# Oliverbansk/Holistic-Robot-Pose-Estimation

Hardware: AMD Instinct MI355X
Metric: images/sec/GPU fwd+bwd HRNet-W32 256x256 bs=64; 1/2/4/8-GPU scaling (higher is better)
Workload: dtype bf16; 1 GPU; full network (HRNet-W32 reg backbone + HRNet-W32 DepthNet + heads + FK loss) fwd+loss+bwd+clip+Adam, BASELINE.json configs[2]; global_batch=64, per_gpu_batch=64, image=3x256x256, hrnet_w32_passes_per_image=2, parallelism=dp1, backend=single-process, rccl_ranks=1, hip_graph=True, plan_mode=hybrid, inputs=resident in HBM, optimizer=hrpe_amd.optim.FusedClipAdam (clip 5 + Adam, lr 1e-4)

## Files before the change

holistic-robot-pose-estimation_amd/_native.py:

```python
import ctypes as C
import os
import subprocess

_HERE = os.path.dirname(os.path.abspath(__file__))
LIB_PATH = os.environ.get("HRP_LIB") or os.path.join(_HERE, "libhrp_hip.so")
CSRC = os.path.join(_HERE, "csrc")

HRP_F32, HRP_BF16, HRP_F32X3 = 0, 1, 2
MAX_TAPS = 16
EW_MAX_IN = 4
EW_IDENTITY, EW_AFFINE, EW_BN_TRAIN = 0, 1, 2
FK_MAX_JOINTS, FK_MAX_KP = 32, 24
PIL_KMAX = 12


class HrpError(RuntimeError):
    pass


class ConvDesc(C.Structure):
    _fields_ = [("x", C.c_void_p), ("w", C.c_void_p), ("y", C.c_void_p), ("res", C.c_void_p),
                ("bias", C.c_void_p), ("scale", C.c_void_p), ("shift", C.c_void_p), ("stats", C.c_void_p),
                ("dtype", C.c_int32),
                ("N", C.c_int32), ("H", C.c_int32), ("W", C.c_int32), ("Cin", C.c_int32), ("x_pitch", C.c_int32),
                ("Ho", C.c_int32), ("Wo", C.c_int32), ("Cout", C.c_int32),
                ("y_H", C.c_int32), ("y_W", C.c_int32), ("y_pitch", C.c_int32), ("res_pitch", C.c_int32),
                ("out_stride", C.c_int32), ("out_off_y", C.c_int32), ("out_off_x", C.c_int32),
                ("in_stride", C.c_int32), ("ntaps", C.c_int32),
                ("dy", C.c_int32 * MAX_TAPS), ("dx", C.c_int32 * MAX_TAPS), ("wtap", C.c_int32 * MAX_TAPS),
                ("w_ntaps", C.c_int32), ("w_cout_pad", C.c_int32), ("relu", C.c_int32),
                ("bnb_x", C.c_void_p), ("bnb_mask", C.c_void_p), ("bnb_consts", C.c_void_p),
                ("bnb_x_pitch", C.c_int32), ("bnb_mask_pitch", C.c_int32),
                ("bnb_stats", C.c_void_p), ("bnb_gamma", C.c_void_p), ("bnb_beta", C.c_void_p),
                ("bnb_count", C.c_float), ("bnb_eps", C.c_float),
                ("pro_mode", C.c_int32), ("pro_reserved", C.c_int32),
                ("pro_x2", C.c_void_p), ("pro_stats", C.c_void_p), ("pro_bsums", C.c_void_p),
                ("pro_gamma", C.c_void_p), ("pro_beta", C.c_void_p),
                ("pro_count", C.c_float), ("pro_eps", C.c_float), ("pro_side", C.c_void_p),
                ("pro_mask", C.c_void_p), ("pro_side2", C.c_void_p), ("pro_side2_acc", C.c_int32), ("pro_reserved2", C.c_int32),
                ("res_mask", C.c_void_p),
                ("tail_mode", C.c_int32), ("tail_side_acc", C.c_int32), ("tail_stats", C.c_void_p), ("tail_bsums", C.c_void_p),
                ("tail_gamma", C.c_void_p), ("tail_beta", C.c_void_p), ("tail_count", C.c_float), ("tail_eps", C.c_float),
                ("tail_mask", C.c_void_p), ("tail_g", C.c_void_p), ("tail_side", C.c_void_p),
                ("tail_x2", C.c_void_p), ("tail_w2", C.c_void_p), ("tail_stats2", C.c_void_p), ("tail_gamma2", C.c_void_p),
                ("tail_beta2", C.c_void_p)]


class WgradDesc(C.Structure):
    _fields_ = [("x", C.c_void_p), ("dy", C.c_void_p), ("dw", C.c_void_p),
                ("dtype", C.c_int32),
                ("N", C.c_int32), ("H", C.c_int32), ("W", C.c_int32), ("Cin", C.c_int32), ("x_pitch", C.c_int32),
                ("Ho", C.c_int32), ("Wo", C.c_int32), ("Cout", C.c_int32), ("dy_pitch", C.c_int32),
                ("in_stride", C.c_int32), ("ntaps", C.c_int32),
                ("dy_t", C.c_int32 * MAX_TAPS), ("dx_t", C.c_int32 * MAX_TAPS),
                ("dw_cin", C.c_int32), ("dw_tap_stride", C.c_int32), ("dw_tap_off", C.c_int32), ("accumulate", C.c_int32),
                ("workspace", C.c_void_p), ("workspace_bytes", C.c_int64),
                ("phase", C.c_int32), ("reserved", C.c_int32)]


class WgradFoldDesc(C.Structure):
    _fields_ = [("workspace", C.c_void_p), ("dw", C.c_void_p),
                ("G", C.c_int32), ("pairs", C.c_int32), ("n_cib", C.c_int32), ("nte", C.c_int32), ("nb", C.c_int32),
                ("Cout", C.c_int32), ("dw_cin", C.c_int32), ("ntaps", C.c_int32), ("dw_tap_stride", C.c_int32),
                ("dw_tap_off", C.c_int32), ("accumulate", C.c_int32), ("reserved", C.c_int32)]


WGRAD_FOUR_WAVE, WGRAD_EIGHT_WAVE_BF16, WGRAD_EIGHT_WAVE_F32X3 = range(3)


class WgradConfig(C.Structure):
    _fields_ = [("program", C.c_int32), ("arrange", C.c_int32), ("nks", C.c_int32), ("BM", C.c_int32),
                ("TI", C.c_int32), ("TH", C.c_int32), ("TW", C.c_int32), ("ring", C.c_int32), ("xmode", C.c_int32),
                ("G", C.c_int32), ("ntiles", C.c_int32), ("pairs", C.c_int32), ("use_ws", C.c_int32),
                ("reserved", C.c_int32 * 3)]


class Sim2RealLossDesc(C.Structure):
    _fields_ = [("rendered", C.c_void_p), ("seg", C.c_void_p), ("kp3d", C.c_void_p), ("kp3d_int", C.c_void_p),
                ("B", C.c_int32), ("HW", C.c_int32), ("K", C.c_int32), ("mask_loss", C.c_int32),
                ("w_mask", C.c_float), ("w_iou", C.c_float), ("w_scale", C.c_float), ("w_align", C.c_float),
                ("terms", C.c_void_p), ("d_rendered", C.c_void_p), ("d_kp3d", C.c_void_p), ("d_kp3d_int", C.c_void_p),
                ("workspace", C.c_void_p)]


class SilhouetteDesc(C.Structure):
    _fields_ = [("uv", C.c_void_p), ("xyz", C.c_void_p), ("faces", C.c_void_p),
                ("B", C.c_int32), ("V", C.c_int32), ("F", C.c_int32), ("H", C.c_int32), ("W", C.c_int32),
                ("sigma", C.c_float), ("blur_radius", C.c_float), ("alpha", C.c_void_p), ("logp", C.c_void_p), ("count", C.c_void_p)]


BLOCK_MAX = 2


class BlockDesc(C.Structure):
    _fields_ = [("conv1", ConvDesc), ("conv2", ConvDesc)]


class BlockInfo(C.Structure):
    _fields_ = [("n", C.c_int32), ("grid", C.c_int32), ("lds_bytes", C.c_int32), ("reserved", C.c_int32),
                ("first_wg", C.c_int32 * BLOCK_MAX), ("bands", C.c_int32 * BLOCK_MAX)]


class PackEntry(C.Structure):
    _fields_ = [("src", C.c_void_p), ("dst", C.c_void_p), ("dst_t", C.c_void_p),
                ("Cout", C.c_int32), ("Cin", C.c_int32), ("ntaps", C.c_int32), ("pad_t", C.c_int32)]


class EwInput(C.Structure):
    _fields_ = [("ptr", C.c_void_p), ("pitch", C.c_int32), ("up", C.c_int32), ("mode", C.c_int32),
                ("a", C.c_void_p), ("b", C.c_void_p), ("stats", C.c_void_p),
                ("count", C.c_float), ("eps", C.c_float)]


class EwDesc(C.Structure):
    _fields_ = [("inp", EwInput * EW_MAX_IN), ("nin", C.c_int32), ("out", C.c_void_p),
                ("out_pitch", C.c_int32), ("dtype", C.c_int32),
                ("N", C.c_int32), ("H", C.c_int32), ("W", C.c_int32), ("C", C.c_int32), ("relu", C.c_int32),
                ("mask", C.c_void_p), ("mask_pitch", C.c_int32), ("consts_out", C.c_void_p)]


class EwBwdDesc(C.Structure):
    _fields_ = [("dout", C.c_void_p), ("out", C.c_void_p), ("dout_pitch", C.c_int32), ("out_pitch", C.c_int32),
                ("inp", EwInput), ("din", C.c_void_p), ("din_pitch", C.c_int32), ("sums", C.c_void_p),
                ("dtype", C.c_int32), ("N", C.c_int32), ("H", C.c_int32), ("W", C.c_int32), ("C", C.c_int32),
                ("relu", C.c_int32), ("accumulate", C.c_int32),
                ("mask", C.c_void_p), ("mask_pitch", C.c_int32),
                ("din2", C.c_void_p), ("din2_pitch", C.c_int32), ("accumulate2", C.c_int32), ("pooled", C.c_void_p)]


class BnEntry(C.Structure):
    _fields_ = [("stats", C.c_void_p), ("a", C.c_void_p), ("b", C.c_void_p), ("c", C.c_void_p), ("d", C.c_void_p),
                ("out_scale", C.c_void_p), ("out_shift", C.c_void_p), ("counter", C.c_void_p),
                ("C", C.c_int32), ("count", C.c_float), ("momentum", C.c_float), ("eps", C.c_float),
                ("accumulate", C.c_int32)]


BATCH_MAX = 32
BATCH_CONV, BATCH_WGRAD, BATCH_EW_FWD, BATCH_EW_BWD_REDUCE, BATCH_EW_BWD_APPLY, BATCH_WGRAD_FOLD = range(6)


class BatchInfo(C.Structure):
    _fields_ = [("family", C.c_int32), ("n", C.c_int32), ("dtype", C.c_int32), ("variant", C.c_int32),
                ("grid", C.c_int32), ("lds_bytes", C.c_int32), ("grid2", C.c_int32),
                ("grid3", C.c_int32), ("lds_bytes3", C.c_int32),
                ("blk0", C.c_int32 * (BATCH_MAX + 1)), ("blk2", C.c_int32 * (BATCH_MAX + 1)),
                ("ws_bytes", C.c_int64 * BATCH_MAX)]


class PoseLossDesc(C.Structure):
    _fields_ = [(n, C.c_void_p) for n in ("pose", "rot", "trans", "root_uv", "depth", "xyz_int", "xyz_fk",
                                          "gt_pose", "gt_root_rot", "gt_root_trans", "gt_root_uv", "gt_kp3d", "gt_kp2d", "mask", "K",
                                          "d_pose", "d_rot", "d_trans", "d_root_uv", "d_depth", "d_xyz_int", "d_xyz_fk", "out")] + \
               [("weights", C.c_float * 10), ("B", C.c_int32), ("P", C.c_int32), ("J", C.c_int32), ("root", C.c_int32),
                ("image_size", C.c_float), ("rot_dim", C.c_int32)]


class EvalDesc(C.Structure):
    INPUTS = ("pred_kp3d_fk", "pred_kp3d_int", "gt_kp3d", "gt_kp2d", "K", "pred_joint", "gt_joint", "pred_rot", "gt_rot")
    PER_IMAGE = ("error3d", "error2d", "mean_jointerror", "error_depth", "batch_error_relative", "error3d_relative",
                 "error3d_int", "error2d_int", "error_depth_int", "batch_error_relative_int", "error3d_relative_int")
    PER_BATCH = ("dis3d", "dis2d", "dis3d_int", "dis2d_int", "l1_jointerror", "rotation_diff")
    _fields_ = [(n, C.c_void_p) for n in INPUTS + PER_IMAGE + PER_BATCH] + \
               [(n, C.c_int32) for n in ("B", "nkp", "dof", "rot_dim", "root", "drop_last_joint", "offset", "capacity",
                                         "batch_index", "batch_capacity")]


DEPTH_LOSS_MAX_KP = 16
DEPTH_LOSS_KINDS = {"l1": 0, "mse": 1}
XY_LOSS_KINDS = {None: 0, "l1": 1, "mse": 2}


class DepthLossDesc(C.Structure):
    POINTERS = ("pred", "gt_root_trans", "gt_kp3d", "mask", "loss", "d_pred", "errors", "losses")
    _fields_ = [(n, C.c_void_p) for n in POINTERS] + \
               [(n, C.c_int32) for n in ("B", "W", "J", "nk")] + [("kp_index", C.c_int32 * DEPTH_LOSS_MAX_KP)] + \
               [(n, C.c_int32) for n in ("depth_loss", "xy_loss", "root_col", "want_grad", "offset", "capacity", "batch_index",
                                         "batch_capacity")]


SIM2REAL_ROW = ("loss", "loss_joint", "loss_rot", "loss_trans", "loss_uv", "loss_depth", "loss_error2d", "loss_error3d", "loss_mask",
                "loss_scale", "loss_iou", "loss_error3d_align")


class Sim2RealMonitorDesc(C.Structure):
    INPUTS = ("pose", "rot", "trans", "root_uv", "depth", "xyz_fk", "gt_pose", "gt_root_rot", "gt_root_trans", "gt_root_uv",
              "gt_kp3d", "gt_kp2d", "mask", "K")
    _fields_ = [(n, C.c_void_p) for n in INPUTS + ("mask_terms", "row", "meters", "rows")] + \
               [("B", C.c_int32), ("P", C.c_int32), ("J", C.c_int32), ("image_size", C.c_float), ("row_index", C.c_int32),
                ("capacity", C.c_int32)]


OPT_CHUNK = 4096


class OptTensor(C.Structure):
    _fields_ = [("param", C.c_void_p), ("grad", C.c_void_p), ("exp_avg", C.c_void_p), ("exp_avg_sq", C.c_void_p),
                ("numel", C.c_int64)]


class OptChunk(C.Structure):
    _fields_ = [("tensor", C.c_int32), ("offset", C.c_int32)]


class OptGroup(C.Structure):
    _fields_ = [("lr", C.c_float), ("beta1", C.c_float), ("beta2", C.c_float), ("eps", C.c_float),
                ("weight_decay", C.c_float), ("reserved", C.c_float * 3)]


class RegStepDesc(C.Structure):
    _fields_ = [("M", C.c_int32), ("P", C.c_int32), ("K", C.c_int32), ("N", C.c_int32),
                ("u_prev", C.c_void_p), ("u_bias", C.c_void_p), ("z", C.c_void_p), ("zw", C.c_void_p),
                ("z_len", C.c_int32), ("z_pitch", C.c_int32), ("zw_sk", C.c_int32), ("zw_sp", C.c_int32),
                ("u_out", C.c_void_p), ("a", C.c_void_p), ("a_mask", C.c_void_p), ("v", C.c_void_p),
                ("a_pitch", C.c_int32), ("v_sk", C.c_int32), ("v_sp", C.c_int32), ("a2_pitch", C.c_int32),
                ("a_out", C.c_void_p), ("w", C.c_void_p), ("bias", C.c_void_p), ("out_mask", C.c_void_p),
                ("a2", C.c_void_p), ("w2", C.c_void_p), ("w_sn", C.c_int64), ("w_sk", C.c_int64),
                ("out_pitch", C.c_int32), ("out_accumulate", C.c_int32), ("out_sum_accumulate", C.c_int32), ("w2_sk", C.c_int32),
                ("out", C.c_void_p), ("out_sum", C.c_void_p)]


class LinWgradDesc(C.Structure):
    _fields_ = [("x", C.c_void_p), ("dy", C.c_void_p), ("dw", C.c_void_p), ("dbias", C.c_void_p),
                ("x_pitch", C.c_int32), ("dy_pitch", C.c_int32), ("dw_ld", C.c_int32), ("M", C.c_int32),
                ("K", C.c_int32), ("N", C.c_int32), ("accumulate", C.c_int32), ("reserved", C.c_int32)]


REG_MAX_P, REG_MAX_PROBLEMS, LIN_WGRAD_MAX = 16, 4, 8
COPY_MAX = 16


class CopyDesc(C.Structure):
    _fields_ = [("src", C.c_void_p), ("dst", C.c_void_p), ("src_pitch", C.c_int), ("dst_pitch", C.c_int), ("rows", C.c_int),
                ("cols", C.c_int), ("accumulate", C.c_int), ("reserved", C.c_int)]


def copy_cols_batch(items, stream):
    for i0 in range(0, len(items), COPY_MAX):
        grp = items[i0:i0 + COPY_MAX]
        arr = (CopyDesc * len(grp))()
        for d, (src, sp, dst, dp, rows, cols, acc) in zip(arr, grp):
            d.src, d.src_pitch, d.dst, d.dst_pitch, d.rows, d.cols, d.accumulate = src, sp, dst, dp, rows, cols, acc
        call("hrp_copy_cols_batch", arr, len(grp), stream)


class FkChain(C.Structure):
    _fields_ = [("njoints", C.c_int32), ("parent", C.c_int32 * FK_MAX_JOINTS), ("type", C.c_int32 * FK_MAX_JOINTS),
                ("cfg", C.c_int32 * FK_MAX_JOINTS), ("mimic_mul", C.c_float * FK_MAX_JOINTS),
                ("mimic_off", C.c_float * FK_MAX_JOINTS), ("origin", (C.c_float * 12) * FK_MAX_JOINTS),
                ("axis", (C.c_float * 3) * FK_MAX_JOINTS), ("nkp", C.c_int32), ("kp_frame", C.c_int32 * FK_MAX_KP),
                ("kp_offset", (C.c_float * 3) * FK_MAX_KP), ("dof", C.c_int32)]


DREAM_BANDS = 32
DREAM_JITTER, DREAM_OCCLUSION, DREAM_SHARPNESS, DREAM_CONTRAST, DREAM_BRIGHTNESS, DREAM_COLOR = 1, 2, 4, 8, 16, 32


class DreamSample(C.Structure):
    _fields_ = [("jitter", C.c_double * 3), ("enh", C.c_double * 4), ("flags", C.c_int32),
                ("occ_x", C.c_int32), ("occ_y", C.c_int32), ("occ_w", C.c_int32), ("occ_h", C.c_int32),
                ("pad_x", C.c_int32), ("pad_y", C.c_int32), ("work_w", C.c_int32), ("work_h", C.c_int32),
                ("crop_x0", C.c_int32), ("crop_y0", C.c_int32), ("crop_x1", C.c_int32), ("crop_y1", C.c_int32),
                ("off_x", C.c_int32), ("off_y", C.c_int32), ("side", C.c_int32), ("reserved", C.c_int32),
                ("noise_off", C.c_int64), ("scratch_off", C.c_int64)]


JPEG_ERR_DATA, JPEG_ERR_MARKER, JPEG_ERR_CODE, JPEG_ERR_INDEX, JPEG_ERR_DESC, JPEG_WARN_TRAILING, JPEG_ERR_CHECKSUM = 1, 2, 4, 8, 16, 32, 64


class JpegHuff(C.Structure):
    _fields_ = [("counts", C.c_uint8 * 16), ("values", C.c_uint8 * 256)]


class JpegImage(C.Structure):
    _fields_ = [("scan_off", C.c_int64), ("scan_len", C.c_int64), ("coef_off", C.c_int64), ("plane_off", C.c_int64),
                ("frame_off", C.c_int64), ("width", C.c_int32), ("height", C.c_int32), ("hsamp", C.c_int32), ("vsamp", C.c_int32),
                ("restart_interval", C.c_int32), ("scan_sum", C.c_uint32), ("sum_len", C.c_int64),
                ("comp_tq", C.c_uint8 * 4), ("comp_td", C.c_uint8 * 4), ("comp_ta", C.c_uint8 * 4), ("reserved2", C.c_uint8 * 4),
                ("quant", (C.c_uint16 * 64) * 4), ("dc", JpegHuff * 2), ("ac", JpegHuff * 2)]


class JpegSegment(C.Structure):
    _fields_ = [("off", C.c_int64), ("len", C.c_int64), ("image", C.c_int32), ("mcu0", C.c_int32)]


TRACK_NO_ESTIMATE, TRACK_BAD_BOX, TRACK_LOST_OUT = 1, 2, 4
TRACK_BBOX_EXTENDED, TRACK_BBOX_ORIGIN, TRACK_BBOX_STRICT = 0, 1, 2
PNP_NO_CONSENSUS, PNP_CONVERGED, PNP_FEW_POINTS = 1, 2, 4
PNP_POOLED_MAX_N, PNP_POOLED_REFITS = 16384, 8
TRACK_MAX_KP, TRACK_MAX_SIZE = 32, 4096
SEED_SKIPPED, SEED_TAKEN, SEED_REFUSED = 1, 2, 4
VERIFY_SKIPPED, VERIFY_KEPT, VERIFY_UNDECIDED, VERIFY_DROPPED = 1, 2, 4, 8
VERIFY_FAIL_SUPPORT, VERIFY_FAIL_COVERAGE, VERIFY_FAIL_IOU = 16, 32, 64
TRACK_MAX_BONES, TRACK_MAX_SAMPLES = 32, 64
KIN_CONVERGED, KIN_AT_LIMIT, KIN_FEW_ROWS, KIN_BAD_START = 1, 2, 4, 8
KIN_MAX_IT = 200
KF_INIT, KF_COASTED, KF_LOST, KF_BAD_START, KF_REWRAPPED, KF_CONVERGED, KF_AT_LIMIT = 1, 2, 4, 8, 16, 32, 64
KIN_FILTER_MAX_N = 20
KS_SMOOTHED, KS_TAIL, KS_INVALID, KS_BAD_LINK, KS_CLAMPED = 1, 2, 4, 8, 16
KP_STRIP_ROWS = 1


class TrackGeom(C.Structure):
    _fields_ = [("status", C.c_int32), ("crop_x0", C.c_int32), ("crop_y0", C.c_int32), ("crop_x1", C.c_int32), ("crop_y1", C.c_int32),
                ("side", C.c_int32), ("off_x", C.c_int32), ("off_y", C.c_int32), ("bbox_strict_bounded", (C.c_float * 4) * 2),
                ("bbox_gt2d_extended", (C.c_float * 4) * 2), ("bbox_strict_bounded_original", C.c_float * 4)]


class TrackVerifyDesc(C.Structure):
    _fields_ = [(n, C.c_void_p) for n in ("state_kp2d", "state_have", "mask", "alpha", "verify_status", "counts", "sums")] + \
               [(n, C.c_int32) for n in ("B", "nkp", "hm", "wm", "nb", "samples", "min_fg", "min_samples")] + \
               [("bones", (C.c_int32 * 2) * TRACK_MAX_BONES), ("scale", C.c_double * 2), ("extend_ratio", C.c_double * 2),
                ("min_support", C.c_double), ("min_coverage", C.c_double), ("min_iou", C.c_double), ("min_prob", C.c_float),
                ("reserved", C.c_int32)]


class KinDesc(C.Structure):
    _fields_ = [(n, C.c_void_p) for n in ("chain", "pts2d", "w2d", "pts3d", "w3d", "K")] + \
               [("K_stride", C.c_int32), ("nkp", C.c_int32)] + [(n, C.c_void_p) for n in ("q0", "rot0", "trans0")] + \
               [("rot_dim", C.c_int32), ("pose_stride", C.c_int32)] + [(n, C.c_void_p) for n in ("q_lo", "q_hi", "prior_q")] + \
               [("free_q", C.c_uint32), ("free_pose", C.c_int32), ("root", C.c_int32), ("B", C.c_int32), ("dof", C.c_int32),
                ("reserved", C.c_int32)] + \
               [(n, C.c_void_p) for n in ("q", "rot", "trans", "xyz", "uv", "rms", "status", "cov")]


class KinFilterDesc(C.Structure):
    _fields_ = [(n, C.c_void_p) for n in ("chain", "pts2d", "w2d", "K")] + [("K_stride", C.c_int32), ("nkp", C.c_int32)] + \
               [(n, C.c_void_p) for n in ("q_in", "rot_in", "trans_in")] + [("rot_dim", C.c_int32), ("pose_stride", C.c_int32)] + \
               [(n, C.c_void_p) for n in ("q_lo", "q_hi", "w_q", "q_meas", "keep", "q_acc", "p0_var")] + \
               [("free_q", C.c_uint32), ("free_pose", C.c_int32), ("root", C.c_int32), ("B", C.c_int32), ("dof", C.c_int32),
                ("max_coast", C.c_int32), ("dt", C.c_double), ("gate_chi2", C.c_double)] + \
               [(n, C.c_void_p) for n in ("mean", "cov", "valid", "coast", "q", "rot", "trans", "xyz", "uv", "vel", "cov_p", "xyz_next", "d2",
                                          "status")]


class KinHistoryDesc(C.Structure):
    _fields_ = [(n, C.c_void_p) for n in ("mean", "cov", "valid", "status", "q_in", "h_mean", "h_cov", "h_valid", "h_flags", "h_dt", "h_q_in")] + \
               [(n, C.c_int32) for n in ("B", "n", "dof", "cap", "slot", "reserved")] + [("dt", C.c_double)]


class KinSmoothDesc(C.Structure):
    _fields_ = [(n, C.c_void_p) for n in ("chain", "mean", "cov", "valid", "flags", "dt", "q_in", "rot_fixed", "trans_fixed", "q_lo", "q_hi",
                                          "q_acc", "gain", "link")] + \
               [("free_q", C.c_uint32)] + [(n, C.c_int32) for n in ("free_pose", "root", "B", "dof", "nkp", "rot_dim", "cap", "first", "L",
                                                                    "want_cov", "reserved")] + \
               [(n, C.c_void_p) for n in ("q", "rot", "trans", "vel", "cov_p", "xyz", "status", "mean_s", "cov_s")]


_P, _I, _F, _L, _Z = C.c_void_p, C.c_int, C.c_float, C.c_int64, C.c_size_t
PROTOTYPES = {
    "hrp_version": [], "hrp_device_ok": [],
    "hrp_nchw_to_nhwc": [_P, _P, _I, _I, _I, _I, _I, _I, _P],
    "hrp_nhwc_to_nchw": [_P, _P, _I, _I, _I, _I, _I, _I, _P],
    "hrp_nchw_grad_from_nhwc": [_P, _P, _I, _I, _I, _I, _I, _I, _P],
    "hrp_pack_weights": [_P, _I, _I, _I, _P],
    "hrp_pack_blocks": [_I, _I, _I, _I, _I, _I],
    "hrp_pack_weights_compact": [_P, _P, _I, _I, _I, _P],
    "hrp_nchw_to_nhwc_s2d": [_P, _P, _I, _I, _I, _I, _I, _I, _P],
    "hrp_u8_nchw_to_nhwc": [_P, _P, _I, _I, _I, _I, _I, _I, _F, _I, _P],
    "hrp_gather_f32": [_P, _P, _P, _I, _I, _P],
    "hrp_pil_resize_table": [_I, _I, _P],
    "hrp_pil_resize_normalize": [_P, _I, _I, _I, _I, _P, _P, _I, _I, _P, _I, _I, _I, _P, _P, _P],
    "hrp_broadcast_hw": [_P, _I, _P, _I, _I, _I, _I, _I, _P],
    "hrp_bilinear_nhwc_to_nchw": [_P, _I, _I, _I, _I, _I, _I, _P, _I, _I, _I, _P],
    "hrp_fill_zero": [_P, _L, _P],
    "hrp_maxpool3x3s2_fwd": [_P, _I, _I, _I, _I, _I, _I, _P, _I, _P, _P],
    "hrp_maxpool3x3s2_bwd": [_P, _I, _P, _P, _I, _I, _I, _I, _I, _I, _I, _P],
    "hrp_conv2d_fwd": [C.POINTER(ConvDesc), _P],
    "hrp_conv_rowstrip_channels": [C.POINTER(ConvDesc)],
    "hrp_conv_pointwise": [C.POINTER(ConvDesc)],
    "hrp_conv_parity_fusable": [C.POINTER(ConvDesc)],
    "hrp_conv_parity_fuse_enable": [_I],
    "hrp_conv_tile_config": [C.POINTER(ConvDesc)],
    "hrp_conv2d_bwd_weight": [C.POINTER(WgradDesc), _P],
    "hrp_colsum": [_P, _I, _L, _I, _I, _P, _I, _P, _L, _P],
    "hrp_colsum_workspace_bytes": [_L, _I],
    "hrp_ew_fwd": [C.POINTER(EwDesc), _P],
    "hrp_ew_bwd_reduce": [C.POINTER(EwBwdDesc), _P],
    "hrp_ew_pool2": [_P, _I, _I, _P, _I, _I, _I, _I, _I, _P, _P],
    "hrp_ew_bwd_apply": [C.POINTER(EwBwdDesc), _P],
    "hrp_bn_running_update": [_P, _I, _P], "hrp_bn_fold": [_P, _I, _P], "hrp_bn_param_grad": [_P, _I, _P],
    "hrp_avgpool_fwd": [_P, _I, _I, _I, _I, _I, _P, _I, _P],
    "hrp_avgpool_bwd": [_P, _I, _P, _I, _I, _I, _I, _I, _I, _P],
    "hrp_softargmax3d_fwd": [_P, _I, _I, _I, _I, _I, _I, _I, _I, _I, _P, _P, _P],
    "hrp_softargmax3d_bwd": [_P, _I, _I, _I, _I, _I, _I, _I, _I, _I, _P, _P, _P, _P, _I, _P],
    "hrp_pose_geometry_fwd": [_P, _P, _P, _P, _I, _I, _I, _F, _F, _P, _P, _P, _P, _P],
    "hrp_pose_geometry_bwd": [_P, _P, _P, _P, _I, _I, _I, _F, _F, _P, _P, _P, _P, _P, _P, _P],
    "hrp_fk_project_fwd": [_P, _P, _P, _P, _P, _I, _I, _P, _P, _P, _P],
    "hrp_fk_project_bwd": [_P, _P, _P, _P, _P, _I, _I, _P, _P, _P, _P, _P, _P],
    "hrp_fk_project_rot_fwd": [_P, _P, _P, _I, _P, _P, _I, _I, _P, _P, _P, _P],
    "hrp_fk_project_rot_bwd": [_P, _P, _P, _I, _P, _P, _I, _I, _P, _P, _P, _P, _P, _P],
    "hrp_copy_cols": [_P, _I, _P, _I, _I, _I, _I, _P],
    "hrp_copy_cols_batch": [_P, _I, _P],
    "hrp_scale_rows": [_P, _I, _I, _I, _P, _F, _P],
    "hrp_mul_f32": [_P, _I, _P, _I, _P, _I, _I, _I, _I, _P],
    "hrp_opt_grad_sumsq": [_P, _P, _I, _P, _P, _P],
    "hrp_opt_adam_step": [_P, _P, _I, _P, _F, _P, _F, _F, _F, _F, _P],
    "hrp_opt_adam_step_groups": [_P, _P, _I, _P, _F, _P, _P, _I, _P, _P],
    "hrp_opt_set_group": [_P, _I, _I, _F, _F, _F, _F, _F, _P],
    "hrp_grad_accumulate": [_P, _P, _L, _I, _F, _P],
    "hrp_batch_prepare": [_I, _P, _I, _P, C.POINTER(BatchInfo)],
    "hrp_batch_launch": [_P, C.POINTER(BatchInfo), _P],
    "hrp_batch_conv_parity_configs": [_P, C.POINTER(BatchInfo), _P],
    "hrp_softargmax_flat_fwd": [_P, _I, _I, _I, _I, _I, _P, _P, _P],
    "hrp_softargmax_flat_bwd": [_P, _I, _I, _I, _I, _I, _P, _P, _P, _P, _I, _P],
    "hrp_rot6d_compose_fwd": [_P, _P, _P, _I, _P],
    "hrp_rot6d_compose_bwd": [_P, _P, _P, _P, _P, _I, _I, _I, _P],
    "hrp_wgrad_fold_desc_of": [C.POINTER(WgradDesc), C.POINTER(WgradFoldDesc)],
    "hrp_batch_wgrad_fold_descs": [_P, C.POINTER(BatchInfo), C.POINTER(WgradFoldDesc)],
    "hrp_wgrad_config_of": [C.POINTER(WgradDesc), C.POINTER(WgradConfig)],
    "hrp_batch_wgrad_configs": [_P, C.POINTER(BatchInfo), C.POINTER(WgradConfig)],
    "hrp_block_channels": [C.POINTER(BlockDesc)],
    "hrp_block_prepare": [_P, _I, _P, C.POINTER(BlockInfo)],
    "hrp_block_launch": [_P, C.POINTER(BlockInfo), _P],
    "hrp_pose_loss": [C.POINTER(PoseLossDesc), _P],
    "hrp_l1_loss": [_P, _P, _F, _I, _P, _P, _P],
    "hrp_sim2real_loss": [C.POINTER(Sim2RealLossDesc), _P],
    "hrp_mesh_pose": [_P, _P, _P, _P, _I, _I, _P, _P, _I, _P, _P, _P, _P],
    "hrp_mesh_pose_bwd": [_P, _P, _P, _P, _I, _I, _P, _P, _I, _P, _P, _P, _P],
    "hrp_silhouette_fwd": [C.POINTER(SilhouetteDesc), _P],
    "hrp_silhouette_bwd": [C.POINTER(SilhouetteDesc), _P, _P, _P],
    "hrp_linear_fwd": [_P, _I, _P, _P, _P, _I, _P, _I, _I, _I, _I, _P, _L, _P],
    "hrp_linear_bwd_data": [_P, _I, _P, _P, _I, _I, _I, _I, _I, _P, _L, _P],
    "hrp_linear_workspace_bytes": [_I, _I, _I],
    "hrp_linear_bwd_weight": [_P, _I, _P, _I, _P, _P, _I, _I, _I, _I, _P],
    "hrp_rng_advance": [_P, _P],
    "hrp_dropout_f32": [_P, _I, _P, _I, _P, _I, _I, _F, _P, C.c_uint32, _P],
    "hrp_dropout_masks": [_P, _L, _F, _P, C.c_uint32, _P],
    "hrp_regressor_step": [_P, _I, _P],
    "hrp_linear_wgrad_batch": [_P, _I, _P],
    "hrp_project_fwd": [_P, _P, _I, _I, _P, _P],
    "hrp_project_bwd": [_P, _P, _P, _I, _I, _P, _P],
    "hrp_pnp_solve": [_P, _P, _I, _P, _I, _P, _I, _I, _P, _P, _P, _P],
    "hrp_pnp_bwd": [_P, _P, _I, _P, _I, _P, _P, _I, _I, _I, _P, _P, _P, _P, _P, _P, _P],
    "hrp_pnp_solve_robust": [_P, _P, _I, _P, _I, _P, _I, _I, C.c_double, _I, _I, C.c_uint32, _I, _P, _P, _P, _P, _P],
    "hrp_pnp_bwd_masked": [_P, _P, _I, _P, _I, _P, _P, _P, _I, _I, _I, _P, _P, _P, _P, _P, _P, _P],
    "hrp_pnp_pooled_workspace_bytes": [_I, _I, _I, C.POINTER(C.c_size_t)],
    "hrp_pnp_solve_pooled": [_P, _P, _P, _I, _P, _I, _I, C.c_double, _I, _I, C.c_uint32, _I, _P, _Z, _P, _P, _P, _P, _P, _P],
    "hrp_dream_augment": [_P, _I, _I, _I, _P, _P, _L, _I, _I, _P, _L, _P, _P],
    "hrp_dream_crop_resize": [_P, _L, _P, _P, _I, _I, _I, _P, _I, _I, _P, _I, _I, _P],
    "hrp_eval_batch": [C.POINTER(EvalDesc), _P],
    "hrp_depth_loss": [C.POINTER(DepthLossDesc), _P],
    "hrp_sim2real_monitor": [C.POINTER(Sim2RealMonitorDesc), _P],
    "hrp_jpeg_decode": [_P, _I, _P, _I, _P, _Z, _P, _Z, _P, _Z, _P, _Z, _P, _P],
    "hrp_jpeg_decode_stage": [_I, _I, _P, _I, _P, _I, _P, _Z, _P, _Z, _P, _Z, _P, _Z, _P, _P],
    "hrp_jpeg_decode_sync": [_P, _I, _P, _I, _P, _I, _I, _P, _Z, _P, _Z, _P, _Z, _P, _Z, _P, _Z, _P, _P],
    "hrp_jpeg_decode_sync_stage": [_I, _I, _I, _P, _I, _P, _I, _P, _I, _I, _P, _Z, _P, _Z, _P, _Z, _P, _Z, _P, _Z, _P, _P],
    "hrp_jpeg_sync_scratch_bytes": [_Z, _I, _I],
    "hrp_track_prepare": [_P, _P, _P, _P, _I, _I, _I, _I, _P, _I, _I, _P, _I, _I, C.POINTER(C.c_double), _I, _P, _P, _P, _P, _P],
    "hrp_track_update": [_P, _P, _I, _I, _I, _I, _I, _P, _P, _P, _P, _P],
    "hrp_track_seed": [_P, _I, _I, C.POINTER(C.c_double), _P, _I, _I, _F, _P, _F, _I, _I, _I, _I, _P, _P, _P, _P],
    "hrp_track_verify": [C.POINTER(TrackVerifyDesc), _P],
    "hrp_kin_solve": [C.POINTER(KinDesc), _P],
    "hrp_kin_filter_step": [C.POINTER(KinFilterDesc), _P],
    "hrp_kin_history_push": [C.POINTER(KinHistoryDesc), _P],
    "hrp_kin_smooth": [C.POINTER(KinSmoothDesc), _P],
    "hrp_kp_readout_pack": [_P, _I, _I, _P, _I, _P],
    "hrp_kp_readout_ws": [_I, _I],
    "hrp_kp_readout_fwd": [_P, _I, _I, _I, _I, _I, _I, _P, _P, _I, _F, _F, _F, _F, _P, _P, _P, _L, _P],
}

_lib = None


def source_hash():
    import glob
    import hashlib
    files = [os.path.basename(f) for f in glob.glob(os.path.join(CSRC, "*.hip")) + glob.glob(os.path.join(CSRC, "*.h"))]
    names = sorted(files + ["../../include/hrp.h", "Makefile"])
    h = hashlib.sha256()
    for n in names:
        with open(os.path.join(CSRC, n), "rb") as fh:
            h.update(fh.read())
    return h.hexdigest()[:16]


def build(force=False):
    if force:
        subprocess.run(["make", "-C", CSRC, "clean"], check=True, stdout=subprocess.DEVNULL)
    r = subprocess.run(["make", "-C", CSRC, "-j8"], stdout=subprocess.PIPE, stderr=subprocess.STDOUT, text=True)
    if r.returncode != 0:
        raise HrpError("building libhrp_hip.so failed:\n" + r.stdout[-4000:])
    return LIB_PATH


def lib():
    global _lib
    if _lib is None:
        if not os.path.exists(LIB_PATH):
            raise HrpError(f"{LIB_PATH} not found: run `python -c 'import __graft_entry__ as g; g.build()'` "
                           "(there is no CPU fallback)")
        import torch
        L = C.CDLL(LIB_PATH)
        for name, args in PROTOTYPES.items():
            fn = getattr(L, name)
            fn.argtypes = args
            fn.restype = C.c_int
        L.hrp_last_error.restype = C.c_char_p
        L.hrp_last_error.argtypes = []
        L.hrp_source_hash.restype = C.c_char_p
        L.hrp_source_hash.argtypes = []
        L.hrp_wgrad_workspace_bytes.restype = C.c_int64
        L.hrp_linear_workspace_bytes.restype = C.c_int64
        L.hrp_colsum_workspace_bytes.restype = C.c_int64
        L.hrp_wgrad_workspace_bytes.argtypes = [C.POINTER(WgradDesc)]
        L.hrp_batch_table_bytes.restype = C.c_int64
        L.hrp_batch_table_bytes.argtypes = [C.c_int, C.c_int]
        L.hrp_block_table_bytes.restype = C.c_int64
        L.hrp_block_table_bytes.argtypes = []
        L.hrp_jpeg_sync_scratch_bytes.restype = C.c_size_t
        L.hrp_kp_readout_ws.restype = C.c_int64
        _lib = L
    return _lib


def check(rc, what=""):
    if rc != 0:
        raise HrpError(f"{what} failed ({rc}): {lib().hrp_last_error().decode()}")


_profile_hook = None


def set_profile_hook(fn):
    global _profile_hook
    _profile_hook = fn


def profiling():
    return _profile_hook is not None


_skip = frozenset(filter(None, os.environ.get("HRP_SKIP", "").split(",")))


def call(name, *args):
    if _skip and name in _skip:
        return
    if _profile_hook is not None:
        _profile_hook(name, args, lambda: check(getattr(lib(), name)(*args), name))
        return
    check(getattr(lib(), name)(*args), name)


def call_batch(batch, stream):
    name = "hrp_batch_launch"
    if _skip and (name in _skip or FAMILY_FN[batch.fam] in _skip):
        return
    fn = lambda: check(lib().hrp_batch_launch(batch.table.data_ptr(), C.byref(batch.info), stream), name)
    if _profile_hook is not None:
        _profile_hook(name, (batch,), fn)
        return
    fn()


def call_block(batch, stream):
    name = "hrp_block_launch"
    if _skip and name in _skip:
        return
    fn = lambda: check(lib().hrp_block_launch(batch.table, C.byref(batch.info), stream), name)
    if _profile_hook is not None:
        _profile_hook(name, (batch,), fn)
        return
    fn()


FAMILY_FN = {"block": "hrp_block_launch", "conv": "hrp_conv2d_fwd", "wgrad": "hrp_conv2d_bwd_weight", "wgrad_fold": "hrp_wgrad_fold", "ew_fwd": "hrp_ew_fwd", "ew_red": "hrp_ew_bwd_reduce",
             "ew_app": "hrp_ew_bwd_apply"}
```

holistic-robot-pose-estimation_amd/csrc/core.hip:

```cpp
#include "hrp_common.h"
#include <type_traits>
#include <string.h>

namespace hrp {

static thread_local char g_err[512] = "";

void set_error(const char* fmt, ...) {
  va_list ap;
  va_start(ap, fmt);
  vsnprintf(g_err, sizeof(g_err), fmt, ap);
  va_end(ap);
}

int check_launch(const char* what) {
  hipError_t e = hipGetLastError();
  if (e != hipSuccess) {
    set_error("%s: %s", what, hipGetErrorString(e));
    return HRP_ERR_LAUNCH;
  }
  return HRP_OK;
}

template <typename T, typename S>
__global__ __launch_bounds__(256) void nchw_to_nhwc_kernel(const S* __restrict__ src, void* __restrict__ dst,
                                                           int C, int HW, int pitch, float div) {
  size_t p = (size_t)blockIdx.x * 256 + threadIdx.x;
  int n = blockIdx.y;
  if (p >= (size_t)HW) return;
  const S* s = src + (size_t)n * C * HW + p;
  size_t o = ((size_t)n * HW + p) * pitch;
  if (pitch * Elem<T>::SZ == 16) {
    constexpr int V = 16 / Elem<T>::SZ;
    float v[V];
#pragma unroll
    for (int c = 0; c < V; ++c) {
      v[c] = c < C ? (float)s[(size_t)c * HW] : 0.f;
      if (sizeof(S) == 1) v[c] = v[c] * (1.0f / div);
    }
    *(uint4*)((char*)dst + o * Elem<T>::SZ) = Elem<T>::pack(v);
    return;
  }
  for (int c = 0; c < pitch; ++c) {
    float v = c < C ? (float)s[(size_t)c * HW] : 0.f;
    if (sizeof(S) == 1) v = v * (1.0f / div);
    Elem<T>::st(dst, o + c, v);
  }
}

template <typename T, typename S>
__global__ __launch_bounds__(256) void nchw_to_nhwc_s2d_kernel(const S* __restrict__ src, void* __restrict__ dst,
                                                               int C, int H, int W, int pitch, float div) {
  const int Ho = (H + 1) / 2, Wo = (W + 1) / 2;
  size_t p = (size_t)blockIdx.x * 256 + threadIdx.x;
  const int n = blockIdx.y;
  if (p >= (size_t)Ho * Wo) return;
  const int y = p / Wo, x = p - (size_t)y * Wo;
  const S* sn = src + (size_t)n * C * H * W;
  size_t o = ((size_t)n * Ho * Wo + p) * pitch;
  for (int k = 0; k < pitch; ++k) {
    float v = 0.f;
    if (k < 4 * C) {
      const int q = k / C, c = k - q * C, iy = 2 * y + (q >> 1), ix = 2 * x + (q & 1);
      if (iy < H && ix < W) v = (float)sn[((size_t)c * H + iy) * W + ix];
      if (sizeof(S) == 1) v = v * (1.0f / div);
    }
    Elem<T>::st(dst, o + k, v);
  }
}

__global__ __launch_bounds__(256) void gather_f32_kernel(const float* __restrict__ src, const int* __restrict__ idx,
                                                         float* __restrict__ dst, int n, int accumulate) {
  const int i = blockIdx.x * 256 + threadIdx.x;
  if (i >= n) return;
  const int j = idx[i];
  const float v = j >= 0 ? src[j] : 0.f;
  dst[i] = accumulate ? dst[i] + v : v;
}

template <typename T>
__global__ __launch_bounds__(256) void maxpool_fwd_kernel(const void* __restrict__ x, int H, int W, int C, int pitch,
                                                          void* __restrict__ y, int Ho, int Wo, int y_pitch,
                                                          uint8_t* __restrict__ arg, long total) {
  constexpr int V = Elem<T>::VEC;
  const int nv = C / V;
  for (long i = (long)blockIdx.x * 256 + threadIdx.x; i < total; i += (long)gridDim.x * 256) {
    const int cv = i % nv;
    long r = i / nv;
    const int ox = r % Wo; r /= Wo;
    const int oy = r % Ho;
    const long n = r / Ho;
    float best[V];
    int bi[V];
#pragma unroll
    for (int k = 0; k < V; ++k) { best[k] = -INFINITY; bi[k] = 0; }
    for (int ky = 0; ky < 3; ++ky) {
      const int iy = 2 * oy - 1 + ky;
      if (iy < 0 || iy >= H) continue;
      for (int kx = 0; kx < 3; ++kx) {
        const int ix = 2 * ox - 1 + kx;
        if (ix < 0 || ix >= W) continue;
        float f[V];
        Elem<T>::unpack(*(const uint4*)((const char*)x + ((((size_t)n * H + iy) * W + ix) * pitch + cv * V) * Elem<T>::SZ), f);
#pragma unroll
        for (int k = 0; k < V; ++k)
          if (f[k] > best[k]) { best[k] = f[k]; bi[k] = ky * 3 + kx; }
      }
    }
    const size_t o = (((size_t)n * Ho + oy) * Wo + ox);
    *(uint4*)((char*)y + (o * y_pitch + cv * V) * Elem<T>::SZ) = Elem<T>::pack(best);
    if (arg) {
#pragma unroll
      for (int k = 0; k < V; ++k) arg[o * C + cv * V + k] = (uint8_t)bi[k];
    }
  }
}

template <typename T>
__global__ __launch_bounds__(256) void maxpool_bwd_kernel(const void* __restrict__ dy, int Ho, int Wo, int dy_pitch,
                                                          const uint8_t* __restrict__ arg, void* __restrict__ dx, int H, int W,
                                                          int C, int pitch, int accumulate, long total) {
  constexpr int V = Elem<T>::VEC;
  const int nv = C / V;
  for (long i = (long)blockIdx.x * 256 + threadIdx.x; i < total; i += (long)gridDim.x * 256) {
    const int cv = i % nv;
    long r = i / nv;
    const int ix = r % W; r /= W;
    const int iy = r % H;
    const long n = r / H;
    float g[V];
#pragma unroll
    for (int k = 0; k < V; ++k) g[k] = 0.f;
    for (int oy = iy / 2; oy <= (iy + 1) / 2; ++oy) {
      if (oy < 0 || oy >= Ho) continue;
      const int ky = iy - (2 * oy - 1);
      if (ky < 0 || ky > 2) continue;
      for (int ox = ix / 2; ox <= (ix + 1) / 2; ++ox) {
        if (ox < 0 || ox >= Wo) continue;
        const int kx = ix - (2 * ox - 1);
        if (kx < 0 || kx > 2) continue;
        const size_t o = (((size_t)n * Ho + oy) * Wo + ox);
        float f[V];
        Elem<T>::unpack(*(const uint4*)((const char*)dy + (o * dy_pitch + cv * V) * Elem<T>::SZ), f);
        const uint8_t* a = arg + o * C + cv * V;
#pragma unroll
        for (int k = 0; k < V; ++k)
          if (a[k] == ky * 3 + kx) g[k] += f[k];
      }
    }
    char* dst = (char*)dx + ((((size_t)n * H + iy) * W + ix) * pitch + cv * V) * Elem<T>::SZ;
    if (accumulate) {
      float old[V];
      Elem<T>::unpack(*(const uint4*)dst, old);
#pragma unroll
      for (int k = 0; k < V; ++k) g[k] += old[k];
    }
    *(uint4*)dst = Elem<T>::pack(g);
  }
}

template <typename T, bool GRAD>
__global__ __launch_bounds__(256) void nhwc_to_nchw_kernel(const void* __restrict__ src, float* __restrict__ dst,
                                                           int C, int HW, int pitch) {
  __shared__ float tile[64][65];
  const int n = blockIdx.z, p0 = blockIdx.x * 64, c0 = blockIdx.y * 64;
  const int tx = threadIdx.x & 63, ty = threadIdx.x >> 6;
  for (int r = ty; r < 64; r += 4) {
    int p = p0 + r, c = c0 + tx;
    tile[r][tx] = (p < HW && c < C) ? Elem<T>::ld(src, ((size_t)n * HW + p) * pitch + c) : 0.f;
  }
  __syncthreads();
  for (int r = ty; r < 64; r += 4) {
    int c = c0 + r, p = p0 + tx;
    if (p < HW && c < C) dst[((size_t)n * C + c) * HW + p] = tile[tx][r];
  }
}

template <typename T>
__device__ __forceinline__ void pack_entry(const hrp_pack_entry& e, const unsigned blk, const unsigned nblk) {
  constexpr int CK = 32 / Elem<T>::SZ;
  const unsigned Cout = e.Cout, Cin = e.Cin, nt = e.ntaps;
  const unsigned cout_pad = (Cout + 31) / 32 * 32, cin_pad = (Cin + 31) / 32 * 32;
  auto store_row = [&](void* dst, size_t row, const float (&v)[CK]) {
    if constexpr (std::is_same<T, f32x3_t>::value) {
      uint4* q = (uint4*)((char*)dst + row * 32);
      split_bf16x8(v, q[0], q[1]);
      return;
    }
    float a[CK / 2], b[CK / 2];
#pragma unroll
    for (int k = 0; k < CK / 2; ++k) { a[k] = v[k]; b[k] = v[CK / 2 + k]; }
    uint4* q = (uint4*)((char*)dst + row * 32);
    q[0] = Elem<T>::pack(a);
    q[1] = Elem<T>::pack(b);
  };
  if (e.dst) {
    const unsigned nch = (Cin + CK - 1) / CK, rows = nch * nt * cout_pad;
    for (unsigned i = blk * 256 + threadIdx.x; i < rows; i += nblk * 256) {
      const unsigned tap = i % nt, q = i / nt, co = q % cout_pad, ch = q / cout_pad;
      float v[CK];
#pragma unroll
      for (int k = 0; k < CK; ++k) {
        const unsigned ci = ch * CK + k;
        v[k] = (co < Cout && ci < Cin) ? e.src[((size_t)co * Cin + ci) * nt + tap] : 0.f;
      }
      store_row(e.dst, (size_t)(ch * nt + tap) * cout_pad + co, v);
    }
  }
  if (e.dst_t) {
    const unsigned nch = (Cout + CK - 1) / CK, rows = nch * nt * cin_pad;
    for (unsigned i = blk * 256 + threadIdx.x; i < rows; i += nblk * 256) {
      const unsigned tap = i % nt, q = i / nt, ci = q % cin_pad, ch = q / cin_pad;
      float v[CK];
#pragma unroll
      for (int k = 0; k < CK; ++k) {
        const unsigned co = ch * CK + k;
        v[k] = (co < Cout && ci < Cin) ? e.src[((size_t)co * Cin + ci) * nt + tap] : 0.f;
      }
      store_row(e.dst_t, (size_t)(ch * (nt + e.pad_t) + tap) * cin_pad + ci, v);
    }
  }
}

template <typename T>
__global__ __launch_bounds__(256) void pack_weights_kernel(const hrp_pack_entry* __restrict__ table) {
  const hrp_pack_entry e = table[blockIdx.y];
  pack_entry<T>(e, blockIdx.x, gridDim.x);
}

constexpr int PACK_TILE_TAPS = 9;
template <typename T>
__device__ __forceinline__ void pack_store_row(void* dst, const size_t row, const float (&v)[32 / Elem<T>::SZ]) {
  constexpr int CK = 32 / Elem<T>::SZ;
  uint4* q = (uint4*)((char*)dst + row * 32);
  if constexpr (std::is_same<T, f32x3_t>::value) {
    split_bf16x8(v, q[0], q[1]);
  } else {
    float a[CK / 2], b[CK / 2];
#pragma unroll
    for (int k = 0; k < CK / 2; ++k) { a[k] = v[k]; b[k] = v[CK / 2 + k]; }
    q[0] = Elem<T>::pack(a);
    q[1] = Elem<T>::pack(b);
  }
}

template <typename T>
__device__ __forceinline__ void pack_entry_tile(const hrp_pack_entry& e, const unsigned tile_id, float* __restrict__ lds) {
  constexpr int CK = 32 / Elem<T>::SZ, NC = 32 / CK;
  const unsigned Cout = e.Cout, Cin = e.Cin, nt = e.ntaps;
  const unsigned cout_pad = (Cout + 31) / 32 * 32, cin_pad = (Cin + 31) / 32 * 32;
  const unsigned n_cit = cin_pad / 32;
  if (tile_id >= (cout_pad / 32) * n_cit) return;
  const unsigned co0 = (tile_id / n_cit) * 32, ci0 = (tile_id % n_cit) * 32;
  const unsigned span = 32 * nt, pitch = span + 1;
  {
    const unsigned wave = threadIdx.x >> 6, lane = threadIdx.x & 63;
    const unsigned valid = Cin > ci0 ? (Cin - ci0 < 32 ? (Cin - ci0) * nt : span) : 0;
    for (unsigned r0 = wave; r0 < 32; r0 += 16) {
      for (unsigned j = lane; j < span; j += 64) {
        float v[4];
#pragma unroll
        for (int u = 0; u < 4; ++u) {
          const unsigned co = co0 + r0 + 4 * u;
          v[u] = (co < Cout && j < valid) ? e.src[((size_t)co * Cin + ci0) * nt + j] : 0.f;
        }
#pragma unroll
        for (int u = 0; u < 4; ++u) lds[(r0 + 4 * u) * pitch + j] = v[u];
      }
    }
  }
  __syncthreads();
  if (e.dst) {
    const unsigned nch = (Cin + CK - 1) / CK;
    for (unsigned r = threadIdx.x; r < NC * nt * 32; r += 256) {
      const unsigned co = r & 31, q = r >> 5, tap = q % nt, c = q / nt, ch = ci0 / CK + c;
      if (ch >= nch) continue;
      float v[CK];
#pragma unroll
      for (int k = 0; k < CK; ++k) v[k] = lds[co * pitch + (c * CK + k) * nt + tap];
      pack_store_row<T>(e.dst, (size_t)(ch * nt + tap) * cout_pad + co0 + co, v);
    }
  }
  if (e.dst_t) {
    const unsigned nch = (Cout + CK - 1) / CK;
    for (unsigned r = threadIdx.x; r < NC * nt * 32; r += 256) {
      const unsigned ci = r & 31, q = r >> 5, tap = q % nt, c = q / nt, ch = co0 / CK + c;
      if (ch >= nch) continue;
      float v[CK];
#pragma unroll
      for (int k = 0; k < CK; ++k) v[k] = lds[(c * CK + k) * pitch + ci * nt + tap];
      pack_store_row<T>(e.dst_t, (size_t)(ch * (nt + e.pad_t) + tap) * cin_pad + ci0 + ci, v);
    }
  }
}

constexpr int PACK_ROWS_PER_BLOCK = 256 * 4;
template <typename T>
__global__ __launch_bounds__(256) void pack_weights_compact_kernel(const hrp_pack_entry* __restrict__ table, const int32_t* __restrict__ first,
                                                                   const int count) {
  int lo = 0, hi = count;
  while (hi - lo > 1) {
    const int mid = (lo + hi) >> 1;
    if (first[mid] <= (int)blockIdx.x) lo = mid; else hi = mid;
  }
  const hrp_pack_entry e = table[lo];
  if (e.ntaps <= PACK_TILE_TAPS) {
    __shared__ float lds[32 * (32 * PACK_TILE_TAPS + 1)];
    pack_entry_tile<T>(e, blockIdx.x - first[lo], lds);
    return;
  }
  pack_entry<T>(e, blockIdx.x - first[lo], first[lo + 1] - first[lo]);
}

template <typename T>
__global__ __launch_bounds__(256) void colsum_kernel(const void* __restrict__ x, long rows, int C, int pitch,
                                                     float* __restrict__ out, float* __restrict__ ws) {
  __shared__ float part[4][64];
  const int tx = threadIdx.x & 63, ty = threadIdx.x >> 6;
  const int c = blockIdx.y * 64 + tx;
  float s = 0.f;
  if (c < C)
    for (long r = (long)blockIdx.x * 4 + ty; r < rows; r += (long)gridDim.x * 4) s += Elem<T>::ld(x, (size_t)r * pitch + c);
  part[ty][tx] = s;
  __syncthreads();
  if (ty == 0 && c < C) {
    const float v = part[0][tx] + part[1][tx] + part[2][tx] + part[3][tx];
    if (ws) ws[(size_t)blockIdx.x * C + c] = v;
    else atomicAdd(&out[c], v);
  }
}

__global__ __launch_bounds__(256) void colsum_fold_kernel(const float* __restrict__ ws, int groups, int C, float* __restrict__ out,
                                                          int accumulate) {
  const int c = blockIdx.x * 256 + threadIdx.x;
  if (c >= C) return;
  float v = 0.f;
  for (int g0 = 0; g0 < groups; g0 += 8) {
    float t[8];
#pragma unroll
    for (int u = 0; u < 8; ++u) t[u] = g0 + u < groups ? ws[(size_t)(g0 + u) * C + c] : 0.f;
#pragma unroll
    for (int u = 0; u < 8; ++u) v += t[u];
  }
  out[c] = accumulate ? out[c] + v : v;
}

__global__ void bn_running_update_kernel(const hrp_bn_entry* __restrict__ table) {
  const hrp_bn_entry e = table[blockIdx.x];
  for (int c = threadIdx.x; c < e.C; c += blockDim.x) {
    float mean = slot_sum(e.stats, c, 2 * e.C) / e.count;
    float var = fmaxf(slot_sum(e.stats, e.C + c, 2 * e.C) / e.count - mean * mean, 0.f);
    float unbiased = e.count > 1.f ? var * (e.count / (e.count - 1.f)) : var;
    e.a[c] = (1.f - e.momentum) * e.a[c] + e.momentum * mean;
    e.b[c] = (1.f - e.momentum) * e.b[c] + e.momentum * unbiased;
  }
  if (threadIdx.x == 0 && e.counter) *e.counter += 1;
}

__global__ void bn_fold_kernel(const hrp_bn_entry* __restrict__ table) {
  const hrp_bn_entry e = table[blockIdx.x];
  for (int c = threadIdx.x; c < e.C; c += blockDim.x) {
    float sc = e.a[c] * rsqrtf(e.d[c] + e.eps);
    e.out_scale[c] = sc;
    e.out_shift[c] = e.b[c] - e.c[c] * sc;
  }
}

__global__ void bn_param_grad_kernel(const hrp_bn_entry* __restrict__ table) {
  const hrp_bn_entry e = table[blockIdx.x];
  for (int c = threadIdx.x; c < e.C; c += blockDim.x) {
    float dbeta = slot_sum(e.stats, c, 2 * e.C), dgamma = slot_sum(e.stats, e.C + c, 2 * e.C);
    if (e.accumulate) { e.a[c] += dgamma; e.b[c] += dbeta; }
    else { e.a[c] = dgamma; e.b[c] = dbeta; }
  }
}

template <typename T>
__global__ __launch_bounds__(256) void avgpool_fwd_kernel(const void* __restrict__ x, int HW, int C, int pitch,
                                                          float* __restrict__ out, int out_pitch) {
  const int n = blockIdx.y;
  const int c = blockIdx.x * 256 + threadIdx.x;
  if (c >= C) return;
  float s = 0.f;
  for (int p = 0; p < HW; ++p) s += Elem<T>::ld(x, ((size_t)n * HW + p) * pitch + c);
  out[(size_t)n * out_pitch + c] = s / (float)HW;
}

template <typename T>
__global__ __launch_bounds__(256) void avgpool_bwd_kernel(const float* __restrict__ dout, int dout_pitch, void* __restrict__ dx,
                                                          int HW, int C, int pitch, int accumulate) {
  const int n = blockIdx.y;
  const int c = blockIdx.x * 256 + threadIdx.x;
  if (c >= C) return;
  const float g = dout[(size_t)n * dout_pitch + c] / (float)HW;
  for (int p = 0; p < HW; ++p) {
    size_t o = ((size_t)n * HW + p) * pitch + c;
    Elem<T>::st(dx, o, accumulate ? Elem<T>::ld(dx, o) + g : g);
  }
}

__global__ void copy_cols_kernel(const float* __restrict__ src, int sp, float* __restrict__ dst, int dp, int rows, int cols, int acc) {
  size_t i = (size_t)blockIdx.x * 256 + threadIdx.x;
  if (i >= (size_t)rows * cols) return;
  int r = i / cols, c = i % cols;
  float v = src[(size_t)r * sp + c];
  float* d = dst + (size_t)r * dp + c;
  *d = acc ? *d + v : v;
}

struct CopyBatchArgs { hrp_copy_desc d[HRP_COPY_MAX]; };
__global__ void copy_cols_batch_kernel(const CopyBatchArgs a) {
  const hrp_copy_desc& d = a.d[blockIdx.y];
  const size_t total = (size_t)d.rows * d.cols;
  for (size_t i = (size_t)blockIdx.x * 256 + threadIdx.x; i < total; i += (size_t)gridDim.x * 256) {
    const int r = (int)(i / d.cols), c = (int)(i - (size_t)r * d.cols);
    const float v = d.src ? d.src[(size_t)r * d.src_pitch + c] : 0.f;
    float* q = d.dst + (size_t)r * d.dst_pitch + c;
    *q = d.accumulate ? *q + v : v;
  }
}

__global__ void scale_rows_kernel(float* __restrict__ x, int pitch, int rows, int cols, const float* __restrict__ rs, float s) {
  size_t i = (size_t)blockIdx.x * 256 + threadIdx.x;
  if (i >= (size_t)rows * cols) return;
  int r = i / cols, c = i % cols;
  x[(size_t)r * pitch + c] *= (rs ? rs[r] : 1.f) * s;
}

__global__ void mul_kernel(const float* __restrict__ x, int xp, const float* __restrict__ m, int mp, float* __restrict__ y, int yp,
                           int rows, int cols, int acc) {
  size_t i = (size_t)blockIdx.x * 256 + threadIdx.x;
  if (i >= (size_t)rows * cols) return;
  int r = i / cols, c = i % cols;
  float v = x[(size_t)r * xp + c] * m[(size_t)r * mp + c];
  float* d = y + (size_t)r * yp + c;
  *d = acc ? *d + v : v;
}

__device__ __forceinline__ void philox_round(uint32_t (&c)[4], uint32_t k0, uint32_t k1) {
  const uint32_t hi0 = __umulhi(0xD2511F53u, c[0]), lo0 = 0xD2511F53u * c[0];
  const uint32_t hi1 = __umulhi(0xCD9E8D57u, c[2]), lo1 = 0xCD9E8D57u * c[2];
  const uint32_t n0 = hi1 ^ c[1] ^ k0, n1 = lo1, n2 = hi0 ^ c[3] ^ k1, n3 = lo0;
  c[0] = n0; c[1] = n1; c[2] = n2; c[3] = n3;
}

__global__ void rng_advance_kernel(uint64_t* state) { state[1] += 1; }

__global__ __launch_bounds__(256) void dropout_kernel(const float* __restrict__ x, int xp, float* __restrict__ y, int yp,
                                                      float* __restrict__ mask, int rows, int cols, float keep,
                                                      const uint64_t* __restrict__ state, uint32_t salt) {
  const size_t q = (size_t)blockIdx.x * 256 + threadIdx.x;
  const size_t n = (size_t)rows * cols;
  if (q * 4 >= n) return;
  const uint64_t seed = state[0], step = state[1];
  uint32_t c[4] = {(uint32_t)q, (uint32_t)(q >> 32) ^ salt, (uint32_t)step, (uint32_t)(step >> 32)};
  uint32_t k0 = (uint32_t)seed, k1 = (uint32_t)(seed >> 32);
#pragma unroll
  for (int r = 0; r < 10; ++r) {
    philox_round(c, k0, k1);
    k0 += 0x9E3779B9u; k1 += 0xBB67AE85u;
  }
  const float scale = 1.0f / keep;
#pragma unroll
  for (int j = 0; j < 4; ++j) {
    const size_t i = q * 4 + j;
    if (i >= n) break;
    const float u = (float)(c[j] >> 8) * (1.0f / 16777216.0f);
    const float m = u < keep ? scale : 0.f;
    const int r = (int)(i / cols), cc = (int)(i - (size_t)r * cols);
    mask[i] = m;
    y[(size_t)r * yp + cc] = x[(size_t)r * xp + cc] * m;
  }
}

}

using namespace hrp;

#ifndef HRP_SRC_HASH
#define HRP_SRC_HASH "unknown"
#endif
extern "C" const char* hrp_source_hash(void) { return HRP_SRC_HASH; }

extern "C" int hrp_rng_advance(uint64_t* state_dev, void* stream) {
  HRP_REQUIRE(state_dev, "rng_advance: null state");
  hipLaunchKernelGGL(rng_advance_kernel, dim3(1), dim3(1), 0, (hipStream_t)stream, state_dev);
  return check_launch("rng_advance");
}

extern "C" int hrp_dropout_f32(const float* x, int x_pitch, float* y, int y_pitch, float* mask, int rows, int cols, float keep,
                               const uint64_t* state_dev, uint32_t salt, void* stream) {
  HRP_REQUIRE(x && y && mask && state_dev && rows > 0 && cols > 0, "dropout: bad args");
  HRP_REQUIRE(keep > 0.f && keep <= 1.f, "dropout: keep probability %f", (double)keep);
  const size_t quads = ((size_t)rows * cols + 3) / 4;
  hipLaunchKernelGGL(dropout_kernel, dim3((unsigned)((quads + 255) / 256)), dim3(256), 0, (hipStream_t)stream, x, x_pitch, y, y_pitch,
                     mask, rows, cols, keep, state_dev, salt);
  return check_launch("dropout");
}

extern "C" int hrp_mul_f32(const float* x, int x_pitch, const float* m, int m_pitch, float* y, int y_pitch, int rows, int cols,
                           int accumulate, void* stream) {
  HRP_REQUIRE(x && m && y && rows > 0 && cols > 0, "mul_f32: bad args");
  hipLaunchKernelGGL(mul_kernel, dim3(cdiv(rows * cols, 256)), dim3(256), 0, (hipStream_t)stream, x, x_pitch, m, m_pitch, y, y_pitch,
                     rows, cols, accumulate);
  return check_launch("mul_f32");
}

extern "C" const char* hrp_last_error(void) { return hrp::g_err; }
extern "C" int hrp_version(void) { return 100; }

extern "C" int hrp_device_ok(void) {
  int dev = 0;
  if (hipGetDevice(&dev) != hipSuccess) return 0;
  hipDeviceProp_t p;
  if (hipGetDeviceProperties(&p, dev) != hipSuccess) return 0;
  return strncmp(p.gcnArchName, "gfx950", 6) == 0 ? 1 : 0;
}

extern "C" int hrp_nchw_to_nhwc(const float* src, void* dst, int dtype, int N, int C, int H, int W, int dst_pitch, void* stream) {
  HRP_REQUIRE(src && dst && N > 0 && C > 0 && dst_pitch >= C, "nchw_to_nhwc: bad args");
  dim3 grid(cdiv(H * W, 256), N);
  if (dtype == HRP_F32) hipLaunchKernelGGL((nchw_to_nhwc_kernel<float, float>), grid, dim3(256), 0, (hipStream_t)stream, src, dst, C, H * W, dst_pitch, 1.f);
  else hipLaunchKernelGGL((nchw_to_nhwc_kernel<bf16_t, float>), grid, dim3(256), 0, (hipStream_t)stream, src, dst, C, H * W, dst_pitch, 1.f);
  return check_launch("nchw_to_nhwc");
}

extern "C" int hrp_u8_nchw_to_nhwc(const uint8_t* src, void* dst, int dtype, int N, int C, int H, int W, int dst_pitch,
                                   float divisor, int s2d, void* stream) {
  HRP_REQUIRE(src && dst && N > 0 && C > 0 && divisor > 0.f, "u8_nchw_to_nhwc: bad args");
  HRP_REQUIRE(dst_pitch >= (s2d ? 4 * C : C), "u8_nchw_to_nhwc: dst_pitch too small");
  hipStream_t st = (hipStream_t)stream;
  if (s2d) {
    dim3 grid(cdiv(((H + 1) / 2) * ((W + 1) / 2), 256), N);
    if (dtype == HRP_F32) hipLaunchKernelGGL((nchw_to_nhwc_s2d_kernel<float, uint8_t>), grid, dim3(256), 0, st, src, dst, C, H, W, dst_pitch, divisor);
    else hipLaunchKernelGGL((nchw_to_nhwc_s2d_kernel<bf16_t, uint8_t>), grid, dim3(256), 0, st, src, dst, C, H, W, dst_pitch, divisor);
  } else {
    dim3 grid(cdiv(H * W, 256), N);
    if (dtype == HRP_F32) hipLaunchKernelGGL((nchw_to_nhwc_kernel<float, uint8_t>), grid, dim3(256), 0, st, src, dst, C, H * W, dst_pitch, divisor);
    else hipLaunchKernelGGL((nchw_to_nhwc_kernel<bf16_t, uint8_t>), grid, dim3(256), 0, st, src, dst, C, H * W, dst_pitch, divisor);
  }
  return check_launch("u8_nchw_to_nhwc");
}

extern "C" int hrp_nchw_to_nhwc_s2d(const float* src, void* dst, int dtype, int N, int C, int H, int W, int dst_pitch, void* stream) {
  HRP_REQUIRE(src && dst && N > 0 && C > 0 && dst_pitch >= 4 * C, "nchw_to_nhwc_s2d: bad args");
  dim3 grid(cdiv(((H + 1) / 2) * ((W + 1) / 2), 256), N);
  if (dtype == HRP_F32) hipLaunchKernelGGL((nchw_to_nhwc_s2d_kernel<float, float>), grid, dim3(256), 0, (hipStream_t)stream, src, dst, C, H, W, dst_pitch, 1.f);
  else hipLaunchKernelGGL((nchw_to_nhwc_s2d_kernel<bf16_t, float>), grid, dim3(256), 0, (hipStream_t)stream, src, dst, C, H, W, dst_pitch, 1.f);
  return check_launch("nchw_to_nhwc_s2d");
}

extern "C" int hrp_fill_zero(void* p, int64_t bytes, void* stream) {
  HRP_REQUIRE(p && bytes >= 0, "fill_zero: bad args");
  zero_async(p, (size_t)bytes, (hipStream_t)stream);
  return check_launch("fill_zero");
}

extern "C" int hrp_gather_f32(const float* src, const int32_t* idx, float* dst, int n, int accumulate, void* stream) {
  HRP_REQUIRE(src && idx && dst && n > 0, "gather_f32: bad args");
  hipLaunchKernelGGL(gather_f32_kernel, dim3(cdiv(n, 256)), dim3(256), 0, (hipStream_t)stream, src, idx, dst, n, accumulate);
  return check_launch("gather_f32");
}

extern "C" int hrp_maxpool3x3s2_fwd(const void* x, int dtype, int N, int H, int W, int C, int pitch, void* y, int y_pitch,
                                    uint8_t* argmax, void* stream) {
  const int vec = dtype == HRP_F32 ? 4 : 8, sz = dtype == HRP_F32 ? 4 : 2;
  HRP_REQUIRE(x && y && N > 0 && H > 0 && W > 0 && C > 0, "maxpool_fwd: bad args");
  HRP_REQUIRE(C % vec == 0 && pitch % vec == 0 && y_pitch % vec == 0 && (uintptr_t)x % 16 == 0 && (uintptr_t)y % 16 == 0,
              "maxpool_fwd: channels / pitches must be multiples of %d and the tensors 16-byte aligned", vec);
  (void)sz;
  const int Ho = (H + 2 - 3) / 2 + 1, Wo = (W + 2 - 3) / 2 + 1;
  const long total = (long)N * Ho * Wo * (C / vec);
  long blocks = (total + 255) / 256;
  if (blocks > 4096) blocks = 4096;
  if (dtype == HRP_F32) hipLaunchKernelGGL(maxpool_fwd_kernel<float>, dim3((int)blocks), dim3(256), 0, (hipStream_t)stream, x, H, W, C, pitch, y, Ho, Wo, y_pitch, argmax, total);
  else hipLaunchKernelGGL(maxpool_fwd_kernel<bf16_t>, dim3((int)blocks), dim3(256), 0, (hipStream_t)stream, x, H, W, C, pitch, y, Ho, Wo, y_pitch, argmax, total);
  return check_launch("maxpool_fwd");
}

extern "C" int hrp_maxpool3x3s2_bwd(const void* dy, int dy_pitch, const uint8_t* argmax, void* dx, int dtype, int N, int H, int W,
                                    int C, int pitch, int accumulate, void* stream) {
  const int vec = dtype == HRP_F32 ? 4 : 8;
  HRP_REQUIRE(dy && argmax && dx && N > 0 && H > 0 && W > 0 && C > 0, "maxpool_bwd: bad args");
  HRP_REQUIRE(C % vec == 0 && pitch % vec == 0 && dy_pitch % vec == 0 && (uintptr_t)dx % 16 == 0 && (uintptr_t)dy % 16 == 0,
              "maxpool_bwd: channels / pitches must be multiples of %d and the tensors 16-byte aligned", vec);
  const int Ho = (H + 2 - 3) / 2 + 1, Wo = (W + 2 - 3) / 2 + 1;
  const long total = (long)N * H * W * (C / vec);
  long blocks = (total + 255) / 256;
  if (blocks > 4096) blocks = 4096;
  if (dtype == HRP_F32) hipLaunchKernelGGL(maxpool_bwd_kernel<float>, dim3((int)blocks), dim3(256), 0, (hipStream_t)stream, dy, Ho, Wo, dy_pitch, argmax, dx, H, W, C, pitch, accumulate, total);
  else hipLaunchKernelGGL(maxpool_bwd_kernel<bf16_t>, dim3((int)blocks), dim3(256), 0, (hipStream_t)stream, dy, Ho, Wo, dy_pitch, argmax, dx, H, W, C, pitch, accumulate, total);
  return check_launch("maxpool_bwd");
}

extern "C" int hrp_nhwc_to_nchw(const void* src, float* dst, int dtype, int N, int C, int H, int W, int src_pitch, void* stream) {
  HRP_REQUIRE(src && dst && N > 0 && C > 0 && src_pitch >= C, "nhwc_to_nchw: bad args");
  dim3 grid(cdiv(H * W, 64), cdiv(C, 64), N);
  if (dtype == HRP_F32) hipLaunchKernelGGL((nhwc_to_nchw_kernel<float, false>), grid, dim3(256), 0, (hipStream_t)stream, src, dst, C, H * W, src_pitch);
  else hipLaunchKernelGGL((nhwc_to_nchw_kernel<bf16_t, false>), grid, dim3(256), 0, (hipStream_t)stream, src, dst, C, H * W, src_pitch);
  return check_launch("nhwc_to_nchw");
}

extern "C" int hrp_nchw_grad_from_nhwc(const void* src, float* dst, int dtype, int N, int C, int H, int W, int src_pitch, void* stream) {
  return hrp_nhwc_to_nchw(src, dst, dtype, N, C, H, W, src_pitch, stream);
}

extern "C" int hrp_pack_weights(const hrp_pack_entry* table_dev, int count, int dtype, int max_elems, void* stream) {
  HRP_REQUIRE(table_dev && count > 0, "pack_weights: empty table");
  int bx = cdiv(max_elems, 256 * 16 * 4);
  if (bx < 1) bx = 1;
  if (bx > 256) bx = 256;
  dim3 grid(bx, count);
  if (dtype == HRP_F32) hipLaunchKernelGGL(pack_weights_kernel<float>, grid, dim3(256), 0, (hipStream_t)stream, table_dev);
  else if (dtype == HRP_F32X3) hipLaunchKernelGGL(pack_weights_kernel<f32x3_t>, grid, dim3(256), 0, (hipStream_t)stream, table_dev);
  else hipLaunchKernelGGL(pack_weights_kernel<bf16_t>, grid, dim3(256), 0, (hipStream_t)stream, table_dev);
  return check_launch("pack_weights");
}

extern "C" int hrp_pack_blocks(int Cout, int Cin, int ntaps, int dtype, int has_dst, int has_dst_t) {
  if (Cout <= 0 || Cin <= 0 || ntaps <= 0) return 0;
  const int CK = dtype == HRP_BF16 ? 16 : 8;
  const long cout_pad = (Cout + 31) / 32 * 32, cin_pad = (Cin + 31) / 32 * 32;
  if (ntaps <= PACK_TILE_TAPS) return (int)((cout_pad / 32) * (cin_pad / 32));
  const long rf = has_dst ? (long)cdiv(Cin, CK) * ntaps * cout_pad : 0, rt = has_dst_t ? (long)cdiv(Cout, CK) * ntaps * cin_pad : 0;
  const long rows = rf > rt ? rf : rt;
  const long b = (rows + PACK_ROWS_PER_BLOCK - 1) / PACK_ROWS_PER_BLOCK;
  return (int)(b < 1 ? 1 : b);
}

extern "C" int hrp_pack_weights_compact(const hrp_pack_entry* table_dev, const int32_t* first_block_dev, int count, int total_blocks,
                                        int dtype, void* stream) {
  HRP_REQUIRE(table_dev && first_block_dev && count > 0 && total_blocks >= count, "pack_weights_compact: empty table / fewer workgroups than entries");
  const dim3 grid(total_blocks);
  if (dtype == HRP_F32) hipLaunchKernelGGL(pack_weights_compact_kernel<float>, grid, dim3(256), 0, (hipStream_t)stream, table_dev, first_block_dev, count);
  else if (dtype == HRP_F32X3) hipLaunchKernelGGL(pack_weights_compact_kernel<f32x3_t>, grid, dim3(256), 0, (hipStream_t)stream, table_dev, first_block_dev, count);
  else hipLaunchKernelGGL(pack_weights_compact_kernel<bf16_t>, grid, dim3(256), 0, (hipStream_t)stream, table_dev, first_block_dev, count);
  return check_launch("pack_weights_compact");
}

static inline int colsum_groups(int64_t rows) {
  int gx = (int)((rows + 63) / 64);
  if (gx > 512) gx = 512;
  return gx < 1 ? 1 : gx;
}

extern "C" int64_t hrp_colsum_workspace_bytes(int64_t rows, int C) { return rows > 0 && C > 0 ? (int64_t)colsum_groups(rows) * C * 4 : 0; }

extern "C" int hrp_colsum(const void* x, int dtype, int64_t rows, int C, int pitch, float* out, int accumulate, void* workspace,
                          int64_t workspace_bytes, void* stream) {
  HRP_REQUIRE(x && out && rows > 0 && C > 0, "colsum: bad args");
  const int gx = colsum_groups(rows);
  float* ws = (float*)workspace;
  HRP_REQUIRE(!ws || workspace_bytes >= (int64_t)gx * C * 4, "colsum: workspace too small");
  if (!ws && !accumulate) zero_async(out, sizeof(float) * C, (hipStream_t)stream);
  dim3 grid(gx, cdiv(C, 64));
  if (dtype == HRP_F32) hipLaunchKernelGGL(colsum_kernel<float>, grid, dim3(256), 0, (hipStream_t)stream, x, (long)rows, C, pitch, out, ws);
  else hipLaunchKernelGGL(colsum_kernel<bf16_t>, grid, dim3(256), 0, (hipStream_t)stream, x, (long)rows, C, pitch, out, ws);
  if (ws) hipLaunchKernelGGL(colsum_fold_kernel, dim3(cdiv(C, 256)), dim3(256), 0, (hipStream_t)stream, ws, gx, C, out, accumulate);
  return check_launch("colsum");
}

extern "C" int hrp_bn_running_update(const hrp_bn_entry* table_dev, int count, void* stream) {
  HRP_REQUIRE(table_dev && count > 0, "bn_running_update: empty table");
  hipLaunchKernelGGL(bn_running_update_kernel, dim3(count), dim3(256), 0, (hipStream_t)stream, table_dev);
  return check_launch("bn_running_update");
}
extern "C" int hrp_bn_fold(const hrp_bn_entry* table_dev, int count, void* stream) {
  HRP_REQUIRE(table_dev && count > 0, "bn_fold: empty table");
  hipLaunchKernelGGL(bn_fold_kernel, dim3(count), dim3(256), 0, (hipStream_t)stream, table_dev);
  return check_launch("bn_fold");
}
extern "C" int hrp_bn_param_grad(const hrp_bn_entry* table_dev, int count, void* stream) {
  HRP_REQUIRE(table_dev && count > 0, "bn_param_grad: empty table");
  hipLaunchKernelGGL(bn_param_grad_kernel, dim3(count), dim3(256), 0, (hipStream_t)stream, table_dev);
  return check_launch("bn_param_grad");
}

__global__ __launch_bounds__(256) void opt_grad_sumsq_kernel(const hrp_opt_tensor* __restrict__ tensors,
                                                             const hrp_opt_chunk* __restrict__ chunks,
                                                             float* __restrict__ slots, float* __restrict__ chunk_sums) {
  const hrp_opt_chunk ck = chunks[blockIdx.x];
  const hrp_opt_tensor t = tensors[ck.tensor];
  const int64_t base = (int64_t)ck.offset * HRP_OPT_CHUNK;
  const int64_t left = t.numel - base;
  const int n = left < HRP_OPT_CHUNK ? (int)left : HRP_OPT_CHUNK;
  const float* g = t.grad + base;
  float s = 0.f;
  if ((n & 3) == 0 && ((uintptr_t)g & 15) == 0) {
    for (int i = threadIdx.x * 4; i < n; i += 1024) {
      const float4 v = *(const float4*)(g + i);
      s += v.x * v.x + v.y * v.y + v.z * v.z + v.w * v.w;
    }
  } else {
    for (int i = threadIdx.x; i < n; i += 256) s += g[i] * g[i];
  }
  s = wave_sum(s);
  __shared__ float part[4];
  if ((threadIdx.x & 63) == 0) part[threadIdx.x >> 6] = s;
  __syncthreads();
  if (threadIdx.x == 0) {
    const float tot = part[0] + part[1] + part[2] + part[3];
    if (chunk_sums) chunk_sums[blockIdx.x] = tot;
    else atomicAdd(&slots[blockIdx.x & (HRP_STAT_SLOTS - 1)], tot);
  }
}

__global__ __launch_bounds__(256) void opt_fold_sumsq_kernel(const float* __restrict__ chunk_sums, int n, float* __restrict__ slots) {
  __shared__ float part[256];
  float s = 0.f;
  for (int i = threadIdx.x; i < n; i += 256) s += chunk_sums[i];
  part[threadIdx.x] = s;
  __syncthreads();
  for (int o = 128; o > 0; o >>= 1) {
    if ((int)threadIdx.x < o) part[threadIdx.x] += part[threadIdx.x + o];
    __syncthreads();
  }
  if (threadIdx.x < HRP_STAT_SLOTS) slots[threadIdx.x] = threadIdx.x == 0 ? part[0] : 0.f;
}

template <bool DECAY>
__device__ __forceinline__ void opt_adam_chunk(const hrp_opt_tensor t, const hrp_opt_chunk ck, const float* __restrict__ slots,
                                               float max_norm, const float* __restrict__ step_dev, float lr, float b1, float b2,
                                               float eps, float wd) {
  const int64_t base = (int64_t)ck.offset * HRP_OPT_CHUNK;
  const int64_t left = t.numel - base;
  const int n = left < HRP_OPT_CHUNK ? (int)left : HRP_OPT_CHUNK;
  float clip = 1.f;
  if (max_norm > 0.f) {
    float ss = 0.f;
#pragma unroll
    for (int k = 0; k < HRP_STAT_SLOTS; ++k) ss += slots[k];
    clip = fminf(1.f, max_norm / (sqrtf(ss) + 1e-6f));
  }
  const float step = *step_dev;
  const float bc1 = 1.f - powf(b1, step), bc2 = 1.f - powf(b2, step);
  const float step_size = lr / bc1, inv_sqrt_bc2 = 1.f / sqrtf(bc2);
  float* p = t.param + base;
  float* g = t.grad + base;
  float* m = t.exp_avg + base;
  float* v = t.exp_avg_sq + base;
  auto run = [&](auto with_decay) {
    auto upd = [&](float& pp, float& gg, float& mm, float& vv) {
      gg *= clip;
      if constexpr (decltype(with_decay)::value) {
        const float ge = gg + wd * pp;
        mm = b1 * mm + (1.f - b1) * ge;
        vv = b2 * vv + (1.f - b2) * ge * ge;
      } else {
        mm = b1 * mm + (1.f - b1) * gg;
        vv = b2 * vv + (1.f - b2) * gg * gg;
      }
      pp -= step_size * mm / (sqrtf(vv) * inv_sqrt_bc2 + eps);
    };
    if ((n & 3) == 0 && (((uintptr_t)p | (uintptr_t)g | (uintptr_t)m | (uintptr_t)v) & 15) == 0) {
      for (int i = threadIdx.x * 4; i < n; i += 1024) {
        float4 pp = *(float4*)(p + i), gg = *(float4*)(g + i), mm = *(float4*)(m + i), vv = *(float4*)(v + i);
        upd(pp.x, gg.x, mm.x, vv.x); upd(pp.y, gg.y, mm.y, vv.y); upd(pp.z, gg.z, mm.z, vv.z); upd(pp.w, gg.w, mm.w, vv.w);
        *(float4*)(p + i) = pp; *(float4*)(g + i) = gg; *(float4*)(m + i) = mm; *(float4*)(v + i) = vv;
      }
    } else {
      for (int i = threadIdx.x; i < n; i += 256) upd(p[i], g[i], m[i], v[i]);
    }
  };
  if (DECAY && wd != 0.f) run(std::true_type{});
  else run(std::false_type{});
}

__global__ __launch_bounds__(256) void opt_adam_kernel(const hrp_opt_tensor* __restrict__ tensors,
                                                       const hrp_opt_chunk* __restrict__ chunks,
                                                       const float* __restrict__ slots, float max_norm,
                                                       const float* __restrict__ step_dev, float lr, float b1, float b2,
                                                       float eps) {
  const hrp_opt_chunk ck = chunks[blockIdx.x];
  const hrp_opt_tensor t = tensors[ck.tensor];
  opt_adam_chunk<false>(t, ck, slots, max_norm, step_dev, lr, b1, b2, eps, 0.f);
}

__global__ __launch_bounds__(256) void opt_adam_groups_kernel(const hrp_opt_tensor* __restrict__ tensors,
                                                              const hrp_opt_chunk* __restrict__ chunks,
                                                              const float* __restrict__ slots, float max_norm,
                                                              const float* __restrict__ step_dev,
                                                              const hrp_opt_group* __restrict__ groups, int ngroups,
                                                              const int32_t* __restrict__ tensor_group) {
  const hrp_opt_chunk ck = chunks[blockIdx.x];
  const int gi = tensor_group[ck.tensor];
  const hrp_opt_group h = groups[gi < 0 ? 0 : gi >= ngroups ? ngroups - 1 : gi];
  opt_adam_chunk<true>(tensors[ck.tensor], ck, slots, max_norm, step_dev, h.lr, h.beta1, h.beta2, h.eps, h.weight_decay);
}

__global__ void opt_set_group_kernel(hrp_opt_group* __restrict__ groups, int index, float lr, float b1, float b2, float eps,
                                     float wd) {
  hrp_opt_group h = {};
  h.lr = lr, h.beta1 = b1, h.beta2 = b2, h.eps = eps, h.weight_decay = wd;
  groups[index] = h;
}

extern "C" int hrp_opt_grad_sumsq(const hrp_opt_tensor* tensors_dev, const hrp_opt_chunk* chunks_dev, int nchunks,
                                  float* sumsq_slots, float* chunk_sums, void* stream) {
  HRP_REQUIRE(tensors_dev && chunks_dev && sumsq_slots && nchunks > 0, "opt_grad_sumsq: bad args");
  hipLaunchKernelGGL(opt_grad_sumsq_kernel, dim3(nchunks), dim3(256), 0, (hipStream_t)stream, tensors_dev, chunks_dev, sumsq_slots,
                     chunk_sums);
  if (chunk_sums)
    hipLaunchKernelGGL(opt_fold_sumsq_kernel, dim3(1), dim3(256), 0, (hipStream_t)stream, chunk_sums, nchunks, sumsq_slots);
  return check_launch("opt_grad_sumsq");
}
extern "C" int hrp_opt_adam_step(const hrp_opt_tensor* tensors_dev, const hrp_opt_chunk* chunks_dev, int nchunks,
                                 const float* sumsq_slots, float max_norm, const float* step_dev,
                                 float lr, float beta1, float beta2, float eps, void* stream) {
  HRP_REQUIRE(tensors_dev && chunks_dev && step_dev && nchunks > 0, "opt_adam_step: bad args");
  HRP_REQUIRE(max_norm <= 0.f || sumsq_slots, "opt_adam_step: clipping needs the sum-of-squares slots");
  hipLaunchKernelGGL(opt_adam_kernel, dim3(nchunks), dim3(256), 0, (hipStream_t)stream, tensors_dev, chunks_dev, sumsq_slots,
                     max_norm, step_dev, lr, beta1, beta2, eps);
  return check_launch("opt_adam_step");
}

extern "C" int hrp_opt_adam_step_groups(const hrp_opt_tensor* tensors_dev, const hrp_opt_chunk* chunks_dev, int nchunks,
                                        const float* sumsq_slots, float max_norm, const float* step_dev,
                                        const hrp_opt_group* groups_dev, int ngroups, const int32_t* tensor_group_dev,
                                        void* stream) {
  HRP_REQUIRE(tensors_dev && chunks_dev && step_dev && nchunks > 0, "opt_adam_step_groups: bad args");
  HRP_REQUIRE(groups_dev && tensor_group_dev, "opt_adam_step_groups: null group table");
  HRP_REQUIRE(ngroups >= 1, "opt_adam_step_groups: ngroups %d < 1", ngroups);
  HRP_REQUIRE(max_norm <= 0.f || sumsq_slots, "opt_adam_step_groups: clipping needs the sum-of-squares slots");
  hipLaunchKernelGGL(opt_adam_groups_kernel, dim3(nchunks), dim3(256), 0, (hipStream_t)stream, tensors_dev, chunks_dev,
                     sumsq_slots, max_norm, step_dev, groups_dev, ngroups, tensor_group_dev);
  return check_launch("opt_adam_step_groups");
}
extern "C" int hrp_opt_set_group(hrp_opt_group* groups_dev, int ngroups, int index, float lr, float beta1, float beta2, float eps,
                                 float weight_decay, void* stream) {
  HRP_REQUIRE(groups_dev, "opt_set_group: null group table");
  HRP_REQUIRE(ngroups >= 1, "opt_set_group: ngroups %d < 1", ngroups);
  HRP_REQUIRE(index >= 0 && index < ngroups, "opt_set_group: index %d outside [0, %d)", index, ngroups);
  hipLaunchKernelGGL(opt_set_group_kernel, dim3(1), dim3(1), 0, (hipStream_t)stream, groups_dev, index, lr, beta1, beta2, eps,
                     weight_decay);
  return check_launch("opt_set_group");
}

constexpr int GACC_THREADS = 256, GACC_MAX_BLOCKS = 256 * 8;

typedef float gacc_f4 __attribute__((ext_vector_type(4)));

template <int MODE, bool SCALED, typename V>
__device__ __forceinline__ V gacc_sum(V a, V s, float scale) {
#pragma clang fp contract(off)
  V v = s;
  if (SCALED) v = s * scale;
  if (MODE) v = a + v;
  return v;
}
template <int MODE, typename V>
__device__ __forceinline__ V gacc_load(const V* p) {
  if (MODE) return *p;
  return V(0.f);
}

template <int MODE, bool SCALED>
__global__ __launch_bounds__(GACC_THREADS) void grad_accumulate_kernel(const float* __restrict__ src, float* __restrict__ acc,
                                                                       int64_t n, float scale) {
  const int64_t nvec = n >> 2;
  const int64_t stride = (int64_t)gridDim.x * GACC_THREADS;
  const gacc_f4* __restrict__ s4 = (const gacc_f4*)src;
  gacc_f4* __restrict__ a4 = (gacc_f4*)acc;
  int64_t i = (int64_t)blockIdx.x * GACC_THREADS + threadIdx.x;
  for (; i + stride < nvec; i += 2 * stride) {
    const gacc_f4 s0 = s4[i], s1 = s4[i + stride];
    const gacc_f4 a0 = gacc_load<MODE>(a4 + i), a1 = gacc_load<MODE>(a4 + i + stride);
    a4[i] = gacc_sum<MODE, SCALED>(a0, s0, scale);
    a4[i + stride] = gacc_sum<MODE, SCALED>(a1, s1, scale);
  }
  if (i < nvec) a4[i] = gacc_sum<MODE, SCALED>(gacc_load<MODE>(a4 + i), s4[i], scale);
  const int64_t t = (nvec << 2) + threadIdx.x;
  if (blockIdx.x == 0 && t < n) acc[t] = gacc_sum<MODE, SCALED>(gacc_load<MODE>(acc + t), src[t], scale);
}

extern "C" int hrp_grad_accumulate(const float* src, float* acc, int64_t n, int first, float scale, void* stream) {
  HRP_REQUIRE(src && acc && n > 0, "grad_accumulate: bad args");
  HRP_REQUIRE((uintptr_t)src % 16 == 0 && (uintptr_t)acc % 16 == 0, "grad_accumulate: src and acc must be 16-byte aligned");
  HRP_REQUIRE(src != acc, "grad_accumulate: src and acc are the same buffer");
  const int64_t nvec = n >> 2;
  const int64_t want = (nvec + 2 * GACC_THREADS - 1) / (2 * GACC_THREADS);
  const dim3 grid((unsigned)(want < 1 ? 1 : (want > GACC_MAX_BLOCKS ? GACC_MAX_BLOCKS : want))), block(GACC_THREADS);
  const hipStream_t st = (hipStream_t)stream;
  const bool scaled = scale != 1.f;
  if (first) {
    if (scaled) hipLaunchKernelGGL((grad_accumulate_kernel<0, true>), grid, block, 0, st, src, acc, n, scale);
    else hipLaunchKernelGGL((grad_accumulate_kernel<0, false>), grid, block, 0, st, src, acc, n, scale);
  } else {
    if (scaled) hipLaunchKernelGGL((grad_accumulate_kernel<1, true>), grid, block, 0, st, src, acc, n, scale);
    else hipLaunchKernelGGL((grad_accumulate_kernel<1, false>), grid, block, 0, st, src, acc, n, scale);
  }
  return check_launch("grad_accumulate");
}

extern "C" int hrp_avgpool_fwd(const void* x, int dtype, int N, int HW, int C, int pitch, float* out, int out_pitch, void* stream) {
  HRP_REQUIRE(x && out && N > 0 && HW > 0 && C > 0, "avgpool_fwd: bad args");
  dim3 grid(cdiv(C, 256), N);
  if (dtype == HRP_F32) hipLaunchKernelGGL(avgpool_fwd_kernel<float>, grid, dim3(256), 0, (hipStream_t)stream, x, HW, C, pitch, out, out_pitch);
  else hipLaunchKernelGGL(avgpool_fwd_kernel<bf16_t>, grid, dim3(256), 0, (hipStream_t)stream, x, HW, C, pitch, out, out_pitch);
  return check_launch("avgpool_fwd");
}
extern "C" int hrp_avgpool_bwd(const float* dout, int dout_pitch, void* dx, int dtype, int N, int HW, int C, int pitch, int accumulate, void* stream) {
  HRP_REQUIRE(dout && dx && N > 0 && HW > 0 && C > 0, "avgpool_bwd: bad args");
  dim3 grid(cdiv(C, 256), N);
  if (dtype == HRP_F32) hipLaunchKernelGGL(avgpool_bwd_kernel<float>, grid, dim3(256), 0, (hipStream_t)stream, dout, dout_pitch, dx, HW, C, pitch, accumulate);
  else hipLaunchKernelGGL(avgpool_bwd_kernel<bf16_t>, grid, dim3(256), 0, (hipStream_t)stream, dout, dout_pitch, dx, HW, C, pitch, accumulate);
  return check_launch("avgpool_bwd");
}

extern "C" int hrp_copy_cols(const float* src, int src_pitch, float* dst, int dst_pitch, int rows, int cols, int accumulate, void* stream) {
  HRP_REQUIRE(src && dst && rows > 0 && cols > 0, "copy_cols: bad args");
  hipLaunchKernelGGL(copy_cols_kernel, dim3(cdiv(rows * cols, 256)), dim3(256), 0, (hipStream_t)stream, src, src_pitch, dst, dst_pitch, rows, cols, accumulate);
  return check_launch("copy_cols");
}
extern "C" int hrp_copy_cols_batch(const hrp_copy_desc* descs, int n, void* stream) {
  HRP_REQUIRE(descs && n > 0 && n <= HRP_COPY_MAX, "copy_cols_batch: 1 .. %d problems (n=%d)", HRP_COPY_MAX, n);
  CopyBatchArgs a;
  size_t most = 0;
  for (int i = 0; i < n; ++i) {
    const hrp_copy_desc& d = descs[i];
    HRP_REQUIRE(d.dst && d.rows > 0 && d.cols > 0 && d.dst_pitch >= d.cols && (!d.src || d.src_pitch >= d.cols),
                "copy_cols_batch: problem %d: bad pointers / shape (rows=%d cols=%d pitches %d -> %d)", i, d.rows, d.cols, d.src_pitch, d.dst_pitch);
    HRP_REQUIRE(d.src || !d.accumulate, "copy_cols_batch: problem %d accumulates nothing (src == NULL)", i);
    a.d[i] = d;
    const size_t t = (size_t)d.rows * d.cols;
    most = t > most ? t : most;
  }
  const int gx = (int)(most >= 64 * 256 ? 64 : cdiv((int)most, 256));
  hipLaunchKernelGGL(copy_cols_batch_kernel, dim3(gx, n), dim3(256), 0, (hipStream_t)stream, a);
  return check_launch("copy_cols_batch");
}
extern "C" int hrp_scale_rows(float* x, int pitch, int rows, int cols, const float* row_scale, float s, void* stream) {
  HRP_REQUIRE(x && rows > 0 && cols > 0, "scale_rows: bad args");
  hipLaunchKernelGGL(scale_rows_kernel, dim3(cdiv(rows * cols, 256)), dim3(256), 0, (hipStream_t)stream, x, pitch, rows, cols, row_scale, s);
  return check_launch("scale_rows");
}
```

holistic-robot-pose-estimation_amd/optim.py:

```python
import ctypes as C

import torch

from . import _native as nv


class FusedClipAdam(torch.optim.Optimizer):
    def __init__(self, params, lr=1e-3, betas=(0.9, 0.999), eps=1e-8, max_norm=None, weight_decay=0.0, device_hyper=False):
        params = list(params)
        grouped = any(isinstance(p, dict) for p in params)
        if grouped:
            if not all(isinstance(p, dict) for p in params):
                raise ValueError("FusedClipAdam: either parameters or parameter-group dicts, not both")
            params = [dict(g, params=[p for p in g["params"] if p.requires_grad]) for g in params]
            params = [g for g in params if g["params"]]
        else:
            params = [p for p in params if p.requires_grad]
        if not params:
            raise ValueError("FusedClipAdam: no parameters")
        self._device_hyper = bool(grouped or device_hyper or weight_decay)
        super().__init__(params, dict(lr=float(lr), betas=(float(betas[0]), float(betas[1])), eps=float(eps),
                                      weight_decay=float(weight_decay) if self._device_hyper else 0, amsgrad=False,
                                      maximize=False, foreach=None, capturable=True, differentiable=False, fused=None))
        for g in self.param_groups:
            if g["amsgrad"] or g["maximize"]:
                raise ValueError("FusedClipAdam: amsgrad / maximize are not supported")
        self.params = [p for g in self.param_groups for p in g["params"]] if self._device_hyper else self.param_groups[0]["params"]
        dev = self.params[0].device
        if dev.type != "cuda":
            raise nv.HrpError("FusedClipAdam runs on an MI355X (gfx950) only; there is no CPU path")
        for p in self.params:
            if p.dtype != torch.float32 or not p.is_contiguous() or p.device != dev:
                raise ValueError("FusedClipAdam: parameters must be contiguous fp32 tensors on one device")
        self.device = dev
        self.max_norm = float(max_norm) if max_norm else 0.0
        total = sum((p.numel() + 3) // 4 * 4 for p in self.params)
        self._m = torch.zeros(total, dtype=torch.float32, device=dev)
        self._v = torch.zeros(total, dtype=torch.float32, device=dev)
        self.state_views, off = [], 0
        for p in self.params:
            n = p.numel()
            self.state_views.append((self._m[off:off + n].view_as(p), self._v[off:off + n].view_as(p)))
            off += (n + 3) // 4 * 4
        self.step_count = torch.zeros(1, dtype=torch.float32, device=dev)
        self._publish_state()
        self._slots = torch.zeros(8, dtype=torch.float32, device=dev)
        self._chunk_sums = None
        self._grad_ptrs = None
        self._tensors = self._chunks = None
        self._nchunks = 0
        if self._device_hyper:
            ng = len(self.param_groups)
            self._groups = torch.zeros(ng * C.sizeof(nv.OptGroup) // 4, dtype=torch.float32, device=dev)
            self._tensor_group = torch.tensor([i for i, g in enumerate(self.param_groups) for _ in g["params"]],
                                              dtype=torch.int32, device=dev)
            self._hyper_mirror = [None] * ng
            self.publish_hyper()

    def _hyper(self, g):
        return (float(g["lr"]), float(g["betas"][0]), float(g["betas"][1]), float(g["eps"]), float(g["weight_decay"]))

    def hyper_is_stale(self):
        return self._device_hyper and any(self._hyper(g) != m for g, m in zip(self.param_groups, self._hyper_mirror))

    def publish_hyper(self):
        if not self._device_hyper:
            return
        s = None
        for i, g in enumerate(self.param_groups):
            h = self._hyper(g)
            if h == self._hyper_mirror[i]:
                continue
            if s is None:
                if torch.cuda.is_current_stream_capturing():
                    raise RuntimeError("FusedClipAdam.publish_hyper() during a HIP graph capture: publish before the capture "
                                       "and after every replay")
                s = torch.cuda.current_stream(self.device).cuda_stream
            nv.call("hrp_opt_set_group", self._groups.data_ptr(), len(self.param_groups), i, *h, s)
            self._hyper_mirror[i] = h

    def _publish_state(self):
        for p, (m, v) in zip(self.params, self.state_views):
            self.state[p] = {"step": self.step_count.view(()), "exp_avg": m, "exp_avg_sq": v}

    def state_dict(self):
        sd = super().state_dict()
        sd["state"] = {k: dict(v, step=v["step"].clone()) for k, v in sd["state"].items()}
        return sd

    def load_state_dict(self, state_dict):
        if not self._device_hyper and len(state_dict["param_groups"]) != 1:
            raise ValueError("FusedClipAdam: one parameter group only")
        for g in state_dict["param_groups"]:
            if self._device_hyper:
                if g.get("amsgrad", False) or g.get("maximize", False):
                    raise ValueError("FusedClipAdam: amsgrad / maximize are not supported")
            elif g.get("weight_decay", 0) or g.get("amsgrad", False) or g.get("maximize", False):
                raise ValueError("FusedClipAdam: weight_decay / amsgrad / maximize are not supported")
        super().load_state_dict(state_dict)
        steps = set()
        with torch.no_grad():
            for p, (m, v) in zip(self.params, self.state_views):
                st = self.state.get(p)
                if not st:
                    m.zero_()
                    v.zero_()
                    continue
                m.copy_(st["exp_avg"])
                v.copy_(st["exp_avg_sq"])
                steps.add(float(st["step"]))
            if len(steps) > 1:
                raise ValueError(f"FusedClipAdam: parameters at different step counts {sorted(steps)}")
            self.step_count.fill_(steps.pop() if steps else 0.0)
        for g in self.param_groups:
            g["capturable"] = True
        self._publish_state()

    def _build_tables(self):
        ptrs = tuple(p.grad.data_ptr() for p in self.params)
        if ptrs == self._grad_ptrs:
            return
        tab = (nv.OptTensor * len(self.params))()
        chunks = []
        for i, (p, (m, v)) in enumerate(zip(self.params, self.state_views)):
            g = p.grad
            if g.dtype != torch.float32 or not g.is_contiguous():
                raise ValueError("FusedClipAdam: gradients must be contiguous fp32")
            tab[i].param, tab[i].grad, tab[i].exp_avg, tab[i].exp_avg_sq = p.data_ptr(), g.data_ptr(), m.data_ptr(), v.data_ptr()
            tab[i].numel = p.numel()
            chunks += [(i, k) for k in range((p.numel() + nv.OPT_CHUNK - 1) // nv.OPT_CHUNK)]
        ck = (nv.OptChunk * len(chunks))()
        for j, (i, k) in enumerate(chunks):
            ck[j].tensor, ck[j].offset = i, k
        self._tensors = torch.frombuffer(bytearray(bytes(tab)), dtype=torch.uint8).to(self.device)
        self._chunks = torch.frombuffer(bytearray(bytes(ck)), dtype=torch.uint8).to(self.device)
        self._nchunks = len(chunks)
        self._chunk_sums = torch.zeros(self._nchunks, dtype=torch.float32, device=self.device)
        self._grad_ptrs = ptrs

    def prepare(self):
        if any(p.grad is None for p in self.params):
            raise ValueError("FusedClipAdam: every parameter needs a gradient (run one backward first)")
        self._build_tables()

    @torch.no_grad()
    def step(self, closure=None):
        if closure is not None:
            raise ValueError("FusedClipAdam: closures are not supported")
        if self._device_hyper:
            if not torch.cuda.is_current_stream_capturing():
                self.publish_hyper()
            elif self.hyper_is_stale():
                raise RuntimeError("FusedClipAdam: param_groups changed since the device table was written and a HIP graph is being "
                                   "captured; call publish_hyper() before the capture (and after every replay)")
        self.prepare()
        g = self.param_groups[0]
        s = torch.cuda.current_stream(self.device).cuda_stream
        self.step_count += 1
        if self.max_norm > 0:
            nv.call("hrp_opt_grad_sumsq", self._tensors.data_ptr(), self._chunks.data_ptr(), self._nchunks,
                    self._slots.data_ptr(), self._chunk_sums.data_ptr(), s)
        if self._device_hyper:
            nv.call("hrp_opt_adam_step_groups", self._tensors.data_ptr(), self._chunks.data_ptr(), self._nchunks,
                    self._slots.data_ptr(), self.max_norm, self.step_count.data_ptr(),
                    self._groups.data_ptr(), len(self.param_groups), self._tensor_group.data_ptr(), s)
        else:
            nv.call("hrp_opt_adam_step", self._tensors.data_ptr(), self._chunks.data_ptr(), self._nchunks,
                    self._slots.data_ptr(), self.max_norm, self.step_count.data_ptr(),
                    float(g["lr"]), float(g["betas"][0]), float(g["betas"][1]), float(g["eps"]), s)
        from .plan import bump_param_epoch
        bump_param_epoch()

    def total_norm(self):
        return self._slots.sum().sqrt()

    def zero_grad(self, set_to_none=False):
        for p in self.params:
            if p.grad is not None:
                if set_to_none:
                    p.grad = None
                else:
                    p.grad.zero_()
```

holistic-robot-pose-estimation_amd/plan.py:

```python
import collections
import contextlib
import ctypes as C
import math
import os

import torch

from . import _native as nv
from . import conv_geometry as G
from .conv_geometry import rup as _rup

BN_EPS = 1e-5
STAT_SLOTS = 8


def _dt(dtype):
    return nv.HRP_F32 if dtype == torch.float32 else nv.HRP_BF16


def _cdt(plan, dtype):
    if dtype == torch.float32:
        return nv.HRP_F32X3 if plan.x3 else nv.HRP_F32
    return nv.HRP_BF16


class TensorH:

    def __init__(self, plan, N, H, W, Cc, dtype, buf=None, offset=0, pitch=None, base=None):
        self.plan, self.N, self.H, self.W, self.C, self.dtype = plan, N, H, W, Cc, dtype
        self.pitch = pitch if pitch is not None else _rup(Cc, 8)
        self.offset = offset
        self.base = base
        if buf is None:
            buf = torch.zeros(N * H * W * self.pitch, dtype=dtype, device=plan.device)
            plan.keep.append(buf)
        self.buf = buf
        self._grad = None
        self.grad_written = False
        self.requires_grad = False
        self.stats = None
        self.producer = None
        self.lane_path = plan.lane_path
        self._grad_paths = []
        self.n_readers = self.n_bn_readers = 0

    @property
    def esz(self):
        return self.buf.element_size()

    def ptr(self):
        return self.buf.data_ptr() + self.offset * self.esz

    def grad_buf(self):
        root = self.base if self.base is not None else self
        if root._grad is None:
            root._grad = torch.zeros_like(root.buf)
            self.plan.keep.append(root._grad)
        return root._grad

    def gptr(self):
        return self.grad_buf().data_ptr() + self.offset * self.esz

    def operand(self, grad=False):
        return G.Operand(self.gptr() if grad else self.ptr(), self.N, self.H, self.W, self.C, self.pitch)

    def take_grad_slot(self):
        acc = self.grad_written
        self.grad_written = True
        self.grad_buf()
        root = self.base if self.base is not None else self
        root.grad_written = True
        self.plan.grad_owner[self.gptr()] = root
        here = self.plan.lane_path
        if any(lanes_concurrent(here, q) for q in root._grad_paths):
            raise RuntimeError("plan: a gradient is accumulated from two concurrent lanes")
        root._grad_paths.append(here)
        return 1 if acc else 0

    def check_readable(self):
        if lanes_concurrent(self.plan.lane_path, self.lane_path):
            raise RuntimeError("plan: a tensor is consumed in a lane concurrent with its producer")
        self.materialize()
        self.n_readers += 1

    def materialize(self):
        op = getattr(self, "pending_input", None)
        if op is not None:
            self.pending_input = None
            self.plan.pending_inputs.remove(self)
            self.lane_path = self.plan.lane_path
            self.plan.fwd.append(op)
        pend = getattr(self, "pending_block_end", None)
        if pend is not None:
            self.pending_block_end = None
            self.plan.fwd.append(pend["launch"])
            if self in self.plan.pending_block_ends:
                self.plan.pending_block_ends.remove(self)

    def view4(self):
        return self.buf.view(self.N, self.H, self.W, self.pitch)[..., :self.C]


class Term:

    def __init__(self, t, bn=None, up=1):
        self.t, self.bn, self.up = t, bn, up


class ParamW:

    def __init__(self, param, cout, cin, ntaps):
        self.param, self.cout, self.cin, self.ntaps = param, cout, cin, ntaps
        self.fwd_off = self.bwd_off = None
        self.pad_t = 0
        self.t_ntaps = set()
        self.grad_written = False
        self.first_use = None
        self.src = None


SERIAL_LANES = bool(os.environ.get("HRP_SERIAL_LANES"))

MAX_LANE_DEPTH = 1

PLAN_MODE = os.environ.get("HRP_PLAN_MODE", "hybrid")
BATCHING = True
WGRAD_DEFER = True
WGRAD_FOLD_EVERY = 32
WGRAD_SINK = int(os.environ.get("HRP_WGRAD_SINK", "16"))
PARITY_PAD = True
PARITY_FUSE = os.environ.get("HRP_PARITY_FUSE", "1") not in ("0", "")
ROWCONV_FUSE = True
BLOCK_END_FUSE = True
BLOCK_END_FWD_FUSE = os.environ.get("HRP_BLOCK_END_FWD", "1") not in ("0", "")
BLOCK_FUSE = os.environ.get("HRP_BLOCK_FUSE", "1") not in ("0", "")
BNECK_TAIL_FUSE = os.environ.get("HRP_TAIL_FUSE", "1") not in ("0", "")
POOL_FUSE_GRADS = os.environ.get("HRP_POOL_FUSE", "0") not in ("0", "")
LAZY_INPUTS = os.environ.get("HRP_LAZY_INPUTS", "1") not in ("0", "")
PLAN_STATS = bool(os.environ.get("HRP_PLAN_STATS"))
DBG_SYNC = os.environ.get("HRP_DBG_SYNC")

MAX_TILE_DILATION = 4

PARAM_EPOCH = 0
_PLAN_SERIAL = 0


def bump_param_epoch():
    global PARAM_EPOCH
    PARAM_EPOCH += 1


Entry = collections.namedtuple("Entry", "lane path op")


class _OpList(list):

    def __init__(self, plan):
        super().__init__()
        self.plan = plan

    def append(self, op):
        list.append(self, Entry(self.plan.cur_lane, self.plan.lane_path, op))


FAMILIES = {"conv": (nv.BATCH_CONV, "hrp_conv2d_fwd", nv.ConvDesc),
            "wgrad": (nv.BATCH_WGRAD, "hrp_conv2d_bwd_weight", nv.WgradDesc),
            "ew_fwd": (nv.BATCH_EW_FWD, "hrp_ew_fwd", nv.EwDesc),
            "ew_red": (nv.BATCH_EW_BWD_REDUCE, "hrp_ew_bwd_reduce", nv.EwBwdDesc),
            "ew_app": (nv.BATCH_EW_BWD_APPLY, "hrp_ew_bwd_apply", nv.EwBwdDesc),
            "wgrad_fold": (nv.BATCH_WGRAD_FOLD, None, nv.WgradFoldDesc)}
PARITY_KEY = ("conv", nv.HRP_BF16, "parity")


class LaunchOp:
    __slots__ = ()
    fam = None

    def launches(self):
        return [self]

    def merge_key(self):
        return None

    def set_ws(self, regions):
        for it, (ws, nbytes) in zip(self.launches(), regions):
            it.desc.workspace, it.desc.workspace_bytes = ws, nbytes


def is_fam(op, *fams):
    return isinstance(op, LaunchOp) and op.fam in fams


def marker_kind(e):
    return e.op.kind if e.lane is None else None


class Launch(LaunchOp):
    __slots__ = ("fam", "desc")

    def __init__(self, fam, desc):
        self.fam, self.desc = fam, desc

    def __call__(self, s):
        nv.call(FAMILIES[self.fam][1], C.byref(self.desc), s)

    def ws_need(self, alone=True):
        return [int(nv.lib().hrp_wgrad_workspace_bytes(C.byref(self.desc)))]

    def fold_desc(self):
        f = nv.WgradFoldDesc()
        nv.check(nv.lib().hrp_wgrad_fold_desc_of(C.byref(self.desc), C.byref(f)), "hrp_wgrad_fold_desc_of")
        return f

    def fold_descs(self):
        return [self.fold_desc()]

    def merge_key(self):
        d = self.desc
        esz = 2 if d.dtype == nv.HRP_BF16 else 4
        if self.fam == "conv":
            if d.ntaps not in (1, 2, 4, 9) or (d.Cin * esz) % 32 or (d.dtype != nv.HRP_BF16 and d.H == 1 and d.W == 1 and d.Cin >= 512):
                return None
            if d.ntaps == 1 and nv.lib().hrp_conv_pointwise(C.byref(d)):
                return None
            if PARITY_FUSE and d.out_stride == 2 and nv.lib().hrp_conv_parity_fusable(C.byref(d)):
                return PARITY_KEY
            return ("conv", d.dtype, d.ntaps)
        if self.fam == "wgrad":
            return ("wgrad", d.dtype, d.ntaps, d.reserved)
        if d.C % (16 // esz):
            return None
        return (self.fam, d.dtype)

    def written(self):
        d = self.desc
        if self.fam == "conv":
            main = d.y + ((d.out_off_y * d.y_W + d.out_off_x) * d.y_pitch if d.out_stride > 1 else 0)
            return tuple(a for a in (main, d.pro_side, d.pro_side2) if a)
        if self.fam in ("wgrad", "wgrad_fold"):
            return (d.dw + 4 * d.dw_tap_off,)
        if self.fam == "ew_fwd":
            return (d.out,)
        if self.fam == "ew_red":
            return (d.sums,)
        return tuple(x for x in (d.din, d.din2) if x)


class BatchLaunch(LaunchOp):

    def __init__(self, plan, items):
        self.plan, self.items = plan, list(items)
        self.fam = items[0].fam
        self.info, self.table, self.singles, self.folds = None, None, False, None

    def launches(self):
        return self.items

    def merge_key(self):
        return self.items[0].merge_key()

    def ws_need(self, alone=True):
        n = len(self.items)
        arr = (nv.WgradDesc * n)(*[it.desc for it in self.items])
        info = nv.BatchInfo()
        nv.check(nv.lib().hrp_batch_prepare(nv.BATCH_WGRAD, arr, n, None, C.byref(info)), "hrp_batch_prepare")
        return [max(int(info.ws_bytes[i]), it.ws_need()[0] if alone else 0) for i, it in enumerate(self.items)]

    def prepare(self):
        famid, _, dtype = FAMILIES[self.fam]
        n = len(self.items)
        arr = (dtype * n)(*[it.desc for it in self.items])
        info = nv.BatchInfo()
        nbytes = int(nv.lib().hrp_batch_table_bytes(famid, n))
        host = (C.c_char * nbytes)()
        fuse = nv.lib().hrp_conv_parity_fuse_enable(1 if PARITY_FUSE else 0)
        try:
            nv.check(nv.lib().hrp_batch_prepare(famid, arr, n, host, C.byref(info)), "hrp_batch_prepare")
        except nv.HrpError:
            if self.fam == "wgrad_fold":
                raise
            if PLAN_STATS:
                import sys
                print(f"plan: batch of {n} {self.fam} launches runs one by one ({nv.lib().hrp_last_error().decode()})", file=sys.stderr)
            self.singles = True
            return
        finally:
            nv.lib().hrp_conv_parity_fuse_enable(fuse)
        self.info = info
        if self.fam == "wgrad" and self.items[0].desc.phase == 1:
            folds = (nv.WgradFoldDesc * n)()
            nv.check(nv.lib().hrp_batch_wgrad_fold_descs(host, C.byref(info), folds), "hrp_batch_wgrad_fold_descs")
            self.folds = list(folds)
        self.table = self.plan.upload(host)

    def fold_descs(self):
        if not self.singles:
            return self.folds
        return [it.fold_desc() for it in self.items]

    def __call__(self, s):
        if self.singles:
            for it in self.items:
                it(s)
        else:
            nv.call_batch(self, s)


class BlockLaunch(LaunchOp):
    fam = "block"

    def __init__(self, desc):
        self.desc = desc
        self._single = None

    def merge_key(self):
        return ("block",)

    def written(self):
        return (self.desc.conv2.y,)

    def __call__(self, s):
        if self._single is None:
            self._single = BlockBatch(None, [self])
        self._single(s)


class BlockBatch(LaunchOp):
    fam = "block"

    def __init__(self, plan, items):
        self.plan, self.items = plan, sorted(items, key=lambda it: it.desc.conv1.Cin)
        self.info, self.table = None, None

    def launches(self):
        return self.items

    def prepare(self):
        n = len(self.items)
        arr = (nv.BlockDesc * n)(*[it.desc for it in self.items])
        self.info = nv.BlockInfo()
        self.table = (C.c_char * int(nv.lib().hrp_block_table_bytes()))()
        nv.check(nv.lib().hrp_block_prepare(arr, n, self.table, C.byref(self.info)), "hrp_block_prepare")

    def __call__(self, s):
        if self.table is None:
            self.prepare()
        nv.call_block(self, s)


def _pair_block(plan, ops):
    items = [l for op in ops for l in op.launches()]
    c32 = [it for it in items if it.desc.conv1.Cin == 32]
    c64 = [it for it in items if it.desc.conv1.Cin != 32]
    out = []
    while c32 and c64:
        out.append(BlockBatch(plan, [c32.pop(0), c64.pop(0)]))
    out += [BlockBatch(plan, [it]) for it in c32 + c64]
    return out


def _merge_ops(plan, ops):
    items = [l for op in ops for l in op.launches()]
    step = 4 if ops[0].merge_key() == PARITY_KEY and len(items) % 4 == 0 else 1
    out, cur, seen = [], [], set()
    for i in range(0, len(items), step):
        unit = items[i:i + step]
        w = [a for it in unit for a in it.written()]
        if len(cur) + step > nv.BATCH_MAX or any(a in seen for a in w):
            out.append(cur)
            cur, seen = [], set()
        cur += unit
        seen.update(w)
    out.append(cur)
    return [g[0] if len(g) == 1 else BatchLaunch(plan, g) for g in out]


class _Seq:
    def __init__(self):
        self.items, self.blocks = [], {}


class _Par:
    def __init__(self):
        self.lanes = {}


class _LaneSync:

    def __init__(self, kind, parent, children):
        self.kind, self.parent, self.children = kind, parent, children

    def run(self, streams):
        for c in self.children:
            if self.kind == "fork":
                streams[c].wait_stream(streams[self.parent])
            else:
                streams[self.parent].wait_stream(streams[c])


class _PackJoin:
    kind = "pack_join"

    def __init__(self, plan):
        self.plan = plan

    def run(self, streams):
        if self.plan._pack_stream is not None:
            streams[0].wait_stream(self.plan._pack_stream)

    def __call__(self, s):
        if self.plan._pack_stream is not None and not SERIAL_LANES:
            torch.cuda.current_stream(self.plan.device).wait_stream(self.plan._pack_stream)


def lanes_concurrent(a, b):
    for (ba, la), (bb, lb) in zip(a, b):
        if ba != bb:
            return False
        if la != lb:
            return True
    return False


class GradAccumulation:

    def __init__(self, steps, average):
        self.steps = steps
        self.scale = 1.0 / steps if average else 1.0
        self.index = 0
        self.buf, self.views, self._key = None, {}, None

    def begin(self):
        self.index = 0

    def complete(self):
        return self.index >= self.steps

    def bind(self, plan):
        key = (str(plan.device), plan.grad_arena.numel(), tuple((id(p), off) for p, (off, _) in zip(plan._grad_params, plan._grad_layout)))
        if key == self._key:
            return
        if self.index:
            raise RuntimeError("gradient accumulation: the set of trainable parameters changed in the middle of a cycle "
                               "(this plan lays its gradient arena out differently); call begin_accumulation() first")
        self.buf = torch.zeros_like(plan.grad_arena)
        self.views = {}
        for p, (off, n) in zip(plan._grad_params, plan._grad_layout):
            v = self.buf[off:off + n].view(p.shape)
            v._hrp_plan_grad = True
            self.views[id(p)] = v
        self._key = key

    def accumulate(self, plan, stream):
        self.bind(plan)
        if self.index >= self.steps:
            raise RuntimeError(f"gradient accumulation: {self.steps} micro-batches are already in the buffer "
                               f"(set_grad_accumulation(steps={self.steps})); call begin_accumulation() to start the next cycle")
        nv.call("hrp_grad_accumulate", plan.grad_arena.data_ptr(), self.buf.data_ptr(), plan.grad_arena.numel(),
                1 if self.index == 0 else 0, self.scale, stream)
        self.index += 1


class Plan:
    def __init__(self, device, dtype, training, need_grad):
        self.device, self.dtype, self.training, self.need_grad = device, dtype, training, need_grad
        self.x3 = False
        self.keep = []
        self.cur_lane, self.lane_path, self.n_lanes = 0, (), 1
        self._lane_ids, self._n_blocks, self._side_streams = {}, 0, []
        self.fwd, self.bwd = _OpList(self), _OpList(self)
        self.weights = {}
        self.weight_list = []
        self.bn_train = []
        self.bn_fold = {}
        self.bn_fold_hat = {}
        self.bn_bwd = []
        self.stats_floats = 0
        self.bsums_floats = 0
        self.param_grads = {}
        self.inputs, self.outputs = {}, {}
        self.dyn = {}
        self.built = False
        self._versions = None
        self._late = []
        self.out_handles = []
        self.grad_arena = None
        self._grad_views = {}
        self._grad_layout = []
        self._grad_params = []
        self.accum = None
        self.bwd_split, self.split_active = None, False
        self.bwd_cuts = None
        self.pre_pack = []
        self.tracked_params = []
        self.counters = {}
        self.wgrad_ws_bytes = {}
        self.wgrad_ws = {}
        self.merged, self.fwd_run, self.bwd_run = False, [], []
        self._block_lanes = {}
        self._rng, self.n_dropout = None, 0
        self.linear_grad_written = set()
        self.grad_owner = {}
        self.reg_chains = []
        self.pending_inputs = []
        self.pending_block_ends = []
        self.row_last_writer = {}

    def new(self, N, H, W, Cc, dtype=None, pitch=None):
        return TensorH(self, N, H, W, Cc, dtype or self.dtype, pitch=pitch)

    def weight(self, param, cout, cin, ntaps):
        w = self.weights.get(id(param))
        if w is None:
            w = ParamW(param, cout, cin, ntaps)
            self.weights[id(param)] = w
            self.weight_list.append(w)
        if w.first_use is None:
            w.first_use = len(self.fwd)
        return w

    def preallocate_param_grads(self, params):
        params = [p for p in params if p.requires_grad]
        params = [p for p in params if p.dim() > 1] + [p for p in params if p.dim() <= 1]
        total = sum(_rup(p.numel(), 4) for p in params)
        self.grad_arena = torch.zeros(max(total, 4), dtype=torch.float32, device=self.device)
        off = 0
        self._grad_layout = []
        self._grad_params = params
        for p in params:
            self._grad_views[id(p)] = self.grad_arena[off:off + p.numel()].view(p.shape)
            self._grad_views[id(p)]._hrp_plan_grad = True
            self._grad_layout.append((off, p.numel()))
            off += _rup(p.numel(), 4)

    def grad_of_param(self, p):
        e = self.param_grads.get(id(p))
        if e is None:
            g = self._grad_views.get(id(p))
            if g is None:
                g = torch.zeros_like(p, dtype=torch.float32)
            e = (p, g)
            self.param_grads[id(p)] = e
            self.keep.append(e[1])
        return e[1]

    def rng_state(self):
        if self._rng is None:
            global _PLAN_SERIAL
            _PLAN_SERIAL += 1
            rank = torch.distributed.get_rank() if (torch.distributed.is_available() and torch.distributed.is_initialized()) else 0
            seed = (int(torch.initial_seed()) ^ (rank << 48) ^ (_PLAN_SERIAL << 32)) & 0x7FFFFFFFFFFFFFFF
            self._rng = torch.tensor([seed, 0], dtype=torch.int64, device=self.device)
            self.keep.append(self._rng)
        return self._rng

    def alloc_stats(self, Cc):
        off = self.stats_floats
        self.stats_floats += 2 * Cc * STAT_SLOTS
        return off

    def alloc_bsums(self, Cc):
        off = self.bsums_floats
        self.bsums_floats += 2 * Cc * STAT_SLOTS
        return off

    def finalize(self):
        dev = self.device
        self.stats = torch.zeros(max(self.stats_floats, 2), dtype=torch.float64, device=dev)
        self.bsums = torch.zeros(max(self.bsums_floats, 2), dtype=torch.float64, device=dev)
        cut = self._late_pack_cut()
        self._layout_packed_weights(cut)
        self._pack_stream = None
        self._arena_clean = False
        if self._pack_tables_late:
            self._pack_stream = torch.cuda.Stream(device=dev)
            list.insert(self.fwd, cut, Entry(None, (), _PackJoin(self)))
        self.merged = PLAN_MODE in ("merged", "hybrid")
        if not self.merged:
            self.wgrad_ws = {lane: torch.zeros(max(nb // 4, 4), dtype=torch.float32, device=dev)
                             for lane, nb in self.wgrad_ws_bytes.items()}
        for fn in self._late:
            fn()
        self._late = []
        if self.need_grad:
            passes.fuse_bn_reduce(self)
        if self.merged:
            self.fwd_run, self.bwd_run = passes.flatten(self, self.fwd), passes.flatten(self, self.bwd)
            if WGRAD_SINK > 1 and WGRAD_DEFER and BATCHING:
                self.bwd_run = passes.sink_wgrads(self, self.bwd_run)
            if passes.assign_wgrad_scratch(self):
                self.bwd_run = passes.insert_folds(self, self.bwd_run)
            used = {e.lane for e in self.fwd_run + self.bwd_run if e.lane is not None}
            self._side_streams = [torch.cuda.Stream(device=dev) if (i + 1) in used else None for i in range(self.n_lanes - 1)]
        else:
            self._side_streams = [torch.cuda.Stream(device=dev) for _ in range(self.n_lanes - 1)]
        self._bn_tables()
        self.built = True
        if PLAN_STATS:
            self._print_stats()

    def _layout_packed_weights(self, cut):
        self._pack_tables, self._pack_tables_late = [], []
        for w in self.weight_list:
            assert all(t == w.ntaps + w.pad_t for t in w.t_ntaps), f"plan: data gradients of one weight disagree on its tap slots ({w.t_ntaps}, pad_t {w.pad_t})"
        for dtype in (torch.float32, torch.bfloat16):
            ws = [w for w in self.weight_list if w.dtype == dtype]
            if not ws:
                continue
            esz = G.ELEM[_dt(dtype)][0]
            ck = 32 // esz
            total = 0
            for w in ws:
                nf = math.ceil(w.cin_used / ck) * w.ntaps * _rup(w.cout, 32) * ck
                w.fwd_off = total
                total += _rup(nf, 64)
                w.max_elems = nf
                if w.need_t:
                    nb = math.ceil(w.cout / ck) * (w.ntaps + w.pad_t) * _rup(w.cin_used, 32) * ck
                    w.bwd_off = total
                    total += _rup(nb, 64)
                    w.max_elems = max(nf, nb)
            arena = torch.zeros(total, dtype=dtype, device=self.device)
            self.keep.append(arena)
            for w in ws:
                w.arena = arena
            early = [w for w in ws if cut is None or w.first_use is None or w.first_use < cut]
            late = [w for w in ws if not (cut is None or w.first_use is None or w.first_use < cut)]
            for group, dest in ((early, self._pack_tables), (late, self._pack_tables_late)):
                if not group:
                    continue
                tab = (nv.PackEntry * len(group))()
                for i, w in enumerate(group):
                    tab[i].src = (w.src if w.src is not None else w.param).data_ptr()
                    tab[i].dst = arena.data_ptr() + w.fwd_off * esz
                    tab[i].dst_t = (arena.data_ptr() + w.bwd_off * esz) if w.need_t else None
                    tab[i].Cout, tab[i].Cin, tab[i].ntaps, tab[i].pad_t = w.cout, w.cin, w.ntaps, w.pad_t
                tdev = self.upload(tab)
                cdt = _cdt(self, dtype)
                first = [0]
                for w in group:
                    first.append(first[-1] + nv.lib().hrp_pack_blocks(w.cout, w.cin, w.ntaps, cdt, 1, 1 if w.need_t else 0))
                fdev = torch.tensor(first, dtype=torch.int32, device=self.device)
                self.keep.append(fdev)
                dest.append((tdev, fdev, len(group), first[-1], cdt))

    def _print_stats(self):
        import sys
        msg = f"plan: {len(self.fwd)} forward / {len(self.bwd)} backward ops, {self.n_lanes} lanes, {self.counters}"
        if self.merged:
            ops = [e.op for e in self.fwd_run + self.bwd_run if e.lane is not None]
            nb = sum(isinstance(op, BatchLaunch) and not op.singles for op in ops)
            msg += (f"; {PLAN_MODE}: {sum(e.lane is not None for e in self.fwd_run)} / {sum(e.lane is not None for e in self.bwd_run)}"
                    f" launches, {nb} of them batched, streams {sorted({e.lane for e in self.fwd_run if e.lane is not None})}")
        print(msg, file=sys.stderr)

    def upload(self, cobj, dtype=torch.uint8):
        t = torch.frombuffer(bytearray(bytes(cobj)), dtype=dtype).to(self.device)
        self.keep.append(t)
        return t

    def analyze_backward_split(self, min_frac=0.55, fracs=None):
        return passes.analyze_backward_split(self, min_frac, fracs)

    def _late_pack_cut(self):
        if not self.need_grad or len(self.weight_list) < 64:
            return None
        joins = [i for i, e in enumerate(self.fwd) if marker_kind(e) == "join"]
        forks = [i for i, e in enumerate(self.fwd) if marker_kind(e) == "fork"]
        if len(forks) < 2 or not joins or forks[1] < joins[0]:
            return None
        return joins[0] + 1

    def patch_wgrad_ws(self, g, lane):
        if lane in self.wgrad_ws:
            g.workspace, g.workspace_bytes = self.wgrad_ws[lane].data_ptr(), self.wgrad_ws[lane].numel() * 4

    def late(self, fn):
        self._late.append(fn)

    def late_weight(self, w, *descs, transposed=False, field="w"):
        def patch():
            for d in descs:
                setattr(d, field, w.arena.data_ptr() + (w.bwd_off if transposed else w.fwd_off) * G.ELEM[_dt(w.dtype)][0])
        self.late(patch)

    def _table(self, entries):
        tab = (nv.BnEntry * len(entries))()
        for i, e in enumerate(entries):
            for k, v in e.items():
                setattr(tab[i], k, v)
        return self.upload(tab), len(entries)

    def _bn_tables(self):
        self._run_tab = self._fold_tab = self._pgrad_tab = None
        if self.bn_train:
            ents = []
            for bn, off, count in self.bn_train:
                ents.append(dict(stats=self.stats.data_ptr() + 8 * off, a=bn.running_mean.data_ptr(),
                                 b=bn.running_var.data_ptr(), counter=bn.num_batches_tracked.data_ptr(),
                                 C=bn.num_features, count=float(count), momentum=bn.momentum, eps=bn.eps))
            self._run_tab = self._table(ents)
        if self.bn_fold:
            ents = []
            for bn, sc, sh in self.bn_fold.values():
                ents.append(dict(a=bn.weight.data_ptr(), b=bn.bias.data_ptr(), c=bn.running_mean.data_ptr(),
                                 d=bn.running_var.data_ptr(), out_scale=sc.data_ptr(), out_shift=sh.data_ptr(),
                                 C=bn.num_features, eps=bn.eps))
            if self.bn_fold_hat:
                cmax = max(bn.num_features for bn, _, _ in self.bn_fold_hat.values())
                ones, zeros = torch.ones(cmax, device=self.device), torch.zeros(cmax, device=self.device)
                self.keep += [ones, zeros]
                for bn, inv, nmi in self.bn_fold_hat.values():
                    ents.append(dict(a=ones.data_ptr(), b=zeros.data_ptr(), c=bn.running_mean.data_ptr(),
                                     d=bn.running_var.data_ptr(), out_scale=inv.data_ptr(), out_shift=nmi.data_ptr(),
                                     C=bn.num_features, eps=bn.eps))
            self._fold_tab = self._table(ents)
        if self.bn_bwd:
            ents = []
            for bn, off in self.bn_bwd:
                ents.append(dict(stats=self.bsums.data_ptr() + 8 * off, a=self.grad_of_param(bn.weight).data_ptr(),
                                 b=self.grad_of_param(bn.bias).data_ptr(), C=bn.num_features, accumulate=0))
            self._pgrad_tab = self._table(ents)

    def _stream(self):
        return torch.cuda.current_stream(self.device).cuda_stream

    def params_dirty(self):
        v = tuple(w.param._version for w in self.weight_list) + tuple(t._version for t in self.tracked_params) + \
            tuple(t._version for bn, _, _ in self.bn_fold.values() for t in (bn.weight, bn.bias, bn.running_mean, bn.running_var)) + \
            (PARAM_EPOCH,)
        if v != self._versions:
            self._versions = v
            return True
        return False

    def run_prep(self, force=False):
        if not (force or self.params_dirty()):
            return
        s = self._stream()
        for op in self.pre_pack:
            op(s)
        late_s = s
        if self._pack_stream is not None and not SERIAL_LANES:
            self._pack_stream.wait_stream(torch.cuda.current_stream(self.device))
            late_s = self._pack_stream.cuda_stream
        for tdev, fdev, n, nblk, dt in self._pack_tables_late:
            nv.call("hrp_pack_weights_compact", tdev.data_ptr(), fdev.data_ptr(), n, nblk, dt, late_s)
        if late_s != s and self.need_grad and self.grad_arena is not None:
            with torch.cuda.stream(self._pack_stream):
                self.grad_arena.zero_()
            self._arena_clean = True
        for tdev, fdev, n, nblk, dt in self._pack_tables:
            nv.call("hrp_pack_weights_compact", tdev.data_ptr(), fdev.data_ptr(), n, nblk, dt, s)
        if self._fold_tab:
            nv.call("hrp_bn_fold", self._fold_tab[0].data_ptr(), self._fold_tab[1], s)

    def lane_id(self, parent, index):
        key = (parent, index)
        if key not in self._lane_ids:
            self._lane_ids[key] = self.n_lanes
            self.n_lanes += 1
        return self._lane_ids[key]

    def _run_list(self, ops):
        if SERIAL_LANES:
            h = self._stream()
            for lane, _, op in ops:
                if lane is not None:
                    op(h)
            return
        streams = [torch.cuda.current_stream(self.device)] + self._side_streams
        handles = [st.cuda_stream if st is not None else None for st in streams]
        dbg = DBG_SYNC
        for lane, _, op in ops:
            if lane is None:
                op.run(streams)
                if dbg:
                    torch.cuda.synchronize(self.device)
            else:
                if dbg == "pre1" and lane == 1:
                    torch.cuda.synchronize(self.device)
                op(handles[lane])
                if dbg == "all" or (dbg == "lane1" and lane == 1) or (dbg == "lane0" and lane == 0):
                    torch.cuda.synchronize(self.device)
                elif dbg == "s1" and lane == 1:
                    streams[1].synchronize()

    def fwd_ops(self):
        return self.fwd_run if self.merged else self.fwd

    def bwd_ops(self):
        return self.bwd_run if self.merged else self.bwd

    def run_forward(self):
        global PARAM_EPOCH
        s = self._stream()
        if self._rng is not None:
            nv.call("hrp_rng_advance", self._rng.data_ptr(), s)
        if self.training and self._run_tab:
            PARAM_EPOCH += 1
        if self.stats_floats:
            self.stats.zero_()
        self._run_list(self.fwd_ops())
        if self._run_tab:
            nv.call("hrp_bn_running_update", self._run_tab[0].data_ptr(), self._run_tab[1], s)

    def run_backward(self, part=None):
        s = self._stream()
        cuts = self.bwd_cuts if self.bwd_cuts else ([self.bwd_split] if self.bwd_split is not None else [])
        if part == "first":
            part = ("seg", 0)
        if part == "rest":
            assert len(cuts) == 1, "run_backward('rest') is the two-segment form"
            part = ("seg", 1)
        j = None if part is None else part[1]
        if j in (None, 0):
            if self.grad_arena is not None and not self._arena_clean:
                self.grad_arena.zero_()
            self._arena_clean = False
            if self.bsums_floats:
                self.bsums.zero_()
        ops = self.bwd_ops()
        if j is None:
            self._run_list(ops)
        else:
            lo = 0 if j == 0 else cuts[j - 1]
            hi = cuts[j] if j < len(cuts) else None
            self._run_list(list.__getitem__(ops, slice(lo, hi)))
        if (j is None or j == len(cuts)) and self._pgrad_tab:
            nv.call("hrp_bn_param_grad", self._pgrad_tab[0].data_ptr(), self._pgrad_tab[1], s)


    def publish_param_grads(self):
        if self.accum is not None:
            views = self.accum.views
            for p, g in self.param_grads.values():
                t = views.get(id(p))
                if t is None:
                    raise RuntimeError("gradient accumulation: a parameter of this plan has no slot in the gradient arena")
                if p.grad is None or p.grad is t or getattr(p.grad, "_hrp_plan_grad", False):
                    p.grad = t
                else:
                    raise RuntimeError("gradient accumulation: a parameter carries a foreign .grad tensor (not a plan's); "
                                       "set it to None first - adding the running sum onto it would count micro-batches twice")
            return
        for p, g in self.param_grads.values():
            if p.grad is None or p.grad is g or getattr(p.grad, "_hrp_plan_grad", False):
                p.grad = g
            else:
                p.grad.add_(g)


class _BwdStack(list):

    def __init__(self, plan):
        super().__init__()
        self.plan = plan

    def append(self, fn):
        list.append(self, (self.plan.cur_lane, self.plan.lane_path, fn))


class _Parallel:
    def __init__(self, pb, block, lanes):
        self.pb, self.block, self.lanes = pb, block, lanes

    @contextlib.contextmanager
    def lane(self, i):
        p = self.pb.plan
        saved = (p.cur_lane, p.lane_path)
        p.cur_lane, p.lane_path = self.lanes[i], saved[1] + ((self.block, i),)
        try:
            yield
        finally:
            p.cur_lane, p.lane_path = saved


from .plan_blocks import BlockOps
from .plan_heads import HeadOps
from . import plan_passes as passes


class PlanBuilder(BlockOps, HeadOps):
    def __init__(self, plan):
        self.plan = plan
        self.bwd_stack = _BwdStack(plan)
        self.fuse_inference = (not plan.training) and (not plan.need_grad)

    def image_input(self, name, N, Cc, H, W, u8=False, dtype=None, lazy=False):
        p = self.plan
        t = p.new(N, H, W, Cc, dtype)
        dt = _dt(t.dtype)

        def op(s):
            x = p.dyn[name]
            if u8:
                assert x.dtype == torch.uint8
                nv.call("hrp_u8_nchw_to_nhwc", x.data_ptr(), t.ptr(), dt, N, Cc, H, W, t.pitch, 255.0, 0, s)
            else:
                nv.call("hrp_nchw_to_nhwc", x.data_ptr(), t.ptr(), dt, N, Cc, H, W, t.pitch, s)
        if lazy and LAZY_INPUTS:
            t.pending_input = op
            p.pending_inputs.append(t)
        else:
            p.fwd.append(op)
        t.external = name
        return t

    def image_input_s2d(self, name, N, Cc, H, W, u8=False):
        p = self.plan
        t = p.new(N, (H + 1) // 2, (W + 1) // 2, 4 * Cc, pitch=_rup(4 * Cc, 16))
        dt = _dt(t.dtype)

        def op(s):
            x = p.dyn[name]
            if u8:
                assert x.dtype == torch.uint8
                nv.call("hrp_u8_nchw_to_nhwc", x.data_ptr(), t.ptr(), dt, N, Cc, H, W, t.pitch, 255.0, 1, s)
            else:
                nv.call("hrp_nchw_to_nhwc_s2d", x.data_ptr(), t.ptr(), dt, N, Cc, H, W, t.pitch, s)
        p.fwd.append(op)
        t.external = name
        return t

    def stem7x7_s2d(self, xs, weight, want_stats=False):
        p = self.plan
        cout, cin = weight.shape[0], weight.shape[1]
        assert tuple(weight.shape[2:]) == (7, 7) and xs.C == 4 * cin
        dev, dtype = p.device, xs.dtype
        idx_w, idx_g = (torch.from_numpy(m).to(dev) for m in G.stem_index_maps(cout, cin))
        w12 = torch.zeros(cout, 4 * cin, 4, 4, dtype=torch.float32, device=dev)
        gw12 = torch.zeros(cout, 4 * cin, 16, dtype=torch.float32, device=dev)
        p.keep += [idx_w, idx_g, w12, gw12]
        p.pre_pack.append(lambda s: nv.call("hrp_gather_f32", weight.data_ptr(), idx_w.data_ptr(), w12.data_ptr(),
                                            w12.numel(), 0, s))
        w = ParamW(weight, cout, 4 * cin, 16)
        w.first_use = len(p.fwd)
        w.src, w.dtype, w.cin_used, w.need_t = w12, dtype, 4 * cin, False
        p.weights[("s2d", id(weight))] = w
        p.weight_list.append(w)
        y = p.new(xs.N, xs.H, xs.W, cout, dtype)
        y.requires_grad = p.need_grad
        d = self._conv_desc(G.stem_s2d(xs.H, xs.W), xs.operand(), y.operand(), dtype)
        if want_stats:
            y.stats = p.alloc_stats(cout)
        self._launch_fwd(d, w, y)
        y.producer = ("conv", d)
        if p.need_grad and weight.requires_grad:
            def bw():
                if not y.grad_written:
                    return
                self._emit_wgrad(G.wgrad_groups(G.TAPS4_STEM, 1), xs.operand(), y.operand(grad=True), w, dtype, scratch=gw12)
                gp = p.grad_of_param(weight)
                acc = 1 if p.grad_arena is not None else 0
                p.bwd.append(lambda s: nv.call("hrp_gather_f32", gw12.data_ptr(), idx_g.data_ptr(), gp.data_ptr(),
                                               gp.numel(), acc, s))
            self.bwd_stack.append(bw)
        return y

    def maxpool3x3s2(self, x):
        p = self.plan
        x.check_readable()
        Ho, Wo = (x.H - 1) // 2 + 1, (x.W - 1) // 2 + 1
        y = p.new(x.N, Ho, Wo, x.C, x.dtype)
        y.requires_grad = p.need_grad and x.requires_grad
        arg = None
        if y.requires_grad:
            arg = torch.zeros(x.N * Ho * Wo * x.C, dtype=torch.uint8, device=p.device)
            p.keep.append(arg)
        p.fwd.append(lambda s: nv.call("hrp_maxpool3x3s2_fwd", x.ptr(), _dt(x.dtype), x.N, x.H, x.W, x.C, x.pitch, y.ptr(),
                                       y.pitch, arg.data_ptr() if arg is not None else None, s))
        if y.requires_grad:
            def bw():
                if not y.grad_written:
                    return
                acc = x.take_grad_slot()
                p.bwd.append(lambda s: nv.call("hrp_maxpool3x3s2_bwd", y.gptr(), y.pitch, arg.data_ptr(), x.gptr(), _dt(x.dtype),
                                               x.N, x.H, x.W, x.C, x.pitch, acc, s))
            self.bwd_stack.append(bw)
        return y

    def deconv4x4s2(self, x, weight, want_stats=False):
        p = self.plan
        x.check_readable()
        cin_t, cout_t = weight.shape[0], weight.shape[1]
        assert tuple(weight.shape[2:]) == (4, 4) and x.C == cin_t
        dtype = x.dtype
        w = p.weight(weight, cin_t, cout_t, 16)
        w.dtype, w.cin_used, w.need_t = dtype, cout_t, True
        y = p.new(x.N, 2 * x.H, 2 * x.W, cout_t, dtype)
        y.requires_grad = p.need_grad
        if want_stats:
            y.stats = p.alloc_stats(cout_t)
        for geo in G.deconv4x4s2_forward(x.H, x.W):
            d = self._conv_desc(geo, x.operand(), y.operand(), dtype)
            self._launch_fwd(d, w, y, transposed=True)
        if p.need_grad:
            self.bwd_stack.append(lambda: self._deconv_bwd(x, w, y, dtype))
        return y

    def _deconv_bwd(self, x, w, y, dtype):
        p = self.plan
        if not y.grad_written:
            return
        if w.param.requires_grad:
            self._emit_wgrad(G.wgrad_groups(G.TAPS4_DECONV, 2), y.operand(grad=True), x.operand(), w, dtype)
        if x.requires_grad:
            acc = x.take_grad_slot()
            d = self._conv_desc(G.deconv4x4s2_data_grad(x.H, x.W), y.operand(grad=True), x.operand(grad=True), dtype,
                                res=(x.gptr(), x.pitch) if acc else None)
            p.late_weight(w, d)
            p.bwd.append(Launch("conv", d))

    def constant(self, N, Cc, value):
        t = self.plan.new(N, 1, 1, Cc, torch.float32, pitch=Cc)
        t.buf.fill_(value)
        return t

    def vector_input(self, name, N, Cc, dense=False):
        p = self.plan
        t = p.new(N, 1, 1, Cc, torch.float32, pitch=Cc if dense else None)

        grp = getattr(self, "_vec_group", None)
        if grp is None or grp["at"] != len(p.fwd) or grp["lane"] != p.lane_path or len(grp["items"]) >= nv.COPY_MAX:
            grp = self._vec_group = dict(items=[], lane=p.lane_path)
            items = grp["items"]
            p.fwd.append(lambda s: nv.copy_cols_batch([(p.dyn[n_].data_ptr(), c_, t_.ptr(), t_.pitch, r_, c_, 0) for n_, r_, c_, t_ in items], s))
            grp["at"] = len(p.fwd)
        grp["items"].append((name, N, Cc, t))
        return t

    def nchw_output(self, t):
        dt = _dt(t.dtype)
        holder = {}
        p = self.plan
        t.materialize()

        def op(s):
            out = torch.empty(t.N, t.C, t.H, t.W, dtype=torch.float32, device=p.device)
            nv.call("hrp_nhwc_to_nchw", t.ptr(), out.data_ptr(), dt, t.N, t.C, t.H, t.W, t.pitch, s)
            holder["out"] = out
        p.fwd.append(op)
        return holder

    def pil_resize_input(self, name, N, H, W, scale=0.5, mean=(0.485, 0.456, 0.406), std=(0.229, 0.224, 0.225)):
        p = self.plan
        Ho, Wo = int(H * scale), int(W * scale)
        if Ho % 2 or Wo % 2:
            raise nv.HrpError(f"pil_resize_input: the resized image {Ho} x {Wo} (image {H} x {W}, scale {scale}) must have even sides: "
                              "it is written straight into the ResNet stem's 2 x 2 space-to-depth layout")
        t = p.new(N, Ho // 2, Wo // 2, 12, pitch=16)
        tabs = []
        for n_in, n_out in ((W, Wo), (H, Ho)):
            host = (C.c_int32 * (n_out * (nv.PIL_KMAX + 2)))()
            nv.check(nv.lib().hrp_pil_resize_table(n_in, n_out, host), "hrp_pil_resize_table")
            tabs.append(p.upload(host, torch.int32))
        m3, s3 = (C.c_float * 3)(*mean), (C.c_float * 3)(*std)
        dt = _dt(t.dtype)
# ... 395 lines not shown
```

holistic-robot-pose-estimation_amd/runtime.py:

```python
import os

import torch
import torch.nn as nn

from . import _native as nv
from .plan import GradAccumulation, Plan, PlanBuilder, _dt


def require_gpu(device):
    if device.type != "cuda":
        raise nv.HrpError("hrpe_amd runs on an MI355X (gfx950) only: tensors must live on a HIP device; "
                          "there is no CPU path")
    nv.lib()


GRAPH_CACHE = not os.environ.get("HRP_NO_MODULE_GRAPH")
PLAN_CACHE_MAX = int(os.environ.get("HRP_PLAN_CACHE", "6"))
GRAPH_WARMUP = 2


class Runner:

    def __init__(self, plan, in_names, outs, img_inputs):
        self.plan, self.in_names, self.outs, self.img_inputs = plan, in_names, outs, img_inputs
        self.calls = self.bwd_calls = 0
        self.g_fwd = self.g_bwd = self.static_in = None
        self.graph_failed = False

    def _forward_launches(self, prep=True):
        p = self.plan
        if prep or p.need_grad:
            p.run_prep(force=p.need_grad)
        p.run_forward()

    def _results(self):
        p = self.plan
        res = [None] * len(self.outs)
        dense = [(i, h, shape) for i, (kind, h, shape) in enumerate(self.outs) if kind != "nchw" and h.dtype == torch.float32]
        if len(dense) > 1:
            flat = torch.empty(sum(h.N * h.C for _, h, _ in dense), dtype=torch.float32, device=p.device)
            items, off = [], 0
            for i, h, shape in dense:
                items.append((h.ptr(), h.pitch, flat.data_ptr() + 4 * off, h.C, h.N, h.C, 0))
                res[i] = flat[off:off + h.N * h.C].view(shape)
                off += h.N * h.C
            nv.copy_cols_batch(items, torch.cuda.current_stream(p.device).cuda_stream)
        for i, (kind, h, shape) in enumerate(self.outs):
            if res[i] is not None:
                continue
            if kind == "nchw":
                res[i] = h["out"].clone() if self.g_fwd is not None else h["out"]
            else:
                res[i] = h.buf.view(-1)[h.offset: h.offset + h.N * h.pitch].view(h.N, h.pitch)[:, : h.C].reshape(shape).clone()
        return tuple(res)

    def _graphs_allowed(self):
        p = self.plan
        return (GRAPH_CACHE and not self.graph_failed and not p.split_active and not torch.cuda.is_current_stream_capturing()
                and not nv.profiling())

    def _capture(self, what):
        p = self.plan
        try:
            g = torch.cuda.CUDAGraph()
            pool = self.g_fwd.pool() if self.g_fwd is not None else None
            with torch.cuda.graph(g, pool=pool, capture_error_mode="thread_local"):
                if what == "fwd":
                    self._forward_launches(prep=False)
                else:
                    p._arena_clean = False
                    p.run_backward(None)
            return g
        except Exception as e:
            import sys
            print(f"hrpe_amd: graph capture of the {what} plan failed ({e!r}); running it eagerly", file=sys.stderr)
            self.graph_failed = True
            return None

    def forward(self, tensors):
        p = self.plan
        self.calls += 1
        if self._graphs_allowed() and self.calls > GRAPH_WARMUP:
            if self.g_fwd is None:
                self.static_in = [torch.empty_like(t) for t in tensors]
                for n, st in zip(self.in_names, self.static_in):
                    p.dyn[n] = st
                self.g_fwd = self._capture("fwd")
            if self.g_fwd is not None and p.need_grad and self.g_bwd is None and self.bwd_calls >= GRAPH_WARMUP:
                self.g_bwd = self._capture("bwd")
        if self.g_fwd is not None and self._graphs_allowed():
            for st, t in zip(self.static_in, tensors):
                st.copy_(t)
            if not p.need_grad:
                p.run_prep(force=False)
            self.g_fwd.replay()
            if p.training and p._run_tab:
                from .plan import bump_param_epoch
                bump_param_epoch()
            return self._results()
        for n, t in zip(self.in_names, tensors):
            p.dyn[n] = t
        self._forward_launches()
        return self._results()

    def backward(self, grads):
        p = self.plan
        s = torch.cuda.current_stream(p.device).cuda_stream
        items, keep = [], []
        for (kind, h, shape), g in zip(self.outs, grads):
            t = h["handle"] if kind == "nchw" else h
            if not (t.requires_grad and t.grad_written):
                continue
            gb = t.grad_buf()
            if kind != "nchw" and t.dtype == torch.float32:
                if g is not None:
                    g = g.reshape(t.N, t.C)
                    if g.dtype != torch.float32 or not g.is_contiguous():
                        g = g.contiguous().float()
                    keep.append(g)
                items.append((None if g is None else g.data_ptr(), t.C, t.gptr(), t.pitch, t.N, t.C, 0))
            elif g is None:
                gb.zero_()
            elif kind == "nchw":
                g = g.contiguous().float()
                nv.call("hrp_nchw_to_nhwc", g.data_ptr(), t.gptr(), _dt(t.dtype), t.N, t.C, t.H, t.W, t.pitch, s)
            else:
                gb.view(t.N, t.pitch)[:, : t.C].copy_(g.reshape(t.N, t.C))
        if items:
            nv.copy_cols_batch(items, s)
        self.bwd_calls += 1
        if self.g_bwd is not None and self._graphs_allowed():
            self.g_bwd.replay()
        else:
            p.run_backward("first" if p.split_active else None)
        if p.accum is not None:
            p.accum.accumulate(p, s)
        p.publish_param_grads()
        gin = []
        for n in self.in_names:
            t = self.img_inputs.get(n)
            if t is not None and t.requires_grad and t.grad_written:
                out = torch.empty(t.N, t.C, t.H, t.W, dtype=torch.float32, device=p.device)
                nv.call("hrp_nhwc_to_nchw", t.gptr(), out.data_ptr(), _dt(t.dtype), t.N, t.C, t.H, t.W, t.pitch, s)
                gin.append(out)
            else:
                gin.append(None)
        return gin


class _PlanFn(torch.autograd.Function):
    @staticmethod
    def forward(ctx, runner, anchor, *tensors):
        ctx.runner = runner
        ctx.n = len(tensors)
        outs = runner.forward(tensors)
        return outs

    @staticmethod
    def backward(ctx, *grads):
        gin = ctx.runner.backward(grads)
        return (None, None) + tuple(gin)


MODE_EPOCH = [0]


class PlannedModule(nn.Module):

    def train(self, mode=True):
        MODE_EPOCH[0] += 1
        return super().train(mode)

    def __init__(self):
        super().__init__()
        object.__setattr__(self, "_plans", {})
        object.__setattr__(self, "_bn_sig", (-1, []))
        object.__setattr__(self, "_compute_dtype", torch.float32)
        object.__setattr__(self, "_x3", False)
        object.__setattr__(self, "_accum", None)
        object.__setattr__(self, "_plan_mode", None)

    def _select_plans(self, mode):
        object.__setattr__(self, "_plan_mode", mode)

    def set_compute_dtype(self, dtype):
        x3 = dtype == "fp32x3"
        if x3:
            dtype = torch.float32
        assert dtype in (torch.float32, torch.bfloat16)
        for m in self.modules():
            if isinstance(m, PlannedModule):
                object.__setattr__(m, "_compute_dtype", dtype)
                object.__setattr__(m, "_x3", x3)
                m._plans.clear()
        return self

    @property
    def compute_dtype(self):
        return self._compute_dtype

    def flat_grads(self):
        if self._accum is not None:
            return [self._accum.buf] if self._accum.buf is not None else []
        return [r.plan.grad_arena for r in self._plans.values() if r.plan.grad_arena is not None]

    def set_grad_accumulation(self, steps, average=False):
        if isinstance(steps, bool) or not isinstance(steps, int) or steps < 1:
            raise ValueError(f"set_grad_accumulation: steps must be an integer >= 1 (got {steps!r})")
        mods = [m for m in self.modules() if isinstance(m, PlannedModule)]
        if steps > 1 and any(r.plan.split_active for m in mods for r in m._plans.values()):
            raise ValueError("set_grad_accumulation(steps > 1) cannot be combined with enable_split_backward(): the overlapped "
                             "all-reduce hands out arena ranges of a single backward; call disable_split_backward() first")
        for m in mods:
            acc = GradAccumulation(steps, bool(average)) if steps > 1 else None
            object.__setattr__(m, "_accum", acc)
            for r in m._plans.values():
                r.plan.accum = acc if r.plan.need_grad else None
        return self

    def begin_accumulation(self):
        for m in self.modules():
            if isinstance(m, PlannedModule) and m._accum is not None:
                m._accum.begin()
        return self

    def accumulation_complete(self):
        return self._accum is None or self._accum.complete()

    def enable_split_backward(self, min_frac=0.55, fracs=None):
        if self._accum is not None:
            raise ValueError("enable_split_backward() cannot be combined with set_grad_accumulation(steps > 1): the ranges it hands "
                             "out are final for ONE backward, not for the accumulated sum; call set_grad_accumulation(1) first")
        runners = [r for r in self._plans.values() if r.plan.grad_arena is not None]
        if len(runners) != 1:
            return None
        plan = runners[0].plan
        if fracs is not None:
            cuts = plan.analyze_backward_split(fracs=fracs)
            if not cuts:
                return None
            plan.bwd_cuts, plan.bwd_split = [c for c, _ in cuts], None
            plan.split_active = True
            return plan, [r for _, r in cuts]
        info = plan.analyze_backward_split(min_frac)
        if info is None:
            return None
        plan.bwd_split, ranges = info
        plan.bwd_cuts = None
        plan.split_active = True
        return plan, ranges

    def check_split_backward(self, ranges):
        runners = [r for r in self._plans.values() if r.plan.grad_arena is not None and r.plan.split_active]
        if len(runners) != 1:
            raise RuntimeError("check_split_backward: no plan with an active split")
        plan = runners[0].plan
        arena = plan.grad_arena
        multi = plan.bwd_cuts is not None
        groups = ranges if multi else [ranges]
        nseg = len(plan.bwd_cuts) + 1 if multi else 2
        snaps = []
        ok = True
        for j in range(1, nseg):
            torch.cuda.synchronize(arena.device)
            grp = groups[j - 1]
            snaps.append((grp, torch.cat([arena[o:o + n] for o, n in grp]).clone() if grp else arena[:0].clone()))
            plan.run_backward(("seg", j))
            torch.cuda.synchronize(arena.device)
            for grp_, before in snaps:
                after = torch.cat([arena[o:o + n] for o, n in grp_]) if grp_ else arena[:0]
                ok = ok and torch.equal(before, after)
        ok = ok and bool(torch.isfinite(arena).all())
        if not ok:
            self.disable_split_backward()
            raise RuntimeError("split backward self-check failed: a later part of the backward touched gradient ranges "
                               "that were final after an earlier one")
        return True

    def disable_split_backward(self):
        for r in self._plans.values():
            r.plan.split_active = False

    def invalidate_plans(self):
        for m in self.modules():
            if isinstance(m, PlannedModule):
                m._plans.clear()
                if m._accum is not None:
                    object.__setattr__(m, "_accum", GradAccumulation(m._accum.steps, m._accum.scale != 1.0))

    def _apply(self, fn, *a, **k):
        r = super()._apply(fn, *a, **k)
        self.invalidate_plans()
        return r

    def load_state_dict(self, *a, **k):
        r = super().load_state_dict(*a, **k)
        for m in self.modules():
            if isinstance(m, PlannedModule):
                for pl in m._plans.values():
                    pl.plan._versions = None
        return r

    def _frozen_bn_signature(self):
        if self._bn_sig[0] != MODE_EPOCH[0]:
            object.__setattr__(self, "_bn_sig", (MODE_EPOCH[0], [m for m in self.modules() if hasattr(m, "running_mean")]))
        sig = 0
        if self.training:
            for i, m in enumerate(self._bn_sig[1]):
                if not m.training:
                    sig |= 1 << i
        return sig

    def _run(self, *tensors):
        dev = tensors[0].device
        require_gpu(dev)
        need_grad = torch.is_grad_enabled() and (any(p.requires_grad for p in self.parameters())
                                                 or any(t.requires_grad for t in tensors))
        bn_eval = self._frozen_bn_signature()
        key = (tuple(tuple(t.shape) for t in tensors), self._compute_dtype, self.training, need_grad,
               tuple(bool(t.requires_grad) for t in tensors) if need_grad else (),
               tuple(t.dtype == torch.uint8 for t in tensors), bn_eval, self._x3, self._plan_mode)
        runner = self._plans.pop(key, None)
        if runner is not None:
            self._plans[key] = runner
        if runner is None:
            while len(self._plans) >= PLAN_CACHE_MAX:
                self._plans.pop(next(iter(self._plans)))
            plan = Plan(dev, self._compute_dtype, self.training, need_grad)
            plan.x3 = bool(self._x3)
            if need_grad:
                plan.preallocate_param_grads(list(self.parameters()))
                plan.accum = self._accum
            pb = PlanBuilder(plan)
            in_names, outs, img_inputs = self._build(pb, *tensors)
            for kind, h, shape in outs:
                t = h["handle"] if kind == "nchw" else h
                pb.output(t)
            pb.finish()
            runner = Runner(plan, in_names, outs, img_inputs)
            self._plans[key] = runner
        tensors = tuple(t.contiguous() if t.dtype == torch.uint8 else
                        (t.contiguous().float() if t.dtype != torch.float32 or not t.is_contiguous() else t)
                        for t in tensors)
        if need_grad:
            anchor = next((p for p in self.parameters() if p.requires_grad), None)
            if anchor is None:
                anchor = tensors[0]
            return _PlanFn.apply(runner, anchor, *tensors)
        return runner.forward(tensors)


class SingleTensorModule(PlannedModule):

    def forward(self, x):
        return self._run(x)[0]

    def _build(self, pb, x):
        N, Cc, H, W = x.shape
        t = pb.image_input("x", N, Cc, H, W, u8=x.dtype == torch.uint8)
        t.requires_grad = pb.plan.need_grad and x.requires_grad
        y = self.emit(pb, t)
        holder = pb.nchw_output(y)
        holder["handle"] = y
        return ["x"], [("nchw", holder, None)], {"x": t}
```

include/hrp.h:

```cpp
#ifndef HRP_H
#define HRP_H

#include <stddef.h>
#include <stdint.h>

#ifdef __cplusplus
extern "C" {
#endif

typedef enum { HRP_F32 = 0, HRP_BF16 = 1, HRP_F32X3 = 2 } hrp_dtype;

typedef enum {
  HRP_OK = 0,
  HRP_ERR_ARG = -1,
  HRP_ERR_LAUNCH = -2,
  HRP_ERR_NODEV = -3
} hrp_status;

#define HRP_MAX_TAPS 16

#define HRP_STAT_SLOTS 8

typedef struct hrp_conv_desc {
  const void* x;
  const void* w;
  void* y;
  const void* res;
  const float* bias;
  const float* scale;
  const float* shift;
  double* stats;
  int32_t dtype;
  int32_t N, H, W, Cin, x_pitch;
  int32_t Ho, Wo, Cout;
  int32_t y_H, y_W, y_pitch, res_pitch;
  int32_t out_stride, out_off_y, out_off_x;
  int32_t in_stride;
  int32_t ntaps;
  int32_t dy[HRP_MAX_TAPS], dx[HRP_MAX_TAPS];
  int32_t wtap[HRP_MAX_TAPS];
  int32_t w_ntaps;
  int32_t w_cout_pad;
  int32_t relu;
  const void* bnb_x;
  const uint8_t* bnb_mask;
  const float* bnb_consts;
  int32_t bnb_x_pitch, bnb_mask_pitch;
  const double* bnb_stats;
  const float* bnb_gamma;
  const float* bnb_beta;
  float bnb_count, bnb_eps;
  int32_t pro_mode, pro_reserved;
  const void* pro_x2;
  const double* pro_stats;
  const double* pro_bsums;
  const float* pro_gamma;
  const float* pro_beta;
  float pro_count, pro_eps;
  void* pro_side;
  const uint8_t* pro_mask;
  void* pro_side2;
  int32_t pro_side2_acc, pro_reserved2;
  const uint8_t* res_mask;
  int32_t tail_mode, tail_side_acc;
  const double* tail_stats;
  const double* tail_bsums;
  const float* tail_gamma;
  const float* tail_beta;
  float tail_count, tail_eps;
  uint8_t* tail_mask;
  const void* tail_g;
  void* tail_side;
  const void* tail_x2;
  const void* tail_w2;
  const double* tail_stats2;
  const float* tail_gamma2;
  const float* tail_beta2;
} hrp_conv_desc;

typedef struct hrp_wgrad_desc {
  const void* x;
  const void* dy;
  float* dw;
  int32_t dtype;
  int32_t N, H, W, Cin, x_pitch;
  int32_t Ho, Wo, Cout, dy_pitch;
  int32_t in_stride, ntaps;
  int32_t dy_t[HRP_MAX_TAPS], dx_t[HRP_MAX_TAPS];
  int32_t dw_cin;
  int32_t dw_tap_stride;
  int32_t dw_tap_off;
  int32_t accumulate;
  void* workspace;
  int64_t workspace_bytes;
  int32_t phase;
  int32_t reserved;
} hrp_wgrad_desc;

typedef struct hrp_wgrad_fold_desc {
  const float* workspace;
  float* dw;
  int32_t G, pairs, n_cib, nte, nb;
  int32_t Cout, dw_cin, ntaps, dw_tap_stride, dw_tap_off, accumulate;
  int32_t reserved;
} hrp_wgrad_fold_desc;

typedef struct hrp_pack_entry {
  const float* src;
  void* dst;
  void* dst_t;
  int32_t Cout, Cin, ntaps;
  int32_t pad_t;
} hrp_pack_entry;

#define HRP_EW_MAX_IN 4
typedef enum { HRP_EW_IDENTITY = 0, HRP_EW_AFFINE = 1, HRP_EW_BN_TRAIN = 2 } hrp_ew_mode;

typedef struct hrp_ew_input {
  const void* ptr;
  int32_t pitch;
  int32_t up;
  int32_t mode;
  const float* a;
  const float* b;
  const double* stats;
  float count;
  float eps;
} hrp_ew_input;

typedef struct hrp_ew_desc {
  hrp_ew_input in[HRP_EW_MAX_IN];
  int32_t nin;
  void* out;
  int32_t out_pitch;
  int32_t dtype;
  int32_t N, H, W, C;
  int32_t relu;
  uint8_t* mask;
  int32_t mask_pitch;
  float* consts_out;
} hrp_ew_desc;

typedef struct hrp_ew_bwd_desc {
  const void* dout;
  const void* out;
  int32_t dout_pitch, out_pitch;
  hrp_ew_input in;
  void* din;
  int32_t din_pitch;
  double* sums;
  int32_t dtype;
  int32_t N, H, W, C;
  int32_t relu;
  int32_t accumulate;
  const uint8_t* mask;
  int32_t mask_pitch;
  void* din2;
  int32_t din2_pitch;
  int32_t accumulate2;
  const float* pooled;
} hrp_ew_bwd_desc;

typedef struct hrp_bn_entry {
  const double* stats;
  float* a;
  float* b;
  const float* c;
  const float* d;
  float* out_scale;
  float* out_shift;
  int64_t* counter;
  int32_t C;
  float count, momentum, eps;
  int32_t accumulate;
} hrp_bn_entry;

#define HRP_FK_MAX_JOINTS 32
#define HRP_FK_MAX_KP 24
typedef struct hrp_fk_chain {
  int32_t njoints;
  int32_t parent[HRP_FK_MAX_JOINTS];
  int32_t type[HRP_FK_MAX_JOINTS];
  int32_t cfg[HRP_FK_MAX_JOINTS];
  float mimic_mul[HRP_FK_MAX_JOINTS], mimic_off[HRP_FK_MAX_JOINTS];
  float origin[HRP_FK_MAX_JOINTS][12];
  float axis[HRP_FK_MAX_JOINTS][3];
  int32_t nkp;
  int32_t kp_frame[HRP_FK_MAX_KP];
  float kp_offset[HRP_FK_MAX_KP][3];
  int32_t dof;
} hrp_fk_chain;

const char* hrp_last_error(void);
int hrp_version(void);
const char* hrp_source_hash(void);
int hrp_device_ok(void);

int hrp_nchw_to_nhwc(const float* src, void* dst, int dtype, int N, int C, int H, int W, int dst_pitch, void* stream);
int hrp_nhwc_to_nchw(const void* src, float* dst, int dtype, int N, int C, int H, int W, int src_pitch, void* stream);
int hrp_nchw_grad_from_nhwc(const void* src, float* dst, int dtype, int N, int C, int H, int W, int src_pitch, void* stream);
int hrp_u8_nchw_to_nhwc(const uint8_t* src, void* dst, int dtype, int N, int C, int H, int W, int dst_pitch,
                        float divisor, int s2d, void* stream);
int hrp_pack_weights(const hrp_pack_entry* table_dev, int count, int dtype, int max_elems, void* stream);
int hrp_pack_blocks(int Cout, int Cin, int ntaps, int dtype, int has_dst, int has_dst_t);
int hrp_pack_weights_compact(const hrp_pack_entry* table_dev, const int32_t* first_block_dev, int count, int total_blocks,
                             int dtype, void* stream);
int hrp_nchw_to_nhwc_s2d(const float* src, void* dst, int dtype, int N, int C, int H, int W, int dst_pitch, void* stream);
int hrp_gather_f32(const float* src, const int32_t* idx, float* dst, int n, int accumulate, void* stream);
int hrp_fill_zero(void* p, int64_t bytes, void* stream);
int hrp_maxpool3x3s2_fwd(const void* x, int dtype, int N, int H, int W, int C, int pitch, void* y, int y_pitch,
                         uint8_t* argmax, void* stream);
int hrp_maxpool3x3s2_bwd(const void* dy, int dy_pitch, const uint8_t* argmax, void* dx, int dtype, int N, int H, int W,
                         int C, int pitch, int accumulate, void* stream);

int hrp_conv2d_fwd(const hrp_conv_desc* d, void* stream);
int hrp_conv_rowstrip_channels(const hrp_conv_desc* d);
int hrp_conv_pointwise(const hrp_conv_desc* d);
int hrp_conv_parity_fusable(const hrp_conv_desc* d);
int hrp_conv_parity_fuse_enable(int on);
int hrp_conv_tile_config(const hrp_conv_desc* d);
int hrp_conv2d_bwd_weight(const hrp_wgrad_desc* d, void* stream);
int64_t hrp_wgrad_workspace_bytes(const hrp_wgrad_desc* d);
int64_t hrp_colsum_workspace_bytes(int64_t rows, int C);
int hrp_colsum(const void* x, int dtype, int64_t rows, int C, int pitch, float* out, int accumulate, void* workspace,
               int64_t workspace_bytes, void* stream);

#define HRP_OPT_CHUNK 4096
typedef struct hrp_opt_tensor {
  float* param;
  float* grad;
  float* exp_avg;
  float* exp_avg_sq;
  int64_t numel;
} hrp_opt_tensor;
typedef struct hrp_opt_chunk {
  int32_t tensor;
  int32_t offset;
} hrp_opt_chunk;
int hrp_opt_grad_sumsq(const hrp_opt_tensor* tensors_dev, const hrp_opt_chunk* chunks_dev, int nchunks,
                       float* sumsq_slots, float* chunk_sums, void* stream);
int hrp_opt_adam_step(const hrp_opt_tensor* tensors_dev, const hrp_opt_chunk* chunks_dev, int nchunks,
                      const float* sumsq_slots, float max_norm, const float* step_dev,
                      float lr, float beta1, float beta2, float eps, void* stream);
typedef struct hrp_opt_group {
  float lr, beta1, beta2, eps;
  float weight_decay;
  float reserved[3];
} hrp_opt_group;
int hrp_opt_adam_step_groups(const hrp_opt_tensor* tensors_dev, const hrp_opt_chunk* chunks_dev, int nchunks,
                             const float* sumsq_slots, float max_norm, const float* step_dev,
                             const hrp_opt_group* groups_dev, int ngroups, const int32_t* tensor_group_dev, void* stream);
int hrp_opt_set_group(hrp_opt_group* groups_dev, int ngroups, int index, float lr, float beta1, float beta2, float eps,
                      float weight_decay, void* stream);
int hrp_grad_accumulate(const float* src, float* acc, int64_t n, int first, float scale, void* stream);

int hrp_ew_fwd(const hrp_ew_desc* d, void* stream);
int hrp_ew_bwd_reduce(const hrp_ew_bwd_desc* d, void* stream);
int hrp_ew_pool2(const void* src, int src_dtype, int src_pitch, const uint8_t* mask, int mask_pitch, int N, int H, int W, int C, float* dst,
                 void* stream);
int hrp_ew_bwd_apply(const hrp_ew_bwd_desc* d, void* stream);

typedef enum {
  HRP_BATCH_CONV = 0, HRP_BATCH_WGRAD = 1, HRP_BATCH_EW_FWD = 2, HRP_BATCH_EW_BWD_REDUCE = 3, HRP_BATCH_EW_BWD_APPLY = 4,
  HRP_BATCH_WGRAD_FOLD = 5
} hrp_batch_family;
#define HRP_BATCH_MAX 32
typedef struct hrp_batch_info {
  int32_t family, n, dtype;
  int32_t variant;
  int32_t grid, lds_bytes;
  int32_t grid2;
  int32_t grid3, lds_bytes3;
  int32_t blk0[HRP_BATCH_MAX + 1];
  int32_t blk2[HRP_BATCH_MAX + 1];
  int64_t ws_bytes[HRP_BATCH_MAX];
} hrp_batch_info;
int64_t hrp_batch_table_bytes(int family, int n);
int hrp_batch_prepare(int family, const void* descs, int n, void* table_host, hrp_batch_info* info);
int hrp_batch_launch(const void* table_dev, const hrp_batch_info* info, void* stream);
int hrp_batch_conv_parity_configs(const void* table_host, const hrp_batch_info* info, int32_t* out);
int hrp_wgrad_fold_desc_of(const hrp_wgrad_desc* d, hrp_wgrad_fold_desc* out);
int hrp_batch_wgrad_fold_descs(const void* table_host, const hrp_batch_info* info, hrp_wgrad_fold_desc* out);
typedef enum { HRP_WGRAD_FOUR_WAVE = 0, HRP_WGRAD_EIGHT_WAVE_BF16 = 1, HRP_WGRAD_EIGHT_WAVE_F32X3 = 2 } hrp_wgrad_program;
typedef struct hrp_wgrad_config {
  int32_t program;
  int32_t arrange;
  int32_t nks, BM;
  int32_t TI, TH, TW;
  int32_t ring, xmode;
  int32_t G, ntiles;
  int32_t pairs;
  int32_t use_ws;
  int32_t reserved[3];
} hrp_wgrad_config;
int hrp_wgrad_config_of(const hrp_wgrad_desc* d, hrp_wgrad_config* out);
int hrp_batch_wgrad_configs(const void* table_host, const hrp_batch_info* info, hrp_wgrad_config* out);

#define HRP_PIL_KMAX 12
int hrp_pil_resize_table(int in_size, int out_size, int32_t* out);
int hrp_pil_resize_normalize(const void* src, int src_u8, int N, int H, int W, const int32_t* xtab_dev, const int32_t* ytab_dev,
                             int Ho, int Wo, void* dst, int dtype, int dst_pitch, int s2d, const float* mean3, const float* std3,
                             void* stream);
int hrp_broadcast_hw(const float* src, int src_pitch, void* dst, int dtype, int N, int HW, int C, int dst_pitch, void* stream);
int hrp_bilinear_nhwc_to_nchw(const void* src, int dtype, int N, int h, int w, int C, int pitch, float* dst, int H, int W, int act,
                              void* stream);

#define HRP_BLOCK_MAX 2
typedef struct hrp_block_desc {
  hrp_conv_desc conv1, conv2;
} hrp_block_desc;
typedef struct hrp_block_info {
  int32_t n, grid, lds_bytes, reserved;
  int32_t first_wg[HRP_BLOCK_MAX];
  int32_t bands[HRP_BLOCK_MAX];
} hrp_block_info;
int hrp_block_channels(const hrp_block_desc* d);
int64_t hrp_block_table_bytes(void);
int hrp_block_prepare(const hrp_block_desc* descs, int n, void* table, hrp_block_info* info);
int hrp_block_launch(const void* table, const hrp_block_info* info, void* stream);

int hrp_bn_running_update(const hrp_bn_entry* table_dev, int count, void* stream);
int hrp_bn_fold(const hrp_bn_entry* table_dev, int count, void* stream);
int hrp_bn_param_grad(const hrp_bn_entry* table_dev, int count, void* stream);

int hrp_avgpool_fwd(const void* x, int dtype, int N, int HW, int C, int pitch, float* out, int out_pitch, void* stream);
int hrp_avgpool_bwd(const float* dout, int dout_pitch, void* dx, int dtype, int N, int HW, int C, int pitch, int accumulate, void* stream);

int hrp_softargmax3d_fwd(const void* logits, int dtype, int B, int J, int D, int H, int W, int pitch,
                         int root, int fix_root, float* uvd, float* ms, void* stream);
int hrp_softargmax3d_bwd(const void* logits, int dtype, int B, int J, int D, int H, int W, int pitch,
                         int root, int fix_root, const float* uvd, const float* ms, const float* duvd,
                         void* dlogits, int dpitch, void* stream);

int hrp_pose_geometry_fwd(const float* gamma, const float* k_value, const float* uvd, const float* K,
                          int B, int J, int root, float image_size, float depth_factor,
                          float* depth, float* xyz, float* root_uv, float* trans, void* stream);
int hrp_pose_geometry_bwd(const float* gamma, const float* k_value, const float* uvd, const float* K,
                          int B, int J, int root, float image_size, float depth_factor,
                          const float* d_depth, const float* d_xyz, const float* d_root_uv, const float* d_trans,
                          float* d_gamma, float* d_uvd, void* stream);

int hrp_softargmax_flat_fwd(const void* logits, int dtype, int B, int J, int HW, int pitch, float* coord, float* ms, void* stream);
int hrp_softargmax_flat_bwd(const void* logits, int dtype, int B, int J, int HW, int pitch, const float* coord, const float* ms,
                            const float* dcoord, void* dlogits, int dpitch, void* stream);

int hrp_rot6d_compose_fwd(const float* a, const float* b, float* out, int N, void* stream);
int hrp_rot6d_compose_bwd(const float* a, const float* b, const float* dout, float* da, float* db, int N, int acc_a, int acc_b,
                          void* stream);

int hrp_fk_project_fwd(const hrp_fk_chain* chain_dev, const float* q, const float* rot6d, const float* trans,
                       const float* K, int B, int root, float* xyz, float* uv, float* root_rot6d, void* stream);
typedef struct hrp_silhouette_desc {
  const float* uv;
  const float* xyz;
  const int32_t* faces;
  int32_t B, V, F, H, W;
  float sigma, blur_radius;
  float* alpha;
  int64_t* logp;
  int32_t* count;
} hrp_silhouette_desc;
int hrp_silhouette_fwd(const hrp_silhouette_desc* d, void* stream);
int hrp_silhouette_bwd(const hrp_silhouette_desc* d, const float* d_alpha, float* d_uv, void* stream);

int hrp_mesh_pose(const hrp_fk_chain* chain_dev, const float* q, const float* rot6d, const float* trans, int B, int root_kp,
                  const float* verts, const uint8_t* vert_link, int V, const float* K, float* xyz, float* uv, void* stream);
int hrp_mesh_pose_bwd(const hrp_fk_chain* chain_dev, const float* q, const float* rot6d, const float* trans, int B, int root_kp,
                      const float* verts, const uint8_t* vert_link, int V, const float* d_xyz, float* d_rot6d, float* d_trans, void* stream);
int hrp_fk_project_bwd(const hrp_fk_chain* chain_dev, const float* q, const float* rot6d, const float* trans,
                       const float* K, int B, int root, const float* d_xyz, const float* d_uv,
                       float* d_q, float* d_rot6d, float* d_trans, void* stream);
int hrp_fk_project_rot_fwd(const hrp_fk_chain* chain_dev, const float* q, const float* rot, int rot_dim, const float* trans,
                           const float* K, int B, int root, float* xyz, float* uv, float* root_rot, void* stream);
int hrp_fk_project_rot_bwd(const hrp_fk_chain* chain_dev, const float* q, const float* rot, int rot_dim, const float* trans,
                           const float* K, int B, int root, const float* d_xyz, const float* d_uv,
                           float* d_q, float* d_rot, float* d_trans, void* stream);

int hrp_copy_cols(const float* src, int src_pitch, float* dst, int dst_pitch, int rows, int cols, int accumulate, void* stream);
#define HRP_COPY_MAX 16
typedef struct hrp_copy_desc {
  const float* src;
  float* dst;
  int src_pitch, dst_pitch, rows, cols;
  int accumulate, reserved;
} hrp_copy_desc;
int hrp_copy_cols_batch(const hrp_copy_desc* descs, int n, void* stream);
int hrp_scale_rows(float* x, int pitch, int rows, int cols, const float* row_scale, float s, void* stream);
int hrp_mul_f32(const float* x, int x_pitch, const float* m, int m_pitch, float* y, int y_pitch, int rows, int cols,
                int accumulate, void* stream);
int64_t hrp_linear_workspace_bytes(int M, int K, int N);
int hrp_linear_fwd(const float* x, int x_pitch, const float* w, const float* bias, const float* res, int res_pitch,
                   float* y, int y_pitch, int M, int K, int N, void* workspace, int64_t workspace_bytes, void* stream);
int hrp_linear_bwd_data(const float* dy, int dy_pitch, const float* w, float* dx, int dx_pitch, int M, int K, int N,
                        int accumulate, void* workspace, int64_t workspace_bytes, void* stream);
int hrp_linear_bwd_weight(const float* x, int x_pitch, const float* dy, int dy_pitch, float* dw, float* dbias, int M, int K,
                          int N, int accumulate, void* stream);

typedef struct hrp_pose_loss_desc {
  const float *pose, *rot, *trans, *root_uv, *depth, *xyz_int, *xyz_fk;
  const float *gt_pose, *gt_root_rot, *gt_root_trans, *gt_root_uv;
  const float *gt_kp3d, *gt_kp2d, *mask, *K;
  float *d_pose, *d_rot, *d_trans, *d_root_uv, *d_depth, *d_xyz_int, *d_xyz_fk;
  float* out;
  float weights[10];
  int32_t B, P, J, root;
  float image_size;
  int32_t rot_dim;
} hrp_pose_loss_desc;
int hrp_pose_loss(const hrp_pose_loss_desc* d, void* stream);
int hrp_l1_loss(const float* pred, const float* gt, float scale, int n, float* loss, float* d_pred, void* stream);

typedef struct hrp_sim2real_loss_desc {
  const float* rendered;
  const float* seg;
  const float* kp3d;
  const float* kp3d_int;
  int32_t B, HW, K, mask_loss;
  float w_mask, w_iou, w_scale, w_align;
  float* terms;
  float* d_rendered;
  float* d_kp3d;
  float* d_kp3d_int;
  float* workspace;
} hrp_sim2real_loss_desc;
int hrp_sim2real_loss(const hrp_sim2real_loss_desc* d, void* stream);

int hrp_rng_advance(uint64_t* state_dev, void* stream);
int hrp_dropout_f32(const float* x, int x_pitch, float* y, int y_pitch, float* mask, int rows, int cols, float keep,
                    const uint64_t* state_dev, uint32_t salt, void* stream);
int hrp_dropout_masks(float* masks, int64_t n, float keep, const uint64_t* state_dev, uint32_t salt, void* stream);

#define HRP_REG_MAX_P 16
#define HRP_REG_MAX_PROBLEMS 4
typedef struct hrp_regressor_step_desc {
  int32_t M, P, K, N;
  const float* u_prev;
  const float* u_bias;
  const float* z;
  const float* zw;
  int32_t z_len, z_pitch, zw_sk, zw_sp;
  float* u_out;
  const float* a;
  const float* a_mask;
  const float* v;
  int32_t a_pitch, v_sk, v_sp, a2_pitch;
  float* a_out;
  const float* w;
  const float* bias;
  const float* out_mask;
  const float* a2;
  const float* w2;
  int64_t w_sn, w_sk;
  int32_t out_pitch, out_accumulate, out_sum_accumulate;
  int32_t w2_sk;
  float* out;
  float* out_sum;
} hrp_regressor_step_desc;
int hrp_regressor_step(const hrp_regressor_step_desc* descs, int n, void* stream);

#define HRP_LIN_WGRAD_MAX 8
typedef struct hrp_linear_wgrad_desc {
  const float* x;
  const float* dy;
  float* dw;
  float* dbias;
  int32_t x_pitch, dy_pitch, dw_ld, M, K, N, accumulate, reserved;
} hrp_linear_wgrad_desc;
int hrp_linear_wgrad_batch(const hrp_linear_wgrad_desc* descs, int n, void* stream);

int hrp_project_fwd(const float* K, const float* pts, int B, int P, float* uv, void* stream);
int hrp_project_bwd(const float* K, const float* pts, const float* duv, int B, int P, float* dpts, void* stream);

int hrp_pnp_solve(const float* pts2d, const float* pts3d, int pts3d_stride, const float* K, int K_stride, const float* ini_pose,
                  int B, int n, float* P6d, int* status, float* rms, void* stream);
int hrp_pnp_bwd(const float* pts2d, const float* pts3d, int pts3d_stride, const float* K, int K_stride, const float* P6d,
                const float* grad_out, int B, int n, int fast, float* grad_x, float* grad_z, float* grad_K, float* grad_z_sum,
                float* grad_K_sum, int* status, void* stream);

enum { HRP_PNP_NO_CONSENSUS = 1, HRP_PNP_CONVERGED = 2, HRP_PNP_FEW_POINTS = 4 };
int hrp_pnp_solve_robust(const float* pts2d, const float* pts3d, int pts3d_stride, const float* K, int K_stride,
                         const unsigned char* valid, int B, int n, double reproj_error, int min_inliers, int max_hypotheses,
                         unsigned seed, int refine_all, float* P6d, unsigned char* inliers, int* status, float* rms, void* stream);
int hrp_pnp_bwd_masked(const float* pts2d, const float* pts3d, int pts3d_stride, const float* K, int K_stride, const float* P6d,
                       const float* grad_out, const unsigned char* mask, int B, int n, int fast, float* grad_x, float* grad_z,
                       float* grad_K, float* grad_z_sum, float* grad_K_sum, int* status, void* stream);

enum { HRP_PNP_POOLED_MAX_N = 16384, HRP_PNP_POOLED_REFITS = 8 };
int hrp_pnp_pooled_workspace_bytes(int B, int n, int max_hypotheses, size_t* bytes);
int hrp_pnp_solve_pooled(const float* pts2d, const float* pts3d, const float* K, int K_stride, const unsigned char* valid, int B, int n,
                         double reproj_error, int min_inliers, int max_hypotheses, unsigned seed, int refine_all, void* workspace,
                         size_t workspace_bytes, float* P6d, unsigned char* inliers, int* status, float* rms, float* cov, void* stream);

#define HRP_DREAM_BANDS 32
enum {
  HRP_DREAM_JITTER = 1, HRP_DREAM_OCCLUSION = 2, HRP_DREAM_SHARPNESS = 4, HRP_DREAM_CONTRAST = 8, HRP_DREAM_BRIGHTNESS = 16,
  HRP_DREAM_COLOR = 32
};
typedef struct {
  double jitter[3];
  double enh[4];
  int32_t flags;
  int32_t occ_x, occ_y, occ_w, occ_h;
  int32_t pad_x, pad_y, work_w, work_h;
  int32_t crop_x0, crop_y0, crop_x1, crop_y1;
  int32_t off_x, off_y, side;
  int32_t reserved;
  int64_t noise_off;
  int64_t scratch_off;
} hrp_dream_sample;
int hrp_dream_augment(const uint8_t* frames, int B, int H, int W, const hrp_dream_sample* table_dev, const uint8_t* noise,
                      int64_t noise_bytes, int max_h, int max_w, uint8_t* scratch, int64_t scratch_bytes, uint64_t* lsum, void* stream);
int hrp_dream_crop_resize(const uint8_t* scratch, int64_t scratch_bytes, const hrp_dream_sample* table_dev, const uint64_t* lsum, int B,
                          int max_h, int max_w, uint8_t* out0, int h0, int w0, uint8_t* out1, int h1, int w1, void* stream);

typedef struct hrp_eval_desc {
  const float* pred_kp3d_fk;
  const float* pred_kp3d_int;
  const float* gt_kp3d;
  const float* gt_kp2d;
  const float* K;
  const float* pred_joint;
  const float* gt_joint;
  const float* pred_rot;
  const float* gt_rot;
  float *error3d, *error2d, *mean_jointerror, *error_depth, *batch_error_relative, *error3d_relative;
  float *error3d_int, *error2d_int, *error_depth_int, *batch_error_relative_int, *error3d_relative_int;
  float *dis3d, *dis2d, *dis3d_int, *dis2d_int;
  float* l1_jointerror;
  float* rotation_diff;
  int32_t B, nkp, dof;
  int32_t rot_dim;
  int32_t root;
  int32_t drop_last_joint;
  int32_t offset, capacity;
  int32_t batch_index, batch_capacity;
} hrp_eval_desc;
int hrp_eval_batch(const hrp_eval_desc* d, void* stream);

#define HRP_DEPTH_LOSS_MAX_KP 16
enum { HRP_DEPTH_LOSS_L1 = 0, HRP_DEPTH_LOSS_MSE = 1 };
enum { HRP_XY_LOSS_NONE = 0, HRP_XY_LOSS_L1 = 1, HRP_XY_LOSS_MSE = 2 };
typedef struct hrp_depth_loss_desc {
  const float* pred;
  const float* gt_root_trans;
  const float* gt_kp3d;
  const float* mask;
  float* loss;
  float* d_pred;
  float* errors;
  float* losses;
  int32_t B, W, J, nk;
  int32_t kp_index[HRP_DEPTH_LOSS_MAX_KP];
  int32_t depth_loss, xy_loss;
  int32_t root_col;
// ... 205 lines not shown
```

Before: 2087 images/sec.

## Fuse Adam update with packed-weight layout emission in one optimizer kernel

Adds an optimizer kernel that updates conv weight tiles with Adam, stages the updated fp32 tile in LDS, and writes the packed (and transposed) bf16/f32 layouts the conv kernels consume. The next forward prep then skips repacking those adopted weights, which removes a separate pass that re-reads every parameter. Version and epoch tracking, plus a PackedParameter data hook, detect outside writes and fall back to a full repack. This adds registry bookkeeping and more LDS use in the optimizer, and a stale packed copy would be used if invalidation were missed.

```diff
diff --git a/holistic-robot-pose-estimation_amd/_native.py b/holistic-robot-pose-estimation_amd/_native.py
--- a/holistic-robot-pose-estimation_amd/_native.py
+++ b/holistic-robot-pose-estimation_amd/_native.py
@@ -205,6 +205,19 @@
 class OptGroup(C.Structure):
     _fields_ = [("lr", C.c_float), ("beta1", C.c_float), ("beta2", C.c_float), ("eps", C.c_float),
                 ("weight_decay", C.c_float), ("reserved", C.c_float * 3)]
+
+
+OPT_PACK_SETS = 2
+PACK_TILE_TAPS = 9
+
+
+class OptPackDst(C.Structure):
+    _fields_ = [("dst", C.c_void_p), ("dst_t", C.c_void_p), ("pad_t", C.c_int32), ("dtype", C.c_int32)]
+
+
+class OptTileEntry(C.Structure):
+    _fields_ = [("tensor", C.c_int32), ("Cout", C.c_int32), ("Cin", C.c_int32), ("ntaps", C.c_int32),
+                ("nsets", C.c_int32), ("reserved", C.c_int32), ("set", OptPackDst * OPT_PACK_SETS)]
 
 
 class RegStepDesc(C.Structure):
@@ -396,6 +409,7 @@
     "hrp_opt_grad_sumsq": [_P, _P, _I, _P, _P, _P],
     "hrp_opt_adam_step": [_P, _P, _I, _P, _F, _P, _F, _F, _F, _F, _P],
     "hrp_opt_adam_step_groups": [_P, _P, _I, _P, _F, _P, _P, _I, _P, _P],
+    "hrp_opt_adam_step_pack": [_P, _P, _P, _I, _I, _P, _I, _P, _F, _P, _F, _F, _F, _F, _P, _I, _P, _P],
     "hrp_opt_set_group": [_P, _I, _I, _F, _F, _F, _F, _F, _P],
     "hrp_grad_accumulate": [_P, _P, _L, _I, _F, _P],
     "hrp_batch_prepare": [_I, _P, _I, _P, C.POINTER(BatchInfo)],
diff --git a/holistic-robot-pose-estimation_amd/csrc/core.hip b/holistic-robot-pose-estimation_amd/csrc/core.hip
--- a/holistic-robot-pose-estimation_amd/csrc/core.hip
+++ b/holistic-robot-pose-estimation_amd/csrc/core.hip
@@ -245,8 +245,37 @@
 }
 
 template <typename T>
+__device__ __forceinline__ void pack_tile_rows(void* dst, void* dst_t, const unsigned pad_t, const unsigned Cout, const unsigned Cin,
+                                               const unsigned nt, const unsigned co0, const unsigned ci0, const float* __restrict__ lds) {
+  constexpr int CK = 32 / Elem<T>::SZ, NC = 32 / CK;
+  const unsigned cout_pad = (Cout + 31) / 32 * 32, cin_pad = (Cin + 31) / 32 * 32;
+  const unsigned pitch = 32 * nt + 1;
+  if (dst) {
+    const unsigned nch = (Cin + CK - 1) / CK;
+    for (unsigned r = threadIdx.x; r < NC * nt * 32; r += 256) {
+      const unsigned co = r & 31, q = r >> 5, tap = q % nt, c = q / nt, ch = ci0 / CK + c;
+      if (ch >= nch) continue;
+      float v[CK];
+#pragma unroll
+      for (int k = 0; k < CK; ++k) v[k] = lds[co * pitch + (c * CK + k) * nt + tap];
+      pack_store_row<T>(dst, (size_t)(ch * nt + tap) * cout_pad + co0 + co, v);
+    }
+  }
+  if (dst_t) {
+    const unsigned nch = (Cout + CK - 1) / CK;
+    for (unsigned r = threadIdx.x; r < NC * nt * 32; r += 256) {
+      const unsigned ci = r & 31, q = r >> 5, tap = q % nt, c = q / nt, ch = co0 / CK + c;
+      if (ch >= nch) continue;
+      float v[CK];
+#pragma unroll
+      for (int k = 0; k < CK; ++k) v[k] = lds[(c * CK + k) * pitch + ci * nt + tap];
+      pack_store_row<T>(dst_t, (size_t)(ch * (nt + pad_t) + tap) * cin_pad + ci0 + ci, v);
+    }
+  }
+}
+
+template <typename T>
 __device__ __forceinline__ void pack_entry_tile(const hrp_pack_entry& e, const unsigned tile_id, float* __restrict__ lds) {
-  constexpr int CK = 32 / Elem<T>::SZ, NC = 32 / CK;
   const unsigned Cout = e.Cout, Cin = e.Cin, nt = e.ntaps;
   const unsigned cout_pad = (Cout + 31) / 32 * 32, cin_pad = (Cin + 31) / 32 * 32;
   const unsigned n_cit = cin_pad / 32;
@@ -270,28 +299,7 @@
     }
   }
   __syncthreads();
-  if (e.dst) {
-    const unsigned nch = (Cin + CK - 1) / CK;
-    for (unsigned r = threadIdx.x; r < NC * nt * 32; r += 256) {
-      const unsigned co = r & 31, q = r >> 5, tap = q % nt, c = q / nt, ch = ci0 / CK + c;
-      if (ch >= nch) continue;
-      float v[CK];
-#pragma unroll
-      for (int k = 0; k < CK; ++k) v[k] = lds[co * pitch + (c * CK + k) * nt + tap];
-      pack_store_row<T>(e.dst, (size_t)(ch * nt + tap) * cout_pad + co0 + co, v);
-    }
-  }
-  if (e.dst_t) {
-    const unsigned nch = (Cout + CK - 1) / CK;
-    for (unsigned r = threadIdx.x; r < NC * nt * 32; r += 256) {
-      const unsigned ci = r & 31, q = r >> 5, tap = q % nt, c = q / nt, ch = co0 / CK + c;
-      if (ch >= nch) continue;
-      float v[CK];
-#pragma unroll
-      for (int k = 0; k < CK; ++k) v[k] = lds[(c * CK + k) * pitch + ci * nt + tap];
-      pack_store_row<T>(e.dst_t, (size_t)(ch * (nt + e.pad_t) + tap) * cin_pad + ci0 + ci, v);
-    }
-  }
+  pack_tile_rows<T>(e.dst, e.dst_t, e.pad_t, Cout, Cin, nt, co0, ci0, lds);
 }
 
 constexpr int PACK_ROWS_PER_BLOCK = 256 * 4;
@@ -718,6 +726,40 @@
   if (threadIdx.x < HRP_STAT_SLOTS) slots[threadIdx.x] = threadIdx.x == 0 ? part[0] : 0.f;
 }
 
+struct opt_adam_coef {
+  float clip, b1, b2, step_size, inv_sqrt_bc2, eps, wd;
+};
+__device__ __forceinline__ opt_adam_coef opt_adam_coefs(const float* __restrict__ slots, float max_norm, const float* __restrict__ step_dev,
+                                                        float lr, float b1, float b2, float eps, float wd) {
+  float clip = 1.f;
+  if (max_norm > 0.f) {
+    float ss = 0.f;
+#pragma unroll
+    for (int k = 0; k < HRP_STAT_SLOTS; ++k) ss += slots[k];
+    clip = fminf(1.f, max_norm / (sqrtf(ss) + 1e-6f));
+  }
+  const float step = *step_dev;
+  const float bc1 = 1.f - powf(b1, step), bc2 = 1.f - powf(b2, step);
+  const float step_size = lr / bc1, inv_sqrt_bc2 = 1.f / sqrtf(bc2);
+  return {clip, b1, b2, step_size, inv_sqrt_bc2, eps, wd};
+}
+template <bool WD, bool FUSED>
+__device__ __forceinline__ void opt_adam_update(float& pp, float& gg, float& mm, float& vv, const opt_adam_coef& c) {
+#pragma clang fp contract(off)
+  gg *= c.clip;
+  float ge = gg;
+  if constexpr (WD) ge = __builtin_fmaf(c.wd, pp, gg);
+  if constexpr (FUSED) {
+    mm = __builtin_fmaf(1.f - c.b1, ge, c.b1 * mm);
+    vv = __builtin_fmaf(ge, (1.f - c.b2) * ge, c.b2 * vv);
+    pp -= c.step_size * mm / __builtin_fmaf(sqrtf(vv), c.inv_sqrt_bc2, c.eps);
+  } else {
+    mm = c.b1 * mm + (1.f - c.b1) * ge;
+    vv = c.b2 * vv + (1.f - c.b2) * ge * ge;
+    pp -= c.step_size * mm / (sqrtf(vv) * c.inv_sqrt_bc2 + c.eps);
+  }
+}
+
 template <bool DECAY>
 __device__ __forceinline__ void opt_adam_chunk(const hrp_opt_tensor t, const hrp_opt_chunk ck, const float* __restrict__ slots,
                                                float max_norm, const float* __restrict__ step_dev, float lr, float b1, float b2,
@@ -725,45 +767,137 @@
   const int64_t base = (int64_t)ck.offset * HRP_OPT_CHUNK;
   const int64_t left = t.numel - base;
   const int n = left < HRP_OPT_CHUNK ? (int)left : HRP_OPT_CHUNK;
-  float clip = 1.f;
-  if (max_norm > 0.f) {
-    float ss = 0.f;
-#pragma unroll
-    for (int k = 0; k < HRP_STAT_SLOTS; ++k) ss += slots[k];
-    clip = fminf(1.f, max_norm / (sqrtf(ss) + 1e-6f));
-  }
-  const float step = *step_dev;
-  const float bc1 = 1.f - powf(b1, step), bc2 = 1.f - powf(b2, step);
-  const float step_size = lr / bc1, inv_sqrt_bc2 = 1.f / sqrtf(bc2);
+  const opt_adam_coef c = opt_adam_coefs(slots, max_norm, step_dev, lr, b1, b2, eps, wd);
   float* p = t.param + base;
   float* g = t.grad + base;
   float* m = t.exp_avg + base;
   float* v = t.exp_avg_sq + base;
   auto run = [&](auto with_decay) {
-    auto upd = [&](float& pp, float& gg, float& mm, float& vv) {
-      gg *= clip;
-      if constexpr (decltype(with_decay)::value) {
-        const float ge = gg + wd * pp;
-        mm = b1 * mm + (1.f - b1) * ge;
-        vv = b2 * vv + (1.f - b2) * ge * ge;
-      } else {
-        mm = b1 * mm + (1.f - b1) * gg;
-        vv = b2 * vv + (1.f - b2) * gg * gg;
-      }
-      pp -= step_size * mm / (sqrtf(vv) * inv_sqrt_bc2 + eps);
-    };
+    constexpr bool WD = decltype(with_decay)::value;
     if ((n & 3) == 0 && (((uintptr_t)p | (uintptr_t)g | (uintptr_t)m | (uintptr_t)v) & 15) == 0) {
       for (int i = threadIdx.x * 4; i < n; i += 1024) {
         float4 pp = *(float4*)(p + i), gg = *(float4*)(g + i), mm = *(float4*)(m + i), vv = *(float4*)(v + i);
-        upd(pp.x, gg.x, mm.x, vv.x); upd(pp.y, gg.y, mm.y, vv.y); upd(pp.z, gg.z, mm.z, vv.z); upd(pp.w, gg.w, mm.w, vv.w);
+        opt_adam_update<WD, true>(pp.x, gg.x, mm.x, vv.x, c); opt_adam_update<WD, true>(pp.y, gg.y, mm.y, vv.y, c);
+        opt_adam_update<WD, true>(pp.z, gg.z, mm.z, vv.z, c); opt_adam_update<WD, true>(pp.w, gg.w, mm.w, vv.w, c);
         *(float4*)(p + i) = pp; *(float4*)(g + i) = gg; *(float4*)(m + i) = mm; *(float4*)(v + i) = vv;
       }
     } else {
-      for (int i = threadIdx.x; i < n; i += 256) upd(p[i], g[i], m[i], v[i]);
+      for (int i = threadIdx.x; i < n; i += 256) opt_adam_update<WD, false>(p[i], g[i], m[i], v[i], c);
     }
   };
   if (DECAY && wd != 0.f) run(std::true_type{});
   else run(std::false_type{});
+}
+
+template <bool WD>
+__device__ __forceinline__ void opt_adam_tile_update(const hrp_opt_tensor& t, const unsigned Cout, const unsigned Cin, const unsigned nt,
+                                                     const unsigned co0, const unsigned ci0, const opt_adam_coef& c,
+                                                     float* __restrict__ lds) {
+  const unsigned span = 32 * nt, pitch = span + 1;
+  const unsigned valid = Cin > ci0 ? (Cin - ci0 < 32 ? (Cin - ci0) * nt : span) : 0;
+  const unsigned rows = Cout > co0 ? (Cout - co0 < 32 ? Cout - co0 : 32) : 0;
+  const size_t row_stride = (size_t)Cin * nt, base = ((size_t)co0 * Cin + ci0) * nt;
+  float* p = t.param + base;
+  float* g = t.grad + base;
+  float* m = t.exp_avg + base;
+  float* v = t.exp_avg_sq + base;
+  if ((row_stride & 3) == 0 && (valid & 3) == 0 && (((uintptr_t)p | (uintptr_t)g | (uintptr_t)m | (uintptr_t)v) & 15) == 0) {
+    constexpr int U = 3;
+    const unsigned q = span / 4;
+    for (unsigned k0 = 0; k0 < nt; k0 += U) {
+      float4 pp[U], gg[U], mm[U], vv[U];
+      unsigned row[U], j[U];
+      bool in[U];
+#pragma unroll
+      for (int u = 0; u < U; ++u) {
+        const unsigned f = threadIdx.x + (k0 + u) * 256;
+        row[u] = f / q, j[u] = (f - row[u] * q) * 4;
+        in[u] = k0 + u < nt && row[u] < rows && j[u] < valid;
+        pp[u] = gg[u] = mm[u] = vv[u] = make_float4(0.f, 0.f, 0.f, 0.f);
+        if (in[u]) {
+          const size_t o = row[u] * row_stride + j[u];
+          pp[u] = *(const float4*)(p + o), gg[u] = *(const float4*)(g + o), mm[u] = *(const float4*)(m + o), vv[u] = *(const float4*)(v + o);
+        }
+      }
+#pragma unroll
+      for (int u = 0; u < U; ++u) {
+        if (in[u]) {
+          opt_adam_update<WD, true>(pp[u].x, gg[u].x, mm[u].x, vv[u].x, c); opt_adam_update<WD, true>(pp[u].y, gg[u].y, mm[u].y, vv[u].y, c);
+          opt_adam_update<WD, true>(pp[u].z, gg[u].z, mm[u].z, vv[u].z, c); opt_adam_update<WD, true>(pp[u].w, gg[u].w, mm[u].w, vv[u].w, c);
+          const size_t o = row[u] * row_stride + j[u];
+          *(float4*)(p + o) = pp[u]; *(float4*)(g + o) = gg[u]; *(float4*)(m + o) = mm[u]; *(float4*)(v + o) = vv[u];
+        }
+        if (k0 + u < nt) {
+          float* l = lds + row[u] * pitch + j[u];
+          l[0] = pp[u].x, l[1] = pp[u].y, l[2] = pp[u].z, l[3] = pp[u].w;
+        }
+      }
+    }
+  } else {
+    const bool aligned = (((uintptr_t)t.param | (uintptr_t)t.grad | (uintptr_t)t.exp_avg | (uintptr_t)t.exp_avg_sq) & 15) == 0;
+    const size_t scalar_from = !aligned ? 0 : (t.numel & 3) ? (size_t)((t.numel - 1) / HRP_OPT_CHUNK) * HRP_OPT_CHUNK : (size_t)t.numel;
+    for (unsigned f = threadIdx.x; f < 32 * span; f += 256) {
+      const unsigned row = f / span, j = f - row * span;
+      float pp = 0.f;
+      if (row < rows && j < valid) {
+        const size_t o = row * row_stride + j;
+        float gg = g[o], mm = m[o], vv = v[o];
+        pp = p[o];
+        if (base + o < scalar_from) opt_adam_update<WD, true>(pp, gg, mm, vv, c);
+        else opt_adam_update<WD, false>(pp, gg, mm, vv, c);
+        p[o] = pp, g[o] = gg, m[o] = mm, v[o] = vv;
+      }
+      lds[row * pitch + j] = pp;
+    }
+  }
+}
+
+template <bool GROUPS>
+__global__ __launch_bounds__(256) void opt_adam_pack_kernel(const hrp_opt_tensor* __restrict__ tensors,
+                                                            const hrp_opt_tile_entry* __restrict__ tiles,
+                                                            const int32_t* __restrict__ first, const int ntile_entries,
+                                                            const int total_tiles, const hrp_opt_chunk* __restrict__ chunks,
+                                                            const float* __restrict__ slots, float max_norm,
+                                                            const float* __restrict__ step_dev, float lr, float b1, float b2, float eps,
+                                                            const hrp_opt_group* __restrict__ groups, int ngroups,
+                                                            const int32_t* __restrict__ tensor_group) {
+  __shared__ float lds[32 * (32 * PACK_TILE_TAPS + 1)];
+  float wd = 0.f;
+  auto hyper = [&](const int tensor) {
+    if constexpr (GROUPS) {
+      const int gi = tensor_group[tensor];
+      const hrp_opt_group h = groups[gi < 0 ? 0 : gi >= ngroups ? ngroups - 1 : gi];
+      lr = h.lr, b1 = h.beta1, b2 = h.beta2, eps = h.eps, wd = h.weight_decay;
+    }
+  };
+  if ((int)blockIdx.x >= total_tiles) {
+    const hrp_opt_chunk ck = chunks[blockIdx.x - total_tiles];
+    hyper(ck.tensor);
+    opt_adam_chunk<GROUPS>(tensors[ck.tensor], ck, slots, max_norm, step_dev, lr, b1, b2, eps, wd);
+    return;
+  }
+  int lo = 0, hi = ntile_entries;
+  while (hi - lo > 1) {
+    const int mid = (lo + hi) >> 1;
+    if (first[mid] <= (int)blockIdx.x) lo = mid; else hi = mid;
+  }
+  const hrp_opt_tile_entry& e = tiles[lo];
+  const unsigned Cout = e.Cout, Cin = e.Cin, nt = e.ntaps, tile_id = blockIdx.x - first[lo];
+  const unsigned n_cit = (Cin + 31) / 32;
+  if (nt < 1 || nt > PACK_TILE_TAPS || tile_id >= ((Cout + 31) / 32) * n_cit) return;
+  const unsigned co0 = (tile_id / n_cit) * 32, ci0 = (tile_id % n_cit) * 32;
+  hyper(e.tensor);
+  const opt_adam_coef c = opt_adam_coefs(slots, max_norm, step_dev, lr, b1, b2, eps, wd);
+  const hrp_opt_tensor t = tensors[e.tensor];
+  if (GROUPS && wd != 0.f) opt_adam_tile_update<true>(t, Cout, Cin, nt, co0, ci0, c, lds);
+  else opt_adam_tile_update<false>(t, Cout, Cin, nt, co0, ci0, c, lds);
+  __syncthreads();
+  for (int s = 0; s < e.nsets && s < HRP_OPT_PACK_SETS; ++s) {
+    const hrp_opt_pack_dst d = e.set[s];
+    if (d.dtype == HRP_F32) pack_tile_rows<float>(d.dst, d.dst_t, d.pad_t, Cout, Cin, nt, co0, ci0, lds);
+    else if (d.dtype == HRP_F32X3) pack_tile_rows<f32x3_t>(d.dst, d.dst_t, d.pad_t, Cout, Cin, nt, co0, ci0, lds);
+    else pack_tile_rows<bf16_t>(d.dst, d.dst_t, d.pad_t, Cout, Cin, nt, co0, ci0, lds);
+  }
 }
 
 __global__ __launch_bounds__(256) void opt_adam_kernel(const hrp_opt_tensor* __restrict__ tensors,
@@ -825,6 +959,30 @@
   hipLaunchKernelGGL(opt_adam_groups_kernel, dim3(nchunks), dim3(256), 0, (hipStream_t)stream, tensors_dev, chunks_dev,
                      sumsq_slots, max_norm, step_dev, groups_dev, ngroups, tensor_group_dev);
   return check_launch("opt_adam_step_groups");
+}
+extern "C" int hrp_opt_adam_step_pack(const hrp_opt_tensor* tensors_dev, const hrp_opt_tile_entry* tiles_dev,
+                                      const int32_t* first_tile_dev, int ntile_entries, int total_tiles,
+                                      const hrp_opt_chunk* chunks_dev, int nchunks, const float* sumsq_slots, float max_norm,
+                                      const float* step_dev, float lr, float beta1, float beta2, float eps,
+                                      const hrp_opt_group* groups_dev, int ngroups, const int32_t* tensor_group_dev, void* stream) {
+  HRP_REQUIRE(tensors_dev && step_dev && ntile_entries >= 0 && total_tiles >= 0 && nchunks >= 0 && total_tiles + nchunks > 0,
+              "opt_adam_step_pack: bad args");
+  HRP_REQUIRE(total_tiles == 0 || (tiles_dev && first_tile_dev && ntile_entries > 0 && total_tiles >= ntile_entries),
+              "opt_adam_step_pack: tiles without a table / fewer tiles than entries");
+  HRP_REQUIRE(nchunks == 0 || chunks_dev, "opt_adam_step_pack: chunks without a table");
+  HRP_REQUIRE(max_norm <= 0.f || sumsq_slots, "opt_adam_step_pack: clipping needs the sum-of-squares slots");
+  HRP_REQUIRE(!groups_dev == !tensor_group_dev, "opt_adam_step_pack: group table and tensor -> group map come together");
+  HRP_REQUIRE(!groups_dev || ngroups >= 1, "opt_adam_step_pack: ngroups %d < 1", ngroups);
+  const dim3 grid(total_tiles + nchunks);
+  if (groups_dev)
+    hipLaunchKernelGGL(opt_adam_pack_kernel<true>, grid, dim3(256), 0, (hipStream_t)stream, tensors_dev, tiles_dev, first_tile_dev,
+                       ntile_entries, total_tiles, chunks_dev, sumsq_slots, max_norm, step_dev, 0.f, 0.f, 0.f, 0.f, groups_dev, ngroups,
+                       tensor_group_dev);
+  else
+    hipLaunchKernelGGL(opt_adam_pack_kernel<false>, grid, dim3(256), 0, (hipStream_t)stream, tensors_dev, tiles_dev, first_tile_dev,
+                       ntile_entries, total_tiles, chunks_dev, sumsq_slots, max_norm, step_dev, lr, beta1, beta2, eps, groups_dev, 0,
+                       tensor_group_dev);
+  return check_launch("opt_adam_step_pack");
 }
 extern "C" int hrp_opt_set_group(hrp_opt_group* groups_dev, int ngroups, int index, float lr, float beta1, float beta2, float eps,
                                  float weight_decay, void* stream) {
diff --git a/holistic-robot-pose-estimation_amd/optim.py b/holistic-robot-pose-estimation_amd/optim.py
--- a/holistic-robot-pose-estimation_amd/optim.py
+++ b/holistic-robot-pose-estimation_amd/optim.py
@@ -1,8 +1,25 @@
 import ctypes as C
+import weakref
 
 import torch
 
 from . import _native as nv
+
+
+def pack_step_tables(numels, packed):
+    tiles, first, chunks = [], [0], []
+    for i, n in enumerate(numels):
+        e = packed.get(i)
+        if e is None:
+            chunks += [(i, k) for k in range((n + nv.OPT_CHUNK - 1) // nv.OPT_CHUNK)]
+            continue
+        cout, cin, ntaps, sets = e
+        if not (1 <= ntaps <= nv.PACK_TILE_TAPS and cout * cin * ntaps == n and 1 <= len(sets) <= nv.OPT_PACK_SETS):
+            raise ValueError(f"pack_step_tables: tensor {i} ({n} elements) cannot be walked by tiles as {cout} x {cin} x {ntaps} "
+                             f"with {len(sets)} destination sets")
+        tiles.append((i, cout, cin, ntaps, list(sets)))
+        first.append(first[-1] + ((cout + 31) // 32) * ((cin + 31) // 32))
+    return tiles, first, chunks
 
 
 class FusedClipAdam(torch.optim.Optimizer):
@@ -49,6 +66,10 @@
         self._grad_ptrs = None
         self._tensors = self._chunks = None
         self._nchunks = 0
+        self._registry_epoch = None
+        self._adopted, self._adopted_keep = [], []
+        self._tiles = self._first_tile = self._rest_chunks = None
+        self._ntile_entries = self._ntiles = self._nrest = 0
         if self._device_hyper:
             ng = len(self.param_groups)
             self._groups = torch.zeros(ng * C.sizeof(nv.OptGroup) // 4, dtype=torch.float32, device=dev)
@@ -116,10 +137,50 @@
             g["capturable"] = True
         self._publish_state()
 
+    def _adopt_plans(self):
+        from . import plan as plan_mod
+        self._adopted, self._adopted_keep = [], []
+        packed = {}
+        if not plan_mod.OPT_PACK:
+            return packed
+        index = {id(p): i for i, p in enumerate(self.params)}
+        plans = {}
+        for p in self.params:
+            for r in plan_mod.pack_registrations(p):
+                plans.setdefault(id(r.plan()), r.plan())
+        for pl in plans.values():
+            if pl is None or pl.opt_pack_disabled:
+                continue
+            regs = [(r, r.param()) for r in pl.pack_regs]
+            other = pl._adopter() if pl._adopter is not None else None
+            if (other is not None and other is not self) or any(q is None or id(q) not in index for _, q in regs):
+                pl.disable_opt_pack()
+                continue
+            fits = all(type(q) in (torch.nn.Parameter, plan_mod.PackedParameter) and
+                       (index[id(q)] not in packed or
+                        (len(packed[index[id(q)]][3]) < nv.OPT_PACK_SETS and packed[index[id(q)]][:3] == (r.cout, r.cin, r.ntaps)))
+                       for r, q in regs)
+            if not fits:
+                if other is self:
+                    pl._adopter, pl.packed_by_optimizer = None, False
+                continue
+            for r, q in regs:
+                packed.setdefault(index[id(q)], (r.cout, r.cin, r.ntaps, []))[3].append((r.dst, r.dst_t, r.pad_t, r.cdt))
+                if type(q) is torch.nn.Parameter:
+                    q.__class__ = plan_mod.PackedParameter
+            pl._adopter = weakref.ref(self)
+            self._adopted.append(weakref.ref(pl))
+            self._adopted_keep += [w.arena for w in pl._adoptable]
+        return packed
+
     def _build_tables(self):
+        from . import plan as plan_mod
         ptrs = tuple(p.grad.data_ptr() for p in self.params)
-        if ptrs == self._grad_ptrs:
+        if (ptrs == self._grad_ptrs and self._registry_epoch == plan_mod.PACK_REGISTRY_EPOCH
+                and all(r() is not None for r in self._adopted)):
             return
+        packed = self._adopt_plans()
+        self._registry_epoch = plan_mod.PACK_REGISTRY_EPOCH
         tab = (nv.OptTensor * len(self.params))()
         chunks = []
         for i, (p, (m, v)) in enumerate(zip(self.params, self.state_views)):
@@ -137,6 +198,24 @@
         self._nchunks = len(chunks)
         self._chunk_sums = torch.zeros(self._nchunks, dtype=torch.float32, device=self.device)
         self._grad_ptrs = ptrs
+        self._tiles = self._first_tile = self._rest_chunks = None
+        self._ntile_entries = self._ntiles = self._nrest = 0
+        if packed:
+            tiles, first, rest = pack_step_tables([p.numel() for p in self.params], packed)
+            tt = (nv.OptTileEntry * len(tiles))()
+            for j, (i, cout, cin, ntaps, sets) in enumerate(tiles):
+                tt[j].tensor, tt[j].Cout, tt[j].Cin, tt[j].ntaps, tt[j].nsets = i, cout, cin, ntaps, len(sets)
+                for k, (dst, dst_t, pad_t, cdt) in enumerate(sets):
+                    tt[j].set[k].dst, tt[j].set[k].dst_t, tt[j].set[k].pad_t, tt[j].set[k].dtype = dst, dst_t, pad_t, cdt
+            self._tiles = torch.frombuffer(bytearray(bytes(tt)), dtype=torch.uint8).to(self.device)
+            self._first_tile = torch.tensor(first, dtype=torch.int32, device=self.device)
+            self._ntile_entries, self._ntiles = len(tiles), first[-1]
+            if rest:
+                rk = (nv.OptChunk * len(rest))()
+                for j, (i, k) in enumerate(rest):
+                    rk[j].tensor, rk[j].offset = i, k
+                self._rest_chunks = torch.frombuffer(bytearray(bytes(rk)), dtype=torch.uint8).to(self.device)
+                self._nrest = len(rest)
 
     def prepare(self):
         if any(p.grad is None for p in self.params):
@@ -160,7 +239,19 @@
         if self.max_norm > 0:
             nv.call("hrp_opt_grad_sumsq", self._tensors.data_ptr(), self._chunks.data_ptr(), self._nchunks,
                     self._slots.data_ptr(), self._chunk_sums.data_ptr(), s)
-        if self._device_hyper:
+        if self._ntiles:
+            dh = self._device_hyper
+            nv.call("hrp_opt_adam_step_pack", self._tensors.data_ptr(), self._tiles.data_ptr(), self._first_tile.data_ptr(),
+                    self._ntile_entries, self._ntiles, self._rest_chunks.data_ptr() if self._nrest else None, self._nrest,
+                    self._slots.data_ptr(), self.max_norm, self.step_count.data_ptr(),
+                    float(g["lr"]), float(g["betas"][0]), float(g["betas"][1]), float(g["eps"]),
+                    self._groups.data_ptr() if dh else None, len(self.param_groups) if dh else 0,
+                    self._tensor_group.data_ptr() if dh else None, s)
+            for r in self._adopted:
+                pl = r()
+                if pl is not None:
+                    pl.opt_packed(self)
+        elif self._device_hyper:
             nv.call("hrp_opt_adam_step_groups", self._tensors.data_ptr(), self._chunks.data_ptr(), self._nchunks,
                     self._slots.data_ptr(), self.max_norm, self.step_count.data_ptr(),
                     self._groups.data_ptr(), len(self.param_groups), self._tensor_group.data_ptr(), s)
diff --git a/holistic-robot-pose-estimation_amd/plan.py b/holistic-robot-pose-estimation_amd/plan.py
--- a/holistic-robot-pose-estimation_amd/plan.py
+++ b/holistic-robot-pose-estimation_amd/plan.py
@@ -3,6 +3,7 @@
 import ctypes as C
 import math
 import os
+import weakref
 
 import torch
 
@@ -149,6 +150,61 @@
 def bump_param_epoch():
     global PARAM_EPOCH
     PARAM_EPOCH += 1
+
+
+OPT_PACK = os.environ.get("HRP_OPT_PACK", "0") not in ("0", "")
+PACK_REGISTRY = {}
+PACK_REGISTRY_EPOCH = 0
+FOREIGN_WRITE_EPOCH = 0
+
+
+class PackReg:
+    __slots__ = ("plan", "param", "dst", "dst_t", "cout", "cin", "ntaps", "pad_t", "cdt")
+
+    def __init__(self, plan, w, esz):
+        self.plan, self.param = weakref.ref(plan), weakref.ref(w.param)
+        self.dst = w.arena.data_ptr() + w.fwd_off * esz
+        self.dst_t = (w.arena.data_ptr() + w.bwd_off * esz) if w.need_t else None
+        self.cout, self.cin, self.ntaps, self.pad_t, self.cdt = w.cout, w.cin, w.ntaps, w.pad_t, _cdt(plan, w.dtype)
+
+
+def _registry_changed():
+    global PACK_REGISTRY_EPOCH
+    PACK_REGISTRY_EPOCH += 1
+
+
+def pack_registrations(param):
+    regs = PACK_REGISTRY.get(id(param))
+    if not regs:
+        return []
+    live = [r for r in regs if r.plan() is not None and r.param() is param]
+    if len(live) != len(regs):
+        if live:
+            PACK_REGISTRY[id(param)] = live
+        else:
+            del PACK_REGISTRY[id(param)]
+    return live
+
+
+def _note_foreign_write():
+    global FOREIGN_WRITE_EPOCH
+    FOREIGN_WRITE_EPOCH += 1
+
+
+_TENSOR_DATA = torch._C.TensorBase.data
+
+
+class PackedParameter(torch.nn.Parameter):
+
+    @property
+    def data(self):
+        _note_foreign_write()
+        return _TENSOR_DATA.__get__(self)
+
+    @data.setter
+    def data(self, value):
+        _note_foreign_write()
+        _TENSOR_DATA.__set__(self, value)
 
 
 Entry = collections.namedtuple("Entry", "lane path op")
@@ -506,6 +562,13 @@
         self.pending_inputs = []
         self.pending_block_ends = []
         self.row_last_writer = {}
+        self.pack_regs = []
+        self._adoptable = []
+        self._adopter = None
+        self.opt_pack_disabled = False
+        self.packed_by_optimizer = False
+        self._opt_versions = None
+        self.prep_skipped_pack = False
 
     def new(self, N, H, W, Cc, dtype=None, pitch=None):
         return TensorH(self, N, H, W, Cc, dtype or self.dtype, pitch=pitch)
@@ -597,11 +660,16 @@
             self._side_streams = [torch.cuda.Stream(device=dev) for _ in range(self.n_lanes - 1)]
         self._bn_tables()
         self.built = True
+        if self.pack_regs:
+            for r in self.pack_regs:
+                PACK_REGISTRY[id(r.param())] = pack_registrations(r.param()) + [r]
+            _registry_changed()
         if PLAN_STATS:
             self._print_stats()
 
     def _layout_packed_weights(self, cut):
         self._pack_tables, self._pack_tables_late = [], []
+        self._pack_tables_rest, self._pack_tables_late_rest = [], []
         for w in self.weight_list:
             assert all(t == w.ntaps + w.pad_t for t in w.t_ntaps), f"plan: data gradients of one weight disagree on its tap slots ({w.t_ntaps}, pad_t {w.pad_t})"
         for dtype in (torch.float32, torch.bfloat16):
@@ -627,7 +695,18 @@
                 w.arena = arena
             early = [w for w in ws if cut is None or w.first_use is None or w.first_use < cut]
             late = [w for w in ws if not (cut is None or w.first_use is None or w.first_use < cut)]
-            for group, dest in ((early, self._pack_tables), (late, self._pack_tables_late)):
+            adopt = [w for w in ws if OPT_PACK and self.need_grad and w.src is None and w.ntaps <= nv.PACK_TILE_TAPS
+                     and w.param.requires_grad and w.param.dtype == torch.float32 and w.param.is_contiguous()
+                     and w.param.numel() == w.cout * w.cin * w.ntaps]
+            for w in adopt:
+                self._adoptable.append(w)
+                self.pack_regs.append(PackReg(self, w, esz))
+            aid = {id(w) for w in adopt}
+            groups = [(early, self._pack_tables), (late, self._pack_tables_late)]
+            if adopt:
+                groups += [([w for w in early if id(w) not in aid], self._pack_tables_rest),
+                           ([w for w in late if id(w) not in aid], self._pack_tables_late_rest)]
+            for group, dest in groups:
                 if not group:
                     continue
                 tab = (nv.PackEntry * len(group))()
@@ -745,16 +824,49 @@
         if self._pack_stream is not None and not SERIAL_LANES:
             self._pack_stream.wait_stream(torch.cuda.current_stream(self.device))
             late_s = self._pack_stream.cuda_stream
-        for tdev, fdev, n, nblk, dt in self._pack_tables_late:
+        early_tabs, late_tabs = self._pack_tables, self._pack_tables_late
+        if self._adoptable:
+            self.prep_skipped_pack = bool(force) and self.opt_pack_valid()
+            if self.prep_skipped_pack:
+                early_tabs, late_tabs = self._pack_tables_rest, self._pack_tables_late_rest
+            else:
+                self.packed_by_optimizer = False
+        for tdev, fdev, n, nblk, dt in late_tabs:
             nv.call("hrp_pack_weights_compact", tdev.data_ptr(), fdev.data_ptr(), n, nblk, dt, late_s)
         if late_s != s and self.need_grad and self.grad_arena is not None:
             with torch.cuda.stream(self._pack_stream):
                 self.grad_arena.zero_()
             self._arena_clean = True
-        for tdev, fdev, n, nblk, dt in self._pack_tables:
+        for tdev, fdev, n, nblk, dt in early_tabs:
             nv.call("hrp_pack_weights_compact", tdev.data_ptr(), fdev.data_ptr(), n, nblk, dt, s)
         if self._fold_tab:
             nv.call("hrp_bn_fold", self._fold_tab[0].data_ptr(), self._fold_tab[1], s)
+
+    def _opt_state(self):
+        return tuple(w.param._version for w in self._adoptable) + (FOREIGN_WRITE_EPOCH,)
+
+    def opt_packed(self, optimizer):
+        if self._adopter is not None and self._adopter() is optimizer and not self.opt_pack_disabled:
+            self.packed_by_optimizer, self._opt_versions = True, self._opt_state()
+
+    def opt_pack_valid(self):
+        if not self.packed_by_optimizer:
+            return False
+        if (self.opt_pack_disabled or self._adopter is None or self._adopter() is None
+                or self._opt_state() != self._opt_versions):
+            self.packed_by_optimizer = False
+            return False
+        return True
+
+    def disable_opt_pack(self):
+        self.opt_pack_disabled, self.packed_by_optimizer, self._adopter = True, False, None
+        _registry_changed()
+
+    def pack_all_now(self):
+        s = self._stream()
+        for tdev, fdev, n, nblk, dt in self._pack_tables_late + self._pack_tables:
+            nv.call("hrp_pack_weights_compact", tdev.data_ptr(), fdev.data_ptr(), n, nblk, dt, s)
+        self.packed_by_optimizer = False
 
     def lane_id(self, parent, index):
         key = (parent, index)
diff --git a/holistic-robot-pose-estimation_amd/runtime.py b/holistic-robot-pose-estimation_amd/runtime.py
--- a/holistic-robot-pose-estimation_amd/runtime.py
+++ b/holistic-robot-pose-estimation_amd/runtime.py
@@ -26,6 +26,7 @@
         self.calls = self.bwd_calls = 0
         self.g_fwd = self.g_bwd = self.static_in = None
         self.graph_failed = False
+        self.fwd_skips_pack = False
 
     def _forward_launches(self, prep=True):
         p = self.plan
@@ -86,6 +87,7 @@
                 for n, st in zip(self.in_names, self.static_in):
                     p.dyn[n] = st
                 self.g_fwd = self._capture("fwd")
+                self.fwd_skips_pack = self.g_fwd is not None and p.need_grad and p.prep_skipped_pack
             if self.g_fwd is not None and p.need_grad and self.g_bwd is None and self.bwd_calls >= GRAPH_WARMUP:
                 self.g_bwd = self._capture("bwd")
         if self.g_fwd is not None and self._graphs_allowed():
@@ -93,6 +95,8 @@
                 st.copy_(t)
             if not p.need_grad:
                 p.run_prep(force=False)
+            elif self.fwd_skips_pack and not p.opt_pack_valid():
+                p.pack_all_now()
             self.g_fwd.replay()
             if p.training and p._run_tab:
                 from .plan import bump_param_epoch
diff --git a/include/hrp.h b/include/hrp.h
--- a/include/hrp.h
+++ b/include/hrp.h
@@ -250,6 +250,25 @@
 int hrp_opt_adam_step_groups(const hrp_opt_tensor* tensors_dev, const hrp_opt_chunk* chunks_dev, int nchunks,
                              const float* sumsq_slots, float max_norm, const float* step_dev,
                              const hrp_opt_group* groups_dev, int ngroups, const int32_t* tensor_group_dev, void* stream);
+#define HRP_OPT_PACK_SETS 2
+typedef struct hrp_opt_pack_dst {
+  void* dst;
+  void* dst_t;
+  int32_t pad_t;
+  int32_t dtype;
+} hrp_opt_pack_dst;
+typedef struct hrp_opt_tile_entry {
+  int32_t tensor;
+  int32_t Cout, Cin, ntaps;
+  int32_t nsets;
+  int32_t reserved;
+  hrp_opt_pack_dst set[HRP_OPT_PACK_SETS];
+} hrp_opt_tile_entry;
+int hrp_opt_adam_step_pack(const hrp_opt_tensor* tensors_dev, const hrp_opt_tile_entry* tiles_dev, const int32_t* first_tile_dev,
+                           int ntile_entries, int total_tiles, const hrp_opt_chunk* chunks_dev, int nchunks,
+                           const float* sumsq_slots, float max_norm, const float* step_dev,
+                           float lr, float beta1, float beta2, float eps,
+                           const hrp_opt_group* groups_dev, int ngroups, const int32_t* tensor_group_dev, void* stream);
 int hrp_opt_set_group(hrp_opt_group* groups_dev, int ngroups, int index, float lr, float beta1, float beta2, float eps,
                       float weight_decay, void* stream);
 int hrp_grad_accumulate(const float* src, float* acc, int64_t n, int first, float scale, void* stream);
```

After: 2086 images/sec, median of 2. About the same (-0.0%).
